# damaggu/StableKeypoints

Hardware: AMD Instinct MI355X
Metric: images/sec (token-opt step, 512², N=500 tokens) (higher is better)
Workload: dtype f32

## Files before the change

include/skp.h:

```cpp
#ifndef SKP_H
#define SKP_H

#ifdef __cplusplus
extern "C" {
#endif

#define SKP_OK 0
#define SKP_EBADARG (-1)
#define SKP_ELAUNCH (-2)
#define SKP_MAX_LAYERS 16

const char* skp_last_error(void);
int skp_version(void);

int skp_capture_fwd(const float* z_low, int BH, int s, int N, int R, float* attn, float* stats, void* stream);

int skp_capture_bwd(const float* z_low, int BH, int s, int N, int R, const float* dattn, int group, long long sb,
                    long long sp, long long sn, float gscale, const float* stats, float* dz_low, float* workspace,
                    void* stream);

int skp_capture_maps_fwd(const float* const* z_low, const int* sizes, int L, int B, int H, int N, int R, float* maps,
                         float* const* stats, void* stream);

int skp_capture_maps_bwd(const float* const* z_low, const int* sizes, int L, int B, int H, int N, int R,
                         const float* dmaps, float gscale, const float* const* stats, float* const* dz_low,
                         float* workspace, void* stream);

long long skp_capture_maps_bwd_sel_workspace(const int* sizes, int L, int B, int H, int N, int R, int K);
int skp_capture_maps_bwd_sel(const float* const* z_low, const int* sizes, int L, int B, int H, int N, int R,
                             const long long* sel_tok, int K, const float* gsel, float gscale,
                             const float* const* stats, float* const* dz_low, float* workspace, void* stream);
int skp_sel_bwd_timing(int enable);
int skp_sel_bwd_timing_read(double* ms, int* calls);

int skp_aggregate(const float* const* layers, int L, int BH, int RR, int N, const long long* indices,
                  int n_out, float* out, void* stream);

int skp_resize_bilinear(const float* in, int C, int R, int Ro, float* out, void* stream);
int skp_resize_bilinear_bwd(const float* gout, int C, int R, int Ro, float* gin, void* stream);

int skp_argmax2d(const float* maps, int T, int h, int w, const long long* rows, int n_rows, float* pos,
                 long long* idx, void* stream);

int skp_k_max_pixels(const float* maps, int T, int h, int w, int num, float radius2, float* pos,
                     float* masked, void* stream);

int skp_mask_radius(const float* maps, int T, int h, int w, const float* pos, float radius2, float* out,
                    void* stream);

int skp_weighted_avg(float* maps, int T, int h, int w, float distance, int mutate, float* pos, void* stream);

int skp_gaussian_target(const float* pos, int num, int T, int size, float sigma, float* out, void* stream);

int skp_topk_gaussian(const float* maps, int T, int h, int w, int top_k, float sigma, float epsilon,
                      int num_subjects, long long* out, double* kl, void* workspace, void* stream);

int skp_topk_gaussian_batch(const float* maps, int nb, int T, int h, int w, int top_k, float sigma,
                            float epsilon, int num_subjects, long long* out, double* kl, void* workspace,
                            void* stream);

int skp_topk_keys(const double* keys, int nb, int T, int top_k, long long* out, void* stream);

int skp_entropy_sort(const float* maps, int T, int h, int w, int top_k, long long* out, double* ent,
                     void* workspace, void* stream);

int skp_fps(const float* maps, int T, int h, int w, const long long* cand, int n_cand, int top_k,
            long long* out, int* n_out, void* workspace, void* stream);
int skp_fps_batch(const float* maps, int nb, int T, int h, int w, const long long* cand, int n_cand, int top_k,
                  long long* out, int* n_out, void* workspace, void* stream);
int skp_fps_keys_batch(const double* keys, const float* maps, int nb, int T, int h, int w, int n_cand, int top_k,
                       long long* cand, long long* out, int* n_out, void* workspace, void* stream);

int skp_sharpen_fwd(const float* A, int T, int h, int w, float sigma, int num_subjects, float* pos,
                     double* partial, float* loss, void* stream);
int skp_sharpen_bwd(const float* A, int T, int h, int w, float sigma, int num_subjects, const float* pos,
                     const float* gout, float* dA, void* stream);
int skp_sharpen_fwd_batch(const float* A, int nb, int T, int h, int w, float sigma, int num_subjects, float* pos,
                          double* partial, float* loss, void* stream);
int skp_sharpen_bwd_batch(const float* A, int nb, int T, int h, int w, float sigma, int num_subjects,
                          const float* pos, const float* gout, float* dA, void* stream);

int skp_affine_warp(const float* x, int B, int C, int H, int W, const float* theta, float* out, void* stream);
int skp_affine_warp_bwd(const float* gout, int B, int C, int H, int W, const float* theta, float* gin,
                        void* stream);

int skp_equiv_fwd(const float* A, const float* At, int T, int h, int w, const float* theta_inv,
                  double* partial, float* loss, void* stream);
int skp_equiv_bwd(const float* A, const float* At, int T, int h, int w, const float* theta_inv,
                  const float* gout, float* dA, float* dAt, void* stream);
int skp_equiv_fwd_batch(const float* A, const float* At, int nb, int T, int h, int w, const float* theta_inv,
                        double* partial, float* loss, void* stream);
int skp_equiv_bwd_batch(const float* A, const float* At, int nb, int T, int h, int w, const float* theta_inv,
                        const float* gout, float* dA, float* dAt, void* stream);

int skp_wino_in_transform(const float* x, int B, int C, int H, int W, float* V, void* stream);
int skp_wino_out_transform(const float* M, int B, int K, int H, int W, const float* bias, const float* residual,
                           float* y, void* stream);
int skp_wino_out_transform_kt(const float* M, int B, int K, int H, int W, const float* bias, const float* residual,
                              float* y, float* gn_part, void* stream);

int skp_bgemm_f32(const float* A, long long sAb, long long sAm, long long sAk, const float* B, long long sBb,
                  long long sBk, long long sBn, float* C, long long sCb, long long sCm, long long sCn, int batch,
                  int M, int N, int K, float alpha, int accumulate, void* stream);
int skp_bgemm_f32_2b(const float* A, long long sAo, long long sAb, long long sAm, long long sAk, const float* B,
                     long long sBo, long long sBb, long long sBk, long long sBn, float* C, long long sCo, long long sCb,
                     long long sCm, long long sCn, int batch, int hb, int M, int N, int K, float alpha, int accumulate,
                     void* stream);

int skp_groupnorm_workspace(int B, int C, long long HW, int G);
int skp_groupnorm_fwd(const float* x, const float* gamma, const float* beta, const float* shift, int B, int C,
                      long long HW, int G, float eps, int act, float* y, float* stats, double* partial,
                      void* stream);
int skp_groupnorm_bwd(const float* x, const float* dy, const float* gamma, const float* beta, const float* shift,
                      const float* stats, int B, int C, long long HW, int G, int act, float* dx, double* partial,
                      void* stream);
int skp_groupnorm_fwd_part(const float* x, const float* gamma, const float* beta, const float* shift, const float* part,
                           int nseg, int B, int C, long long HW, int G, float eps, int act, float* y, float* stats,
                           double* partial, void* stream);
int skp_groupnorm_stats(const float* x, const float* shift, int B, int C, long long HW, int G, float eps, float* stats,
                        double* partial, void* stream);
int skp_groupnorm_stats_part(const float* part, int nseg, const float* shift, int B, int C, long long HW, int G,
                             float eps, float* stats, double* partial, void* stream);
int skp_groupnorm_bwd_add(const float* x, const float* dy, const float* gamma, const float* beta, const float* shift,
                          const float* stats, int B, int C, long long HW, int G, int act, const float* dres, float* dx,
                          double* partial, void* stream);
int skp_softmax_bwd(const float* P, float* dP, long long rows, int cols, float alpha, void* stream);
int skp_softmax_fwd(float* S, long long rows, int cols, void* stream);
int skp_attn_dscore(const float* P, const float* dO, const float* V, const float* D, float* out, int BH, int S, int L,
                    int d, float alpha, void* stream);
int skp_attn_bwd_kv(const float* P, const float* dO, const float* Q, const float* V, const float* D, float* dS,
                    float* dV, float* dK, int BH, int S, int L, int d, float alpha, void* stream);
int skp_attn_fwd(const float* Q, const float* K, const float* V, float* O, float* stats, int BH, int S, int L, int d,
                 float scale, void* stream);
int skp_attn_bwd_flash(const float* Q, const float* K, const float* V, const float* dO, const float* stats,
                       const float* D, float* dS, float* dV, float* dK, int BH, int S, int L, int d, float scale,
                       void* stream);
int skp_attn_fwd_bshd(const float* Q, long long q_sb, int q_rs, const float* K, long long k_sb, int k_rs,
                      const float* V, long long v_sb, int v_rs, float* O, long long o_sb, int o_rs, float* stats, int B,
                      int H, int S, int L, int d, float scale, void* stream);
int skp_attn_bwd_flash_bshd(const float* Q, long long q_sb, int q_rs, const float* K, long long k_sb, int k_rs,
                            const float* V, long long v_sb, int v_rs, const float* dO, long long o_sb, int o_rs,
                            const float* stats, const float* D, float* dS, float* dV, long long dv_sb, int dv_rs,
                            float* dK, long long dk_sb, int dk_rs, int B, int H, int S, int L, int d, float scale,
                            void* stream);
int skp_layernorm_fwd(const float* x, const float* gamma, const float* beta, long long rows, int C, float eps, float* y,
                      float* stats, void* stream);
int skp_layernorm_bwd(const float* x, const float* dy, const float* gamma, const float* stats, long long rows, int C,
                      float* dx, void* stream);
int skp_layernorm_bwd_add(const float* x, const float* dy, const float* gamma, const float* stats, long long rows,
                          int C, const float* dres, float* dx, void* stream);
int skp_geglu_fwd(const float* h, long long rows, int I, float* out, void* stream);
int skp_geglu_bwd(const float* h, const float* dout, long long rows, int I, float* dh, void* stream);
int skp_residual_bias_add(const float* a, const float* h, const float* bias, int B, int C, long long HW,
                          float* out, void* stream);
int skp_wino_weights(const float* w, int K, int C, int flip, float* U, void* stream);
int skp_conv3x3_wino(const float* x, const float* U, const float* bias, const float* residual, float* y, int B, int C,
                     int K, int H, int W, int nsplit, float* ws, void* stream);
int skp_wino2_weights(const float* w, int K, int C, int flip, float* U, void* stream);
int skp_conv3x3_wino2(const float* x, const float* U, const float* bias, const float* residual, float* y, int B,
                      int C, int K, int H, int W, int nsplit, float* ws, void* stream);
int skp_conv3x3_wino2_gn(const float* x, const float* U, const float* bias, const float* residual, float* y, int B,
                         int C, int K, int H, int W, int nsplit, float* ws, float* gn_part, void* stream);
int skp_wino2_vtransform(const float* x, float* V, int B, int C, int H, int W, void* stream);
int skp_wino2_vtransform_gn(const float* x, const float* stats, const float* gamma, const float* beta,
                            const float* shift, int G, int act, float* V, int B, int C, int H, int W, void* stream);
int skp_conv3x3_wino2_v(const float* V, const float* U, const float* bias, const float* residual, float* y, int B,
                        int C, int K, int H, int W, int nsplit, float* ws, void* stream);
int skp_conv3x3_wino2_v_gn(const float* V, const float* U, const float* bias, const float* residual, float* y, int B,
                           int C, int K, int H, int W, int nsplit, float* ws, float* gn_part, void* stream);
int skp_conv3x3s2_wino2(const float* x, const float* U, const float* bias, float* y, int B, int C, int K, int H,
                        int W, int nsplit, float* ws, void* stream);

int skp_map_range(const float* maps, int n, int h, int w, float* range, void* stream);
int skp_render_sheet(const float* images, int n, int H, int W, const float* maps, int h, int w, const float* range,
                     const float* lut, float alpha, const float* points, int K, float radius,
                     const unsigned char* colors, int rows, int cols, int f, int pad, unsigned char* out,
                     void* stream);

int skp_tta_reduce_workspace(int B, int n, int S);
int skp_tta_reduce(const float* maps, int B, int C, int n, int S, const float* theta_inv, float* pos, float* avg,
                   void* workspace, void* stream);

#ifdef __cplusplus
}
#endif
#endif
```

stablekeypoints_amd/_lib.py:

```python
import ctypes
import os

import torch

_HERE = os.path.dirname(os.path.abspath(__file__))
LIB_PATH = os.environ.get("SKP_LIB", os.path.join(_HERE, "libskp.so"))

_c_int, _c_float, _c_ll, _p = ctypes.c_int, ctypes.c_float, ctypes.c_longlong, ctypes.c_void_p

_SIGS = {
    "skp_capture_fwd": [_p, _c_int, _c_int, _c_int, _c_int, _p, _p, _p],
    "skp_capture_bwd": [_p, _c_int, _c_int, _c_int, _c_int, _p, _c_int, _c_ll, _c_ll, _c_ll, _c_float, _p, _p, _p,
                        _p],
    "skp_capture_maps_fwd": [ctypes.POINTER(_p), ctypes.POINTER(_c_int), _c_int, _c_int, _c_int, _c_int, _c_int, _p,
                             ctypes.POINTER(_p), _p],
    "skp_capture_maps_bwd": [ctypes.POINTER(_p), ctypes.POINTER(_c_int), _c_int, _c_int, _c_int, _c_int, _c_int, _p,
                             _c_float, ctypes.POINTER(_p), ctypes.POINTER(_p), _p, _p],
    "skp_capture_maps_bwd_sel": [ctypes.POINTER(_p), ctypes.POINTER(_c_int), _c_int, _c_int, _c_int, _c_int, _c_int,
                                 _p, _c_int, _p, _c_float, ctypes.POINTER(_p), ctypes.POINTER(_p), _p, _p],
    "skp_sel_bwd_timing": [_c_int],
    "skp_sel_bwd_timing_read": [_p, _p],
    "skp_capture_maps_bwd_sel_workspace": [ctypes.POINTER(_c_int), _c_int, _c_int, _c_int, _c_int, _c_int, _c_int],
    "skp_aggregate": [ctypes.POINTER(_p), _c_int, _c_int, _c_int, _c_int, _p, _c_int, _p, _p],
    "skp_resize_bilinear": [_p, _c_int, _c_int, _c_int, _p, _p],
    "skp_resize_bilinear_bwd": [_p, _c_int, _c_int, _c_int, _p, _p],
    "skp_argmax2d": [_p, _c_int, _c_int, _c_int, _p, _c_int, _p, _p, _p],
    "skp_k_max_pixels": [_p, _c_int, _c_int, _c_int, _c_int, _c_float, _p, _p, _p],
    "skp_mask_radius": [_p, _c_int, _c_int, _c_int, _p, _c_float, _p, _p],
    "skp_weighted_avg": [_p, _c_int, _c_int, _c_int, _c_float, _c_int, _p, _p],
    "skp_gaussian_target": [_p, _c_int, _c_int, _c_int, _c_float, _p, _p],
    "skp_topk_gaussian": [_p, _c_int, _c_int, _c_int, _c_int, _c_float, _c_float, _c_int, _p, _p, _p, _p],
    "skp_topk_gaussian_batch": [_p, _c_int, _c_int, _c_int, _c_int, _c_int, _c_float, _c_float, _c_int, _p, _p, _p,
                                _p],
    "skp_topk_keys": [_p, _c_int, _c_int, _c_int, _p, _p],
    "skp_entropy_sort": [_p, _c_int, _c_int, _c_int, _c_int, _p, _p, _p, _p],
    "skp_fps": [_p, _c_int, _c_int, _c_int, _p, _c_int, _c_int, _p, _p, _p, _p],
    "skp_fps_batch": [_p, _c_int, _c_int, _c_int, _c_int, _p, _c_int, _c_int, _p, _p, _p, _p],
    "skp_fps_keys_batch": [_p, _p, _c_int, _c_int, _c_int, _c_int, _c_int, _c_int, _p, _p, _p, _p, _p],
    "skp_sharpen_fwd": [_p, _c_int, _c_int, _c_int, _c_float, _c_int, _p, _p, _p, _p],
    "skp_sharpen_bwd": [_p, _c_int, _c_int, _c_int, _c_float, _c_int, _p, _p, _p, _p],
    "skp_wino_in_transform": [_p, _c_int, _c_int, _c_int, _c_int, _p, _p],
    "skp_wino_out_transform": [_p, _c_int, _c_int, _c_int, _c_int, _p, _p, _p, _p],
    "skp_wino_out_transform_kt": [_p, _c_int, _c_int, _c_int, _c_int, _p, _p, _p, _p, _p],
    "skp_sharpen_fwd_batch": [_p, _c_int, _c_int, _c_int, _c_int, _c_float, _c_int, _p, _p, _p, _p],
    "skp_sharpen_bwd_batch": [_p, _c_int, _c_int, _c_int, _c_int, _c_float, _c_int, _p, _p, _p, _p],
    "skp_affine_warp": [_p, _c_int, _c_int, _c_int, _c_int, _p, _p, _p],
    "skp_affine_warp_bwd": [_p, _c_int, _c_int, _c_int, _c_int, _p, _p, _p],
    "skp_equiv_fwd": [_p, _p, _c_int, _c_int, _c_int, _p, _p, _p, _p],
    "skp_equiv_bwd": [_p, _p, _c_int, _c_int, _c_int, _p, _p, _p, _p, _p],
    "skp_equiv_fwd_batch": [_p, _p, _c_int, _c_int, _c_int, _c_int, _p, _p, _p, _p],
    "skp_equiv_bwd_batch": [_p, _p, _c_int, _c_int, _c_int, _c_int, _p, _p, _p, _p, _p],
    "skp_bgemm_f32": [_p, _c_ll, _c_ll, _c_ll, _p, _c_ll, _c_ll, _c_ll, _p, _c_ll, _c_ll, _c_ll, _c_int, _c_int,
                      _c_int, _c_int, _c_float, _c_int, _p],
    "skp_bgemm_f32_2b": [_p, _c_ll, _c_ll, _c_ll, _c_ll, _p, _c_ll, _c_ll, _c_ll, _c_ll, _p, _c_ll, _c_ll, _c_ll,
                         _c_ll, _c_int, _c_int, _c_int, _c_int, _c_int, _c_float, _c_int, _p],
    "skp_groupnorm_workspace": [_c_int, _c_int, _c_ll, _c_int],
    "skp_groupnorm_fwd": [_p, _p, _p, _p, _c_int, _c_int, _c_ll, _c_int, _c_float, _c_int, _p, _p, _p, _p],
    "skp_groupnorm_bwd": [_p, _p, _p, _p, _p, _p, _c_int, _c_int, _c_ll, _c_int, _c_int, _p, _p, _p],
    "skp_groupnorm_bwd_add": [_p, _p, _p, _p, _p, _p, _c_int, _c_int, _c_ll, _c_int, _c_int, _p, _p, _p, _p],
    "skp_residual_bias_add": [_p, _p, _p, _c_int, _c_int, _c_ll, _p, _p],
    "skp_softmax_bwd": [_p, _p, _c_ll, _c_int, _c_float, _p],
    "skp_softmax_fwd": [_p, _c_ll, _c_int, _p],
    "skp_attn_dscore": [_p, _p, _p, _p, _p, _c_int, _c_int, _c_int, _c_int, _c_float, _p],
    "skp_attn_bwd_kv": [_p, _p, _p, _p, _p, _p, _p, _p, _c_int, _c_int, _c_int, _c_int, _c_float, _p],
    "skp_attn_fwd": [_p, _p, _p, _p, _p, _c_int, _c_int, _c_int, _c_int, _c_float, _p],
    "skp_attn_bwd_flash": [_p, _p, _p, _p, _p, _p, _p, _p, _p, _c_int, _c_int, _c_int, _c_int, _c_float, _p],
    "skp_attn_fwd_bshd": [_p, _c_ll, _c_int, _p, _c_ll, _c_int, _p, _c_ll, _c_int, _p, _c_ll, _c_int, _p, _c_int, _c_int,
                          _c_int, _c_int, _c_int, _c_float, _p],
    "skp_attn_bwd_flash_bshd": [_p, _c_ll, _c_int, _p, _c_ll, _c_int, _p, _c_ll, _c_int, _p, _c_ll, _c_int, _p, _p, _p,
                                _p, _c_ll, _c_int, _p, _c_ll, _c_int, _c_int, _c_int, _c_int, _c_int, _c_int, _c_float,
                                _p],
    "skp_layernorm_fwd": [_p, _p, _p, _c_ll, _c_int, _c_float, _p, _p, _p],
    "skp_layernorm_bwd": [_p, _p, _p, _p, _c_ll, _c_int, _p, _p],
    "skp_layernorm_bwd_add": [_p, _p, _p, _p, _c_ll, _c_int, _p, _p, _p],
    "skp_geglu_fwd": [_p, _c_ll, _c_int, _p, _p],
    "skp_geglu_bwd": [_p, _p, _c_ll, _c_int, _p, _p],
    "skp_wino_weights": [_p, _c_int, _c_int, _c_int, _p, _p],
    "skp_conv3x3_wino": [_p, _p, _p, _p, _p, _c_int, _c_int, _c_int, _c_int, _c_int, _c_int, _p, _p],
    "skp_wino2_weights": [_p, _c_int, _c_int, _c_int, _p, _p],
    "skp_conv3x3_wino2": [_p, _p, _p, _p, _p, _c_int, _c_int, _c_int, _c_int, _c_int, _c_int, _p, _p],
    "skp_conv3x3_wino2_gn": [_p, _p, _p, _p, _p, _c_int, _c_int, _c_int, _c_int, _c_int, _c_int, _p, _p, _p],
    "skp_groupnorm_fwd_part": [_p, _p, _p, _p, _p, _c_int, _c_int, _c_int, _c_ll, _c_int, _c_float, _c_int, _p, _p, _p,
                               _p],
    "skp_groupnorm_stats": [_p, _p, _c_int, _c_int, _c_ll, _c_int, _c_float, _p, _p, _p],
    "skp_groupnorm_stats_part": [_p, _c_int, _p, _c_int, _c_int, _c_ll, _c_int, _c_float, _p, _p, _p],
    "skp_wino2_vtransform": [_p, _p, _c_int, _c_int, _c_int, _c_int, _p],
    "skp_wino2_vtransform_gn": [_p, _p, _p, _p, _p, _c_int, _c_int, _p, _c_int, _c_int, _c_int, _c_int, _p],
    "skp_conv3x3_wino2_v": [_p, _p, _p, _p, _p, _c_int, _c_int, _c_int, _c_int, _c_int, _c_int, _p, _p],
    "skp_conv3x3_wino2_v_gn": [_p, _p, _p, _p, _p, _c_int, _c_int, _c_int, _c_int, _c_int, _c_int, _p, _p, _p],
    "skp_conv3x3s2_wino2":[_p, _p, _p, _p, _c_int, _c_int, _c_int, _c_int, _c_int, _c_int, _p, _p],
    "skp_map_range": [_p, _c_int, _c_int, _c_int, _p, _p],
    "skp_render_sheet": [_p, _c_int, _c_int, _c_int, _p, _c_int, _c_int, _p, _p, _c_float, _p, _c_int, _c_float, _p,
                         _c_int, _c_int, _c_int, _c_int, _p, _p],
    "skp_tta_reduce_workspace": [_c_int, _c_int, _c_int],
    "skp_tta_reduce": [_p, _c_int, _c_int, _c_int, _c_int, _p, _p, _p, _p, _p],
    "skp_version": [],
}


_RESTYPE = {"skp_capture_maps_bwd_sel_workspace": _c_ll}
_MEASUREMENT_ONLY = {"skp_sel_bwd_timing", "skp_sel_bwd_timing_read"}


class SkpLibraryError(RuntimeError):
    pass


_lib = None


def lib():
    global _lib
    if _lib is None:
        if not os.path.exists(LIB_PATH):
            raise SkpLibraryError(f"libskp.so not found at {LIB_PATH}: build it with "
                                  "`python -c 'import __graft_entry__ as g; g.build()'` or `make -C stablekeypoints_amd/csrc`")
        try:
            L = ctypes.CDLL(LIB_PATH)
        except OSError as e:
            raise SkpLibraryError(f"cannot load {LIB_PATH}: {e}") from e
        for name, args in _SIGS.items():
            if name in _MEASUREMENT_ONLY and not hasattr(L, name):
                continue
            f = getattr(L, name)
            f.argtypes = args
            f.restype = _RESTYPE.get(name, _c_int)
        L.skp_last_error.argtypes = []
        L.skp_last_error.restype = ctypes.c_char_p
        _lib = L
    return _lib


def exported_symbols():
    return list(_SIGS) + ["skp_last_error"]


def call(name, *args):
    rc = getattr(lib(), name)(*args)
    if rc != 0:
        msg = lib().skp_last_error().decode(errors="replace")
        raise RuntimeError(f"{name} failed (rc={rc}): {msg}")


def ptr(t):
    return None if t is None else ctypes.c_void_p(t.data_ptr())


def stream(device=None):
    return ctypes.c_void_p(torch.cuda.current_stream(device).cuda_stream)


def require_device(*tensors):
    for t in tensors:
        if t is not None and not t.is_cuda:
            raise ValueError("stablekeypoints_amd ops run on the HIP device only; got a CPU tensor "
                             "(there is no CPU fallback: the CPU oracle lives under oracle/ and is test-only)")
```

stablekeypoints_amd/csrc/skp_conv.hip:

```cpp
#include <cstdlib>

#include "skp_common.h"
#include "skp_gn.h"

using namespace skp;

#ifndef SKP_WINO_DEBUG
#define SKP_WINO_DEBUG 0
#endif
#ifndef SKP_WINO2_DEBUG
#define SKP_WINO2_DEBUG 0
#endif

namespace {

typedef float f32x4 __attribute__((ext_vector_type(4)));
typedef unsigned int u32x4 __attribute__((ext_vector_type(4)));

constexpr int kMT = 64;
constexpr int kNC = 32;
constexpr int kCK = 4;
constexpr int kP = 36;
constexpr int kThreads = 512;
constexpr int kUs = kCK * kNC * kP;
constexpr int kUChunks = kUs * 4 / 1024;
constexpr int kRawRow = 64 * 16 + 64 * 4 + 64 * 4;
constexpr int kRawWave = 6 * kRawRow;

static_assert(kMT == 64 && kCK == 4, "wave w of 0..3 = stage channel w, lane = tile");
static_assert(kUs * 4 % 1024 == 0, "U stage in whole 1-KB chunks");

typedef __attribute__((address_space(3))) void* lds_ptr_t;

__device__ __forceinline__ void bt6(float a0, float a1, float a2, float a3, float a4, float a5, float* y, int s) {
  y[0 * s] = a0 - 1.5f * a1 - 2.0f * a2 + 1.5f * a3 + a4;
  y[1 * s] = -a1 + 0.5f * a2 + 2.5f * a3 + a4;
  y[2 * s] = a1 - 2.5f * a2 + 0.5f * a3 + a4;
  y[3 * s] = -2.0f * a1 - a2 + 2.0f * a3 + a4;
  y[4 * s] = 0.5f * a1 - a2 - 0.5f * a3 + a4;
  y[5 * s] = a1 - 1.5f * a2 - 2.0f * a3 + 1.5f * a4 + a5;
}

__device__ __forceinline__ void at6(float m0, float m1, float m2, float m3, float m4, float m5, float* y, int s) {
  const float p = m1 + m2, q = m1 - m2;
  y[0 * s] = m0 + p + m3 + m4;
  y[1 * s] = q + 0.5f * m3 - 2.0f * m4;
  y[2 * s] = p + 0.25f * m3 + 4.0f * m4;
  y[3 * s] = q + 0.125f * m3 - 8.0f * m4 + m5;
}

__device__ __forceinline__ void input_transform(const float* d, float* v) {
  float t[36];
#pragma unroll
  for (int c = 0; c < 6; ++c) bt6(d[c], d[6 + c], d[12 + c], d[18 + c], d[24 + c], d[30 + c], t + c, 6);
#pragma unroll
  for (int r = 0; r < 6; ++r) bt6(t[6 * r], t[6 * r + 1], t[6 * r + 2], t[6 * r + 3], t[6 * r + 4], t[6 * r + 5], v + 6 * r, 1);
}

__device__ __forceinline__ void output_transform(const float* m, float* y) {
  float s[24];
#pragma unroll
  for (int c = 0; c < 6; ++c) at6(m[c], m[6 + c], m[12 + c], m[18 + c], m[24 + c], m[30 + c], s + c, 6);
#pragma unroll
  for (int r = 0; r < 4; ++r) at6(s[6 * r], s[6 * r + 1], s[6 * r + 2], s[6 * r + 3], s[6 * r + 4], s[6 * r + 5], y + 4 * r, 1);
}

struct PatchAddr {
  unsigned row[6];
  unsigned dl;
  unsigned mask;
};

__device__ __forceinline__ void dma_patches(__amdgpu_buffer_rsrc_t rs, const PatchAddr& pa, char* raw) {
#pragma unroll
  for (int r = 0; r < 6; ++r) {
    char* dst = raw + r * kRawRow;
    __builtin_amdgcn_raw_ptr_buffer_load_lds(rs, (lds_ptr_t)dst, 16, pa.row[r], 0, 0, 0);
    __builtin_amdgcn_raw_ptr_buffer_load_lds(rs, (lds_ptr_t)(dst + 1024), 4, pa.row[r] - pa.dl, 0, 0, 0);
    __builtin_amdgcn_raw_ptr_buffer_load_lds(rs, (lds_ptr_t)(dst + 1280), 4, pa.row[r] + 16, 0, 0, 0);
  }
}

__device__ __forceinline__ void transform_patch(const char* raw, unsigned mask, int lane, float* vd, bool store = true) {
  float d[36];
#pragma unroll
  for (int r = 0; r < 6; ++r) {
    const char* row = raw + r * kRawRow;
    const float4 m = *reinterpret_cast<const float4*>(row + lane * 16);
    const float l = *reinterpret_cast<const float*>(row + 1024 + lane * 4);
    const float rr = *reinterpret_cast<const float*>(row + 1280 + lane * 4);
    const bool ok = (mask >> r) & 1u;
    d[6 * r + 0] = (ok && (mask & 64u)) ? l : 0.0f;
    d[6 * r + 1] = ok ? m.x : 0.0f;
    d[6 * r + 2] = ok ? m.y : 0.0f;
    d[6 * r + 3] = ok ? m.z : 0.0f;
    d[6 * r + 4] = ok ? m.w : 0.0f;
    d[6 * r + 5] = (ok && (mask & 128u)) ? rr : 0.0f;
  }
#pragma unroll
  for (int c = 0; c < 6; ++c) {
    float t[6];
    bt6(d[c], d[6 + c], d[12 + c], d[18 + c], d[24 + c], d[30 + c], t, 1);
#pragma unroll
    for (int i = 0; i < 6; ++i) d[6 * i + c] = t[i];
  }
#pragma unroll
  for (int i = 0; i < 6; ++i) {
    float v[6];
    bt6(d[6 * i], d[6 * i + 1], d[6 * i + 2], d[6 * i + 3], d[6 * i + 4], d[6 * i + 5], v, 1);
    if (store) {
      *reinterpret_cast<float2*>(vd + 6 * i) = make_float2(v[0], v[1]);
      *reinterpret_cast<float2*>(vd + 6 * i + 2) = make_float2(v[2], v[3]);
      *reinterpret_cast<float2*>(vd + 6 * i + 4) = make_float2(v[4], v[5]);
    }
  }
}

template <int EPI, int MT>
__global__ __launch_bounds__(kThreads) __attribute__((amdgpu_waves_per_eu(2, 2))) void wino_f4_kernel(
    const float* __restrict__ x, const float* __restrict__ U, const float* __restrict__ bias,
    const float* __restrict__ res, float* __restrict__ y, int nimg, int C, int K, int H, int W, int tw, int tpi,
    int ntiles, int ntb, int nkb, int kb_major, int csplit, int dbg) {
  constexpr int NC = kMT * kNC / MT;
  constexpr int VS = kCK * MT * kP, US = kCK * NC * kP;
  constexpr int NWM = MT / 16;
  __shared__ __attribute__((aligned(16))) float V0[VS], V1[VS];
  __shared__ __attribute__((aligned(16))) float U0[US], U1[US];
  __shared__ __attribute__((aligned(16))) char Raw[4 * kRawWave];

  const int G = gridDim.x;
  const int g = blockIdx.x;
  const int Lg = (G % 8 == 0) ? (g % 8) * (G / 8) + g / 8 : g;
  const int sp = Lg / (ntb * nkb);
  const int L = Lg - sp * (ntb * nkb);
  int tb, kb;
  if (kb_major) {
    kb = L / ntb;
    tb = L - kb * ntb;
  } else {
    tb = L / nkb;
    kb = L - tb * nkb;
  }
  const int c0 = sp * csplit;
  y += (size_t)sp * nimg * K * ((EPI & 4) ? (H / 2) * (W / 2) : H * W);

  const int tid = threadIdx.x, lane = tid & 63;
  const int wv = __builtin_amdgcn_readfirstlane(tid >> 6);
  const int wm = wv % NWM, wn = wv / NWM;
  const bool patcher = wv < 4;
  const size_t plane = (size_t)H * W;
  PatchAddr pa;
  {
    const int pt = tb * MT + lane;
    const bool pvalid = lane < MT && pt < ntiles;
    int pb = 0, py0 = 0, px0 = 0;
    if (pvalid) {
      pb = pt / tpi;
      const int r = pt - pb * tpi;
      const int ty = r / tw;
      py0 = 4 * ty;
      px0 = 4 * (r - ty * tw);
    }
    const unsigned base = (unsigned)(((size_t)pb * C + (wv & 3)) * plane);
    pa.mask = (px0 > 0 ? 64u : 0u) | (px0 + 4 < W ? 128u : 0u);
    pa.dl = px0 > 0 ? 4u : 0u;
#pragma unroll
    for (int r = 0; r < 6; ++r) {
      const int yy = py0 - 1 + r;
      if (pvalid && yy >= 0 && yy < H) pa.mask |= 1u << r;
      const int yc = yy < 0 ? 0 : (yy >= H ? H - 1 : yy);
      pa.row[r] = (base + (unsigned)(yc * W + px0)) * 4u;
    }
  }
  const float* Ub = U + ((size_t)(kb * (NC / kNC)) * C + c0) * kNC * kP;
  const size_t uhalf = (size_t)C * kNC * kP;
  const int nst = csplit / kCK;
  const size_t xfloats = (size_t)nimg * C * plane;
  char* raw = Raw + (wv & 3) * kRawWave;
  const bool vstore = lane < MT;
  const int vrow = ((wv & 3) * MT + (vstore ? lane : 0)) * kP;
  auto xrsrc = [&](int s) {
    const size_t off = ((size_t)c0 + (size_t)s * kCK) * plane;
    return __builtin_amdgcn_make_buffer_rsrc((void*)(x + off), (short)0, (dbg & 1) ? 0 : (int)((xfloats - off) * 4), 0x00020000);
  };
  auto dma_u = [&](int s, float* ubuf) {
    char* dst = reinterpret_cast<char*>(ubuf);
#pragma unroll
    for (int h = 0; h < NC / kNC; ++h) {
      const __amdgpu_buffer_rsrc_t rs = __builtin_amdgcn_make_buffer_rsrc(
          (void*)(Ub + h * uhalf + (size_t)s * kUs), (short)0, (dbg & 2) ? 0 : kUs * 4, 0x00020000);
#pragma unroll
      for (int c = wv - 4; c < kUChunks; c += 4)
        __builtin_amdgcn_raw_ptr_buffer_load_lds(rs, (lds_ptr_t)(dst + h * kUs * 4 + c * 1024), 16, lane * 16, c * 1024,
                                                 0, 0);
    }
  };

  f32x4 acc[kP];
#pragma unroll
  for (int p = 0; p < kP; ++p) acc[p] = f32x4{0.f, 0.f, 0.f, 0.f};

  if (patcher) {
    dma_patches(xrsrc(0), pa, raw);
    __builtin_amdgcn_s_waitcnt(0);
    transform_patch(raw, pa.mask, lane, V0 + vrow, vstore);
    if (nst > 1) dma_patches(xrsrc(1), pa, raw);
  } else {
    dma_u(0, U0);
  }
  __builtin_amdgcn_s_waitcnt(0);
  __syncthreads();

  const int aoff = ((lane >> 4) * MT + wm * 16 + (lane & 15)) * kP;
  const int boff = (wn >> 1) * kUs + ((lane >> 4) * kNC + (wn & 1) * 16 + (lane & 15)) * kP;
  auto phase = [&](int s, const float* vc, const float* uc, float* vn, float* un) {
    if (s + 1 < nst) {
      if (patcher) {
        if (!(dbg & 4)) transform_patch(raw, pa.mask, lane, vn + vrow, vstore);
        if (s + 2 < nst) dma_patches(xrsrc(s + 2), pa, raw);
      } else {
        dma_u(s + 1, un);
      }
    }
    const float* va = vc + aoff;
    const float* ub = uc + boff;
#pragma unroll
    for (int q = 0; q < 9; ++q) {
      if (dbg & 8) break;
      const float4 a = *reinterpret_cast<const float4*>(va + 4 * q);
      const float4 b = *reinterpret_cast<const float4*>(ub + 4 * q);
      acc[4 * q + 0] = __builtin_amdgcn_mfma_f32_16x16x4f32(a.x, b.x, acc[4 * q + 0], 0, 0, 0);
      acc[4 * q + 1] = __builtin_amdgcn_mfma_f32_16x16x4f32(a.y, b.y, acc[4 * q + 1], 0, 0, 0);
      acc[4 * q + 2] = __builtin_amdgcn_mfma_f32_16x16x4f32(a.z, b.z, acc[4 * q + 2], 0, 0, 0);
      acc[4 * q + 3] = __builtin_amdgcn_mfma_f32_16x16x4f32(a.w, b.w, acc[4 * q + 3], 0, 0, 0);
    }
    __builtin_amdgcn_s_waitcnt(0);
    __syncthreads();
  };
  for (int s = 0; s < nst; s += 2) {
    phase(s, V0, U0, V1, U1);
    if (s + 1 < nst) phase(s + 1, V1, U1, V0, U0);
  }

  const int k = kb * NC + wn * 16 + (lane & 15);
  const float bv = (EPI & 1) ? bias[k] : 0.0f;
#pragma unroll
  for (int r = 0; r < 4; ++r) {
    const int t = tb * MT + wm * 16 + 4 * (lane >> 4) + r;
    if (t >= ntiles) continue;
    float m[36], o[16];
#pragma unroll
    for (int p = 0; p < kP; ++p) m[p] = acc[p][r];
    output_transform(m, o);
    const int b = t / tpi;
    const int rr = t - b * tpi;
    const int ty = rr / tw;
    const int tx = rr - ty * tw;
    const size_t off = ((size_t)b * K + k) * plane + (size_t)(4 * ty) * W + 4 * tx;
#pragma unroll
    for (int i = 0; i < 4; ++i) {
      float4 val = make_float4(o[4 * i] + bv, o[4 * i + 1] + bv, o[4 * i + 2] + bv, o[4 * i + 3] + bv);
      if (EPI & 2) {
        const float4 rv = *reinterpret_cast<const float4*>(res + off + (size_t)i * W);
        val.x += rv.x;
        val.y += rv.y;
        val.z += rv.z;
        val.w += rv.w;
      }
      *reinterpret_cast<float4*>(y + off + (size_t)i * W) = val;
    }
  }
}

__global__ void wino_weights_kernel(const float* __restrict__ w, int K, int C, int flip, float* __restrict__ U) {
  const long long i = blockIdx.x * (long long)blockDim.x + threadIdx.x;
  if (i >= (long long)K * C) return;
  const int k = (int)(i / C), c = (int)(i - (long long)k * C);
  double g[9];
  for (int u = 0; u < 3; ++u)
    for (int v = 0; v < 3; ++v)
      g[3 * u + v] = flip ? (double)w[((size_t)c * K + k) * 9 + (2 - u) * 3 + (2 - v)]
                          : (double)w[((size_t)k * C + c) * 9 + u * 3 + v];
  const double Gm[6][3] = {{1.0, 0.0, 0.0},
                           {1.0 / 3, 1.0 / 3, 1.0 / 3},
                           {-1.0 / 3, 1.0 / 3, -1.0 / 3},
                           {-16.0 / 15, -8.0 / 15, -4.0 / 15},
                           {1.0 / 15, -2.0 / 15, 4.0 / 15},
                           {0.0, 0.0, 1.0}};
  double t[6][3];
  for (int a = 0; a < 6; ++a)
    for (int v = 0; v < 3; ++v) t[a][v] = Gm[a][0] * g[v] + Gm[a][1] * g[3 + v] + Gm[a][2] * g[6 + v];
  float* out = U + (((size_t)(k / kNC) * C + c) * kNC + (k % kNC)) * kP;
  for (int a = 0; a < 6; ++a)
    for (int b = 0; b < 6; ++b) out[6 * a + b] = (float)(t[a][0] * Gm[b][0] + t[a][1] * Gm[b][1] + t[a][2] * Gm[b][2]);
}

bool aligned16(const void* p) { return (reinterpret_cast<uintptr_t>(p) & 15) == 0; }

}

extern "C" int skp_wino_weights(const float* w, int K, int C, int flip, float* U, void* stream) {
  SKP_CHECK_ARG(w && U, "null pointer");
  SKP_CHECK_ARG(K > 0 && C > 0, "non-positive shape");
  SKP_CHECK_ARG(K % kNC == 0, "output channels must be a multiple of 32");
  const long long n = (long long)K * C;
  hipLaunchKernelGGL(wino_weights_kernel, dim3((unsigned)((n + 255) / 256)), dim3(256), 0, as_stream(stream), w, K, C,
                     flip, U);
  SKP_LAUNCH_CHECK();
  return SKP_OK;
}

namespace {

__global__ void splitk_reduce_kernel(const float4* __restrict__ ws, int nsplit, long long n4, int K, int hw4,
                                     const float* __restrict__ bias, const float4* __restrict__ res,
                                     float4* __restrict__ y) {
  const long long i = blockIdx.x * (long long)blockDim.x + threadIdx.x;
  if (i >= n4) return;
  float4 v = ws[i];
  for (int s = 1; s < nsplit; ++s) {
    const float4 p = ws[(long long)s * n4 + i];
    v.x += p.x;
    v.y += p.y;
    v.z += p.z;
    v.w += p.w;
  }
  if (bias) {
    const float b = bias[(i / hw4) % K];
    v.x += b;
    v.y += b;
    v.z += b;
    v.w += b;
  }
  if (res) {
    const float4 r = res[i];
    v.x += r.x;
    v.y += r.y;
    v.z += r.z;
    v.w += r.w;
  }
  y[i] = v;
}

int splitk_reduce(const float* ws, int nsplit, int B, int K, int HW, const float* bias, const float* residual,
                  float* y, hipStream_t st) {
  const long long n4 = (long long)B * K * HW / 4;
  hipLaunchKernelGGL(splitk_reduce_kernel, dim3((unsigned)((n4 + 255) / 256)), dim3(256), 0, st,
                     reinterpret_cast<const float4*>(ws), nsplit, n4, K, HW / 4, bias,
                     reinterpret_cast<const float4*>(residual), reinterpret_cast<float4*>(y));
  SKP_LAUNCH_CHECK();
  return SKP_OK;
}

}

extern "C" int skp_conv3x3_wino(const float* x, const float* U, const float* bias, const float* residual, float* y,
                                int B, int C, int K, int H, int W, int nsplit, float* ws, void* stream) {
  SKP_CHECK_ARG(x && U && y, "null pointer");
  SKP_CHECK_ARG(B > 0 && C > 0 && K > 0 && H > 0 && W > 0, "non-positive shape");
  SKP_CHECK_ARG(C % kCK == 0, "input channels must be a multiple of 4");
  SKP_CHECK_ARG(K % kNC == 0, "output channels must be a multiple of 32");
  SKP_CHECK_ARG(H % 4 == 0 && W % 4 == 0, "H and W must be multiples of 4");
  SKP_CHECK_ARG(nsplit >= 1 && C % (kCK * nsplit) == 0, "nsplit must divide C into multiples of 4");
  SKP_CHECK_ARG(nsplit == 1 || ws, "split-K needs a workspace of nsplit·B·K·H·W floats");
  SKP_CHECK_ARG(aligned16(x) && aligned16(U) && aligned16(y) && (!residual || aligned16(residual)) &&
                    (!ws || aligned16(ws)),
                "tensors must be 16-byte aligned");
  const int tw = W / 4, tpi = (H / 4) * tw;
  const long long ntiles = (long long)B * tpi;
  SKP_CHECK_ARG(ntiles <= 0x7fffffffLL - kMT, "too many tiles");
  SKP_CHECK_ARG((long long)B * C * H * W * 4 < 0x7fffffffLL, "input larger than 2 GiB (32-bit buffer offsets)");
  const bool wide = ntiles <= 32 && K % 64 == 0;
  const int mt = wide ? 32 : kMT;
  const int ntb = (int)((ntiles + mt - 1) / mt), nkb = K / (wide ? 64 : kNC);
  SKP_CHECK_ARG((long long)ntb * nkb * nsplit <= 0x7fffffffLL, "grid too large");
  const long long ubytes = (long long)K * C * kP * 4;
  const int kb_major = ubytes > (2LL << 20);
  const int epi = nsplit > 1 ? 0 : (bias ? 1 : 0) | (residual ? 2 : 0);
  float* out = nsplit > 1 ? ws : y;
  const int dbg = SKP_WINO_DEBUG;
  hipStream_t st = as_stream(stream);
  const dim3 grid((unsigned)(ntb * nkb * nsplit));
#define SKP_WG(E)                                                                                                    \
  if (wide)                                                                                                          \
    hipLaunchKernelGGL((wino_f4_kernel<E, 32>), grid, dim3(kThreads), 0, st, x, U, bias, residual, out, B, C, K, H, W, \
                       tw, tpi, (int)ntiles, ntb, nkb, kb_major, C / nsplit, dbg);                                    \
  else                                                                                                               \
    hipLaunchKernelGGL((wino_f4_kernel<E, 64>), grid, dim3(kThreads), 0, st, x, U, bias, residual, out, B, C, K, H, W, \
                       tw, tpi, (int)ntiles, ntb, nkb, kb_major, C / nsplit, dbg)
  switch (epi) {
    case 0: SKP_WG(0); break;
    case 1: SKP_WG(1); break;
    case 2: SKP_WG(2); break;
    default: SKP_WG(3); break;
  }
#undef SKP_WG
  SKP_LAUNCH_CHECK();
  if (nsplit > 1) return splitk_reduce(ws, nsplit, B, K, H * W, bias, residual, y, st);
  return SKP_OK;
}

namespace {
namespace w2 {

constexpr int kNC = 32;
constexpr int kCK = 4;
template <int TXB>
struct Geo;
template <>
struct Geo<8> {
  static constexpr int NI = 1, RR = 34, RC = 10, CHF = 1408;
};
template <>
struct Geo<4> {
  static constexpr int NI = 4, RR = 18, RC = 6, CHF = 1744;
};
template <int TXB, int NW>
struct GeoN : Geo<TXB> {};
template <>
struct GeoN<8, 4> {
  static constexpr int NI = 1, RR = 18, RC = 10, CHF = 768;
};
template <>
struct GeoN<4, 4> {
  static constexpr int NI = 2, RR = 18, RC = 6, CHF = 880;
};
template <int TXB, int NW = 8>
struct GeoT : GeoN<TXB, NW> {
  using GeoN<TXB, NW>::NI;
  using GeoN<TXB, NW>::RR;
  using GeoN<TXB, NW>::RC;
  using GeoN<TXB, NW>::CHF;
  static constexpr int RF = 4 * RC;
  static constexpr int RAWF = (4 * CHF + 255) / 256 * 256;
  static constexpr int RAW_INSTR = RAWF / 256;
  static_assert(NI * RR * RF <= CHF, "channel region");
};
constexpr int kUP = 40;
constexpr int kUF = kCK * kNC * kUP;
constexpr int kUInstr = kUF / 256;
constexpr unsigned kOOB = 0x80000000u;
constexpr int kVWF = 4 * 256 + 128;
constexpr int kVF = 4 * kVWF;
typedef unsigned int u32x2 __attribute__((ext_vector_type(2)));
static_assert(kUF % 256 == 0, "whole 1-KB chunks");
static_assert((4 * GeoT<8>::RAWF + 3 * kUF) * 4 <= 160 * 1024 && 3 * (GeoT<4>::RAWF + kUF) * 4 <= 160 * 1024, "LDS");
static_assert(2 * 8 * 1024 <= kUF * 4, "epilogue exchange: two waves' 8 KB per ring buffer");

__device__ constexpr float kBt[6][6] = {{1.f, -1.5f, -2.f, 1.5f, 1.f, 0.f},  {0.f, -1.f, 0.5f, 2.5f, 1.f, 0.f},
                                        {0.f, 1.f, -2.5f, 0.5f, 1.f, 0.f},  {0.f, -2.f, -1.f, 2.f, 1.f, 0.f},
                                        {0.f, 0.5f, -1.f, -0.5f, 1.f, 0.f}, {0.f, 1.f, -1.5f, -2.f, 1.5f, 1.f}};
__device__ constexpr float kAt[4][6] = {{1.f, 1.f, 1.f, 1.f, 1.f, 0.f},
                                        {0.f, 1.f, -1.f, 0.5f, -2.f, 0.f},
                                        {0.f, 1.f, 1.f, 0.25f, 4.f, 0.f},
                                        {0.f, 1.f, -1.f, 0.125f, -8.f, 1.f}};

#ifndef SKP_W2_PACKED
#define SKP_W2_PACKED 1
#endif
#if SKP_W2_PACKED
#define W2_TRANSFORM half_transform_pk
#else
#define W2_TRANSFORM half_transform
#endif

#define W2_VMCNT(n) __builtin_amdgcn_s_waitcnt(((n) & 15) | (((n) >> 4) << 14) | (7 << 4) | (15 << 8))

template <int H, int RF>
__device__ __forceinline__ void half_transform(const float* raw, float* a) {
  float t[3][6];
#pragma unroll
  for (int r = 0; r < 6; ++r) {
    const float4 c0 = *reinterpret_cast<const float4*>(raw + r * RF);
    const float4 c1 = *reinterpret_cast<const float4*>(raw + r * RF + 4);
    const float4 c2 = *reinterpret_cast<const float4*>(raw + r * RF + 8);
    const float d[6] = {c0.w, c1.x, c1.y, c1.z, c1.w, c2.x};
#pragma unroll
    for (int ii = 0; ii < 3; ++ii) {
      const float c = kBt[3 * H + ii][r];
      if (c == 0.0f) continue;
      bool first = true;
#pragma unroll
      for (int rp = 0; rp < r; ++rp)
        if (kBt[3 * H + ii][rp] != 0.0f) first = false;
#pragma unroll
      for (int b = 0; b < 6; ++b)
        t[ii][b] = first ? ((c == 1.0f) ? d[b] : c * d[b]) : ((c == 1.0f) ? t[ii][b] + d[b] : fmaf(c, d[b], t[ii][b]));
    }
    asm volatile("" ::"v"(c0.x), "v"(c0.y), "v"(c0.z), "v"(c2.y), "v"(c2.z), "v"(c2.w));
  }
#pragma unroll
  for (int ii = 0; ii < 3; ++ii) bt6(t[ii][0], t[ii][1], t[ii][2], t[ii][3], t[ii][4], t[ii][5], a + 6 * ii, 1);
}

typedef float f2 __attribute__((ext_vector_type(2)));

template <typename T>
__device__ __forceinline__ void bt6_shared(T a0, T a1, T a2, T a3, T a4, T a5, T* y) {
  const T e = a4 - a2, f = a3 - a1, g = a2 + a3, h = a3 - a2;
  y[0] = __builtin_elementwise_fma((T)1.5f, f, (a0 + e) - a2);
  y[1] = __builtin_elementwise_fma((T)1.5f, g, e + f);
  y[2] = __builtin_elementwise_fma((T)1.5f, h, e - f);
  y[3] = __builtin_elementwise_fma((T)2.0f, f, e);
  y[4] = __builtin_elementwise_fma((T)-0.5f, f, e);
  y[5] = __builtin_elementwise_fma((T)1.5f, e, __builtin_elementwise_fma((T)-2.0f, f, a5 - a1));
}

template <int H, int RF>
__device__ __forceinline__ void half_transform_pk(const float* raw, float* a) {
  f2 t[3][3];
  f2 k0[3], k1[3], k2[3], k3[3];
#pragma unroll
  for (int r = 0; r < 6; ++r) {
    if (H == 1 && r == 0) continue;
    const f32x4 c0 = *reinterpret_cast<const f32x4*>(raw + r * RF);
    const f32x4 c1 = *reinterpret_cast<const f32x4*>(raw + r * RF + 4);
    const f32x4 c2 = *reinterpret_cast<const f32x4*>(raw + r * RF + 8);
    const f2 d[3] = {__builtin_shufflevector(c1, c1, 0, 1), __builtin_shufflevector(c1, c1, 2, 3),
                     __builtin_shufflevector(c0, c2, 3, 4)};
#pragma unroll
    for (int p = 0; p < 3; ++p) {
      if (H == 0) {
        if (r == 0) k0[p] = d[p];
        if (r == 1) { k1[p] = d[p]; k0[p] = __builtin_elementwise_fma((f2)-1.5f, d[p], k0[p]); }
        if (r == 2) { k2[p] = d[p]; k3[p] = __builtin_elementwise_fma((f2)1.5f, d[p], -k1[p]); }
        if (r == 3) { k1[p] = __builtin_elementwise_fma((f2)1.5f, d[p], -k2[p]); k3[p] = k3[p] + d[p]; }
        if (r == 4) {
          const f2 sv = k1[p] + d[p];
          t[0][p] = k0[p] + (sv - k2[p]);
          t[1][p] = sv + k3[p];
          t[2][p] = sv - k3[p];
        }
      } else {
        if (r == 1) k0[p] = d[p];
        if (r == 2) k1[p] = d[p];
        if (r == 3) { k2[p] = d[p] - k0[p]; k3[p] = __builtin_elementwise_fma((f2)-2.0f, k2[p], -k0[p]); }
        if (r == 4) {
          const f2 e = d[p] - k1[p];
          t[0][p] = __builtin_elementwise_fma((f2)2.0f, k2[p], e);
          t[1][p] = __builtin_elementwise_fma((f2)-0.5f, k2[p], e);
          k3[p] = __builtin_elementwise_fma((f2)1.5f, e, k3[p]);
        }
        if (r == 5) t[2][p] = k3[p] + d[p];
      }
    }
    asm volatile("" ::"v"(c0.x), "v"(c0.y), "v"(c0.z), "v"(c2.y), "v"(c2.z), "v"(c2.w));
  }
  const f2 u0 = __builtin_shufflevector(t[0][2], t[1][2], 0, 2), u1 = __builtin_shufflevector(t[0][0], t[1][0], 0, 2);
  const f2 u2 = __builtin_shufflevector(t[0][0], t[1][0], 1, 3), u3 = __builtin_shufflevector(t[0][1], t[1][1], 0, 2);
  const f2 u4 = __builtin_shufflevector(t[0][1], t[1][1], 1, 3), u5 = __builtin_shufflevector(t[0][2], t[1][2], 1, 3);
  f2 y01[6];
  bt6_shared<f2>(u0, u1, u2, u3, u4, u5, y01);
  float y2[6];
  bt6_shared<float>(t[2][2].x, t[2][0].x, t[2][0].y, t[2][1].x, t[2][1].y, t[2][2].y, y2);
#pragma unroll
  for (int j = 0; j < 6; ++j) {
    a[j] = y01[j].x;
    a[6 + j] = y01[j].y;
    a[12 + j] = y2[j];
  }
}

template <int H>
__device__ __forceinline__ void half_output(const float* m, float* y) {
  float s[3][4];
#pragma unroll
  for (int ii = 0; ii < 3; ++ii) at6(m[6 * ii], m[6 * ii + 1], m[6 * ii + 2], m[6 * ii + 3], m[6 * ii + 4], m[6 * ii + 5], s[ii], 1);
#pragma unroll
  for (int r = 0; r < 4; ++r)
#pragma unroll
    for (int c = 0; c < 4; ++c) {
      float v = 0.0f;
      bool first = true;
#pragma unroll
      for (int ii = 0; ii < 3; ++ii) {
        const float a = kAt[r][3 * H + ii];
        if (a == 0.0f) continue;
        v = first ? ((a == 1.0f) ? s[ii][c] : a * s[ii][c]) : fmaf(a, s[ii][c], v);
        first = false;
      }
      y[4 * r + c] = v;
    }
}

}

struct W2Smem {
  float *R0, *R1, *R2, *R3, *U0, *U1, *U2;
};

__device__ __forceinline__ void w2_vmcnt(int n) {
  switch (n) {
    case 0: W2_VMCNT(0); break;
    case 1: W2_VMCNT(1); break;
    case 2: W2_VMCNT(2); break;
    case 3: W2_VMCNT(3); break;
    case 4: W2_VMCNT(4); break;
    case 5: W2_VMCNT(5); break;
    case 6: W2_VMCNT(6); break;
    case 7: W2_VMCNT(7); break;
    case 8: W2_VMCNT(8); break;
    case 9: W2_VMCNT(9); break;
    case 10: W2_VMCNT(10); break;
    case 11: W2_VMCNT(11); break;
    case 12: W2_VMCNT(12); break;
    case 13: W2_VMCNT(13); break;
    case 14: W2_VMCNT(14); break;
    case 15: W2_VMCNT(15); break;
    default: W2_VMCNT(0); break;
  }
}

#ifndef SKP_W2_RS4
#define SKP_W2_RS4 0
#endif

template <int EPI, int HH, int TXB, int NW, bool VST = false>
__device__ __forceinline__ void wino2_body(const W2Smem& sm, const float* __restrict__ x, const float* __restrict__ U,
                                           const float* __restrict__ bias, const float* __restrict__ res,
                                           float* __restrict__ y, int C, int K, int H, int W, int img, int x0,
                                           int y0, int kb, int c0, int csplit, int wv, int dbg,
                                           float2* __restrict__ gnp) {
  using Geo = w2::GeoT<TXB, NW>;
  constexpr int kChF = Geo::CHF, kRowF = Geo::RF, kRawInstr = Geo::RAW_INSTR, NI = Geo::NI, RR = Geo::RR,
                RC = Geo::RC;
  constexpr int kInstr = kRawInstr + w2::kUInstr;
  constexpr int kMaxRaw = (kRawInstr + NW - 1) / NW;
  constexpr int kMaxU = (w2::kUInstr + NW - 1) / NW + 1;
  constexpr int NT = NW * WAVE;
  constexpr int US = NW == 4 ? 2 : 3;
  using w2::kUF;
  using w2::kUP;
  static_assert(!VST || (TXB == 8 && NW == 4), "V-staged form: half-height blocks of 4 waves");
  constexpr int RS = (VST || (TXB == 4 && NW == 4)) ? 2 : (TXB == 8 && NW == 8 && SKP_W2_RS4) ? 4 : 3;
  float *R0 = sm.R0, *R1 = sm.R1, *R2 = sm.R2, *U0 = sm.U0, *U1 = sm.U1, *U2 = sm.U2;
  const int tid = threadIdx.x, lane = tid & 63;
  const int wm = wv % (NW / 2);
  const size_t plane = (size_t)H * W;
  const size_t ximg = (size_t)img * C * plane;

  unsigned voff[kMaxRaw];
  int nraw = 0;
#pragma unroll
  for (int m = 0; m < kMaxRaw; ++m) {
    const int gi = wv + NW * m;
    voff[m] = w2::kOOB;
    if (gi < kRawInstr) {
      ++nraw;
      const int f = 64 * gi + lane;
      const int ch = f / (kChF / 4);
      const int e = f - ch * (kChF / 4);
      const int ii = e / (RR * RC), rem = e - ii * (RR * RC);
      const int row = rem / RC, c4 = rem - row * RC;
      const int yy = y0 - 1 + row, xx = x0 - 4 + 4 * c4;
      if (ch < w2::kCK && ii < NI && yy >= 0 && yy < H && xx >= 0 && xx < W)
        voff[m] = (unsigned)((ximg + ((size_t)ii * C + ch) * plane + (size_t)yy * W + xx) * 4);
    }
  }
  const int nuw = (kInstr - 1 - wv) / NW + 1 - nraw;
  const int ufirst = wv + NW * nraw - kRawInstr;
  const int allow_step = RS == 2 ? 0 : US == 2 ? nraw : RS == 4 ? nuw + 2 * nraw : nuw + nraw;
  const int allow_pro = RS == 2 ? nuw + nraw : US == 2 ? nuw + 2 * nraw : RS == 4 ? 2 * nuw + 3 * nraw : 2 * nuw + 2 * nraw;
  const size_t xend = (size_t)(img + NI) * C * plane;
  const float* Ub = U + ((size_t)kb * C + c0) * w2::kNC * kUP;
  const int nst = csplit / w2::kCK;

  auto issue_raw = [&](int t, float* rs_lds) {
    const bool ok = t < nst;
    const size_t off = ((size_t)c0 + (size_t)(ok ? t : 0) * w2::kCK) * plane;
    const __amdgpu_buffer_rsrc_t rx = __builtin_amdgcn_make_buffer_rsrc(
        (void*)(x + off), (short)0, ok ? (int)((xend - off) * 4) : 0, 0x00020000);
#pragma unroll
    for (int m = 0; m < kMaxRaw; ++m)
      if (m < nraw && !(dbg & 4))
        __builtin_amdgcn_raw_ptr_buffer_load_lds(rx, (lds_ptr_t)(rs_lds + 256 * (wv + NW * m)), 16, voff[m], 0, 0, 0);
  };
  auto issue_u = [&](int t, float* us_lds) {
    const __amdgpu_buffer_rsrc_t ru =
        __builtin_amdgcn_make_buffer_rsrc((void*)(Ub + (size_t)t * kUF), (short)0, kUF * 4, 0x00020000);
#pragma unroll
    for (int m = 0; m < kMaxU; ++m)
      if (m < nuw && !(dbg & 8)) {
        const int q = ufirst + NW * m;
        __builtin_amdgcn_raw_ptr_buffer_load_lds(ru, (lds_ptr_t)(us_lds + 256 * q), 16, lane * 16, q * 1024, 0, 0);
      }
  };

  const int kc = lane >> 4;
  const int tx = lane & (TXB - 1);
  const int ty = TXB == 8 ? 2 * wm + ((lane >> 3) & 1) : (lane >> 2) & 3;
  const int roff = kc * kChF + (TXB == 8 ? 0 : wm * RR * kRowF) + 4 * ty * kRowF + 4 * tx;
  const int uoff = (kc * w2::kNC + (lane & 15)) * kUP + 20 * HH;

  f32x4 acc[2][18];
#pragma unroll
  for (int b = 0; b < 2; ++b)
#pragma unroll
    for (int q = 0; q < 18; ++q) acc[b][q] = f32x4{0.f, 0.f, 0.f, 0.f};
  float a0[18], a1[18];

  auto mfmas = [&](const float* us, const float (&acur)[18]) {
#pragma unroll
    for (int b = 0; b < 2; ++b) {
      const float* ub = us + uoff + b * 16 * kUP;
      float u[18];
#pragma unroll
      for (int j = 0; j < 4; ++j) {
        const float4 v = *reinterpret_cast<const float4*>(ub + 4 * j);
        u[4 * j] = v.x;
        u[4 * j + 1] = v.y;
        u[4 * j + 2] = v.z;
        u[4 * j + 3] = v.w;
      }
      const float2 v2 = *reinterpret_cast<const float2*>(ub + 16);
      u[16] = v2.x;
      u[17] = v2.y;
#pragma unroll
      for (int q = 0; q < 18; ++q) acc[b][q] = __builtin_amdgcn_mfma_f32_16x16x4f32(acur[q], u[q], acc[b][q], 0, 0, 0);
    }
  };

  if constexpr (VST) {
    using w2::kVF;
    using w2::kVWF;
    const int bw = W >> 5;
    const size_t tb = (size_t)img * ((H >> 4) * bw) + (size_t)(y0 >> 4) * bw + (x0 >> 5);
    const float* Vb = x + (tb * (size_t)(C / w2::kCK) + (size_t)(c0 / w2::kCK)) * kVF + wv * kVWF;
    asm volatile("" : "+s"(Vb));
    struct AReg {
      u32x4 c[4];
      w2::u32x2 d;
    };
    auto issue_vu = [&](int t, AReg& an, float* us_lds) {
      const bool ok = t < nst;
      const size_t tt = ok ? (size_t)t : 0;
      const __amdgpu_buffer_rsrc_t rv =
          __builtin_amdgcn_make_buffer_rsrc((void*)(Vb + tt * kVF), (short)0, ok ? kVWF * 4 : 0, 0x00020000);
      const __amdgpu_buffer_rsrc_t ru =
          __builtin_amdgcn_make_buffer_rsrc((void*)(Ub + tt * kUF), (short)0, ok ? kUF * 4 : 0, 0x00020000);
#pragma unroll
      for (int j = 0; j < 4; ++j) an.c[j] = __builtin_amdgcn_raw_buffer_load_b128(rv, lane * 16, j * 1024, 0);
      an.d = __builtin_amdgcn_raw_buffer_load_b64(rv, lane * 8, 4096, 0);
#pragma unroll
      for (int m = 0; m < w2::kUInstr / NW; ++m) {
        const int q = wv + NW * m;
        __builtin_amdgcn_raw_ptr_buffer_load_lds(ru, (lds_ptr_t)(us_lds + 256 * q), 16, lane * 16, q * 1024, 0, 0);
      }
    };
    static_assert(w2::kUInstr % NW == 0, "whole chunks per wave");
    constexpr int kPerStage = 5 + w2::kUInstr / NW;
    auto vstep = [&](int s, const AReg& ac, const float* Us, AReg& ai, float* Ui) {
      W2_VMCNT(kPerStage);
      asm volatile("" ::: "memory");
      __builtin_amdgcn_s_waitcnt(0xC07F);
      __builtin_amdgcn_s_barrier();
      asm volatile("" ::: "memory");
      asm volatile("" ::"v"(ac.c[0]), "v"(ac.c[1]), "v"(ac.c[2]), "v"(ac.c[3]), "v"(ac.d));
      issue_vu(s + 2, ai, Ui);
      __builtin_amdgcn_sched_barrier(0);
      if (s < nst) {
        float a[18];
#pragma unroll
        for (int j = 0; j < 4; ++j)
#pragma unroll
          for (int i = 0; i < 4; ++i) {
            const unsigned v = ac.c[j][i];
            a[4 * j + i] = __uint_as_float(v);
          }
        const unsigned d0 = ac.d[0], d1 = ac.d[1];
        a[16] = __uint_as_float(d0);
        a[17] = __uint_as_float(d1);
        mfmas(Us, a);
      }
    };
    AReg A0, A1, A2;
    issue_vu(0, A0, U0);
    asm volatile("" ::: "memory");
    __builtin_amdgcn_sched_barrier(0);
    issue_vu(1, A1, U1);
    for (int s0 = 0; s0 < nst; s0 += 3) {
      vstep(s0, A0, U0, A2, U2);
      vstep(s0 + 1, A1, U1, A0, U0);
      vstep(s0 + 2, A2, U2, A1, U1);
    }
  } else {
    issue_raw(0, R0);
    if (RS == 4) issue_raw(1, R1);
    issue_u(0, U0);
    if (RS >= 3) issue_raw(RS - 2, RS == 4 ? R2 : R1);
    if (US == 3 && nst > 1) issue_u(1, U1);
    issue_raw(RS - 1, RS == 4 ? sm.R3 : RS == 3 ? R2 : R1);
    w2_vmcnt(nst > 1 ? allow_pro : 0);
    __syncthreads();
    w2::W2_TRANSFORM<HH, kRowF>(R0 + roff, a0);

    auto step = [&](int s, float* Rn, float* Us, float* Ri, float* Ui, const float (&acur)[18], float (&anext)[18]) {
      w2_vmcnt(s + 1 < nst ? allow_step : 0);
      __syncthreads();
      if (s + US - 1 < nst) issue_u(s + US - 1, Ui);
      issue_raw(s + RS, Ri);
      const bool tr = s + 1 < nst && !(dbg & 1);
      if (HH == 0) {
        if (tr) w2::W2_TRANSFORM<HH, kRowF>(Rn + roff, anext);
        if (!(dbg & 2)) mfmas(Us, acur);
      } else {
        if (!(dbg & 2)) mfmas(Us, acur);
        if (tr) w2::W2_TRANSFORM<HH, kRowF>(Rn + roff, anext);
      }
    };
    constexpr int PER = RS == 4 ? 12 : RS == 2 ? 2 : 6;
    float* const Rsl[4] = {R0, R1, R2, sm.R3};
    float* const Usl[3] = {U0, U1, U2};
    for (int s0 = 0; s0 < ((dbg & 16) ? 0 : nst); s0 += PER) {
      step(s0, Rsl[1 % RS], Usl[0], Rsl[0], Usl[US - 1], a0, a1);
  #pragma unroll
      for (int j = 1; j < PER; ++j) {
        if (s0 + j < nst) {
          if ((j & 1) == 0) step(s0 + j, Rsl[(j + 1) % RS], Usl[j % US], Rsl[j % RS], Usl[(j + US - 1) % US], a0, a1);
          else step(s0 + j, Rsl[(j + 1) % RS], Usl[j % US], Rsl[j % RS], Usl[(j + US - 1) % US], a1, a0);
        }
      }
    }

  }

  W2_VMCNT(0);
  __syncthreads();
  if (dbg & 32) return;
  constexpr int PH = (TXB == 8 && NW == 4) ? 16 : 32;
  constexpr int PLS = (TXB == 8 ? PH * 32 : NI * 256) + 4;
  float* const P2 = RS == 2 ? U1 : R2;
  auto plane_of = [&](int c) -> float* {
    float* b = (c >> 2) == 0 ? R0 : (c >> 2) == 1 ? R1 : (c >> 2) == 2 ? P2 : U0;
    return b + (c & 3) * PLS + (c >> 2) * 16;
  };
  float* pl = plane_of(lane & 15);
  const int pbase = TXB == 8 ? (4 * (2 * wm + (lane >> 5))) * 32 + 4 * (4 * ((lane >> 4) & 1))
                             : wm * 256 + (4 * (lane >> 4)) * 16;
  constexpr int PW = TXB == 8 ? 32 : 16;
#pragma unroll
  for (int blk = 0; blk < 2; ++blk) {
    if (HH != blk) {
#pragma unroll
      for (int r = 0; r < 4; ++r) {
        float m[18], o[16];
#pragma unroll
        for (int q = 0; q < 18; ++q) m[q] = acc[blk][q][r];
        w2::half_output<HH>(m, o);
#pragma unroll
        for (int f = 0; f < 4; ++f)
          *reinterpret_cast<float4*>(pl + pbase + f * PW + 4 * r) =
              make_float4(o[4 * f], o[4 * f + 1], o[4 * f + 2], o[4 * f + 3]);
      }
    }
    __syncthreads();
    if (HH == blk) {
#pragma unroll
      for (int r = 0; r < 4; ++r) {
        float m[18], o[16];
#pragma unroll
        for (int q = 0; q < 18; ++q) m[q] = acc[blk][q][r];
        w2::half_output<HH>(m, o);
#pragma unroll
        for (int f = 0; f < 4; ++f) {
          float4* d = reinterpret_cast<float4*>(pl + pbase + f * PW + 4 * r);
          const float4 p = *d;
          *d = make_float4(o[4 * f] + p.x, o[4 * f + 1] + p.y, o[4 * f + 2] + p.z, o[4 * f + 3] + p.w);
        }
      }
    }
    __syncthreads();
    if constexpr ((EPI & 4) != 0) {
      static_assert(TXB == 8 && (EPI & 2) == 0, "stride-2 output: 32-wide blocks, no residual");
      const int Ho = H / 2, Wo = W / 2;
      constexpr int PC2 = (PH / 2) * 4;
#pragma unroll
      for (int i = 0; i < 16 * PC2 / NT; ++i) {
        const int idx = i * NT + tid;
        const int c = idx / PC2, q = idx % PC2;
        const int row = q >> 2, c4 = q & 3;
        const float* pp = plane_of(c) + (2 * row + 1) * 32 + 8 * c4 + 1;
        const int k = kb * w2::kNC + 16 * blk + c;
        const float bv = (EPI & 1) ? bias[k] : 0.0f;
        const size_t o = (((size_t)img * K + k) * Ho + y0 / 2 + row) * Wo + x0 / 2 + 4 * c4;
        const float4 v = make_float4(pp[0] + bv, pp[2] + bv, pp[4] + bv, pp[6] + bv);
        if (dbg & 128) __builtin_nontemporal_store(f32x4{v.x, v.y, v.z, v.w}, reinterpret_cast<f32x4*>(y + o));
        else if (!(dbg & 64)) *reinterpret_cast<float4*>(y + o) = v;
      }
      if (blk == 0) __syncthreads();
      continue;
    }
    constexpr int PCF = TXB == 8 ? PH * 8 : NI * 64;
    constexpr int NIT = 16 * PCF / NT;
    static_assert(TXB != 8 || NIT == 8, "TXB 8: eight wave instructions per wave");
    float g1[4] = {0.f, 0.f, 0.f, 0.f}, g2[4] = {0.f, 0.f, 0.f, 0.f}, piv[4] = {0.f, 0.f, 0.f, 0.f};
#pragma unroll
    for (int i = 0; i < NIT; ++i) {
      const int idx = TXB == 8 ? (((tid >> 6) * NIT + i) << 6) + (tid & 63) : i * NT + tid;
      const int c = idx / PCF, q = idx % PCF;
      const float4 v0 = *reinterpret_cast<const float4*>(plane_of(c) + 4 * q);
      const int k = kb * w2::kNC + 16 * blk + c;
      const float bv = (EPI & 1) ? bias[k] : 0.0f;
      size_t o;
      if (TXB == 8) {
        const int row = q >> 3, c4 = q & 7;
        o = (((size_t)img * K + k) * H + y0 + row) * W + x0 + 4 * c4;
      } else {
        o = ((size_t)(img + (q >> 6)) * K + k) * 256 + 4 * (q & 63);
      }
      float4 v = make_float4(v0.x + bv, v0.y + bv, v0.z + bv, v0.w + bv);
      if (EPI & 2) {
        const float4 rv = *reinterpret_cast<const float4*>(res + o);
        v.x += rv.x;
        v.y += rv.y;
        v.z += rv.z;
        v.w += rv.w;
      }
      if (dbg & 128) __builtin_nontemporal_store(f32x4{v.x, v.y, v.z, v.w}, reinterpret_cast<f32x4*>(y + o));
      else if (!(dbg & 64)) *reinterpret_cast<float4*>(y + o) = v;
      if (TXB == 8 && gnp) {
        if ((i & 1) == 0) piv[i >> 1] = __builtin_bit_cast(float, __builtin_amdgcn_readfirstlane(__builtin_bit_cast(int, v.x)));
        const float p = piv[i >> 1];
        const float dx = v.x - p, dy = v.y - p, dz = v.z - p, dw = v.w - p;
        g1[i >> 1] += (dx + dy) + (dz + dw);
        g2[i >> 1] += (dx * dx + dy * dy) + (dz * dz + dw * dw);
      }
    }
    if (TXB == 8 && gnp) {
      float a[4] = {g1[0], g2[0], g1[1], g2[1]}, b[4] = {g1[2], g2[2], g1[3], g2[3]};
      float u[4];
#pragma unroll
      for (int j = 0; j < 4; ++j) {
        asm volatile("s_nop 1\n\tv_permlane32_swap_b32 %0, %1" : "+v"(a[j]), "+v"(b[j]));
        u[j] = a[j] + b[j];
      }
      float w[2];
#pragma unroll
      for (int j = 0; j < 2; ++j) {
        float x0 = u[j], x1 = u[j + 2];
        asm volatile("s_nop 1\n\tv_permlane16_swap_b32 %0, %1" : "+v"(x0), "+v"(x1));
        w[j] = x0 + x1;
      }
      const int lane = tid & 63;
      const bool hi = (lane & 8) != 0;
      const float keep = hi ? w[1] : w[0], send = hi ? w[0] : w[1];
      float x = keep + dpp_read<0x140>(send);
      x += dpp_read<0x141>(x);
      x += dpp_read<0x4E>(x);
      x += dpp_read<0xB1>(x);
      const float x2 = __shfl_xor(x, 8, 64);
      if ((lane & 15) == 0) {
        const int r = lane >> 4;
        const int J = (tid >> 6) * NIT + 2 * r;
        const int c = (J << 6) / PCF, piece = ((J << 6) % PCF) >> 6;
        const int k = kb * w2::kNC + 16 * blk + c;
        const int seg = ((y0 + 8 * piece) >> 4) * (W >> 5) + (x0 >> 5);
        const float p = r == 0 ? piv[0] : r == 1 ? piv[1] : r == 2 ? piv[2] : piv[3];
        constexpr float inv_n = 1.0f / 512.0f;
        gnp[((size_t)img * K + k) * (size_t)((H >> 4) * (W >> 5)) + seg] =
            make_float2(p + x * inv_n, fmaxf(x2 - x * (x * inv_n), 0.0f));
      }
    }
    if (blk == 0) __syncthreads();
  }
}

template <int EPI, int TXB, int NW = 8>
__global__ __launch_bounds__(NW * WAVE) __attribute__((amdgpu_waves_per_eu(2, 2))) void wino2_kernel(
    const float* __restrict__ x, const float* __restrict__ U, const float* __restrict__ bias,
    const float* __restrict__ res, float* __restrict__ y, int nimg, int C, int K, int H, int W, int bw, int bpi,
    int nblk, int nkb, int kb_major, int csplit, int dbg, float2* __restrict__ gnp) {
  __shared__ __attribute__((aligned(16))) float R0[w2::GeoT<TXB, NW>::RAWF], R1[w2::GeoT<TXB, NW>::RAWF],
      R2[(TXB == 4 && NW == 4) ? 4 : w2::GeoT<TXB, NW>::RAWF],
      R3[(TXB == 8 && NW == 8 && SKP_W2_RS4) ? w2::GeoT<TXB, NW>::RAWF : 4];
  __shared__ __attribute__((aligned(16))) float U0[w2::kUF], U1[w2::kUF], U2[NW == 4 ? 4 : w2::kUF];
  const int G = gridDim.x;
  const int g = blockIdx.x;
  const int Lg = (G % 8 == 0) ? (g % 8) * (G / 8) + g / 8 : g;
  const int sp = Lg / (nblk * nkb);
  const int L = Lg - sp * (nblk * nkb);
  y += (size_t)sp * nimg * K * ((EPI & 4) ? (H / 2) * (W / 2) : H * W);
  int tb, kb;
  if (kb_major) {
    kb = L / nblk;
    tb = L - kb * nblk;
  } else {
    tb = L / nkb;
    kb = L - tb * nkb;
  }
  int img, x0 = 0, y0 = 0;
  if (TXB == 8) {
    img = tb / bpi;
    const int br = tb - img * bpi;
    const int by = br / bw;
    x0 = 32 * (br - by * bw);
    y0 = (NW == 4 ? 16 : 32) * by;
  } else {
    img = (NW == 4 ? 2 : 4) * tb;
  }
  const int wv = __builtin_amdgcn_readfirstlane(threadIdx.x >> 6);
  const W2Smem sm{R0, R1, R2, R3, U0, U1, U2};
  const int c0 = sp * csplit;
  if (wv < NW / 2)
    wino2_body<EPI, 0, TXB, NW>(sm, x, U, bias, res, y, C, K, H, W, img, x0, y0, kb, c0, csplit, wv, dbg, gnp);
  else wino2_body<EPI, 1, TXB, NW>(sm, x, U, bias, res, y, C, K, H, W, img, x0, y0, kb, c0, csplit, wv, dbg, gnp);
}

__global__ void wino2_weights_kernel(const float* __restrict__ w, int K, int C, int flip, float* __restrict__ U) {
  const long long i = blockIdx.x * (long long)blockDim.x + threadIdx.x;
  if (i >= (long long)K * C) return;
  const int k = (int)(i / C), c = (int)(i - (long long)k * C);
  double g[9];
  for (int u = 0; u < 3; ++u)
    for (int v = 0; v < 3; ++v)
      g[3 * u + v] = flip ? (double)w[((size_t)c * K + k) * 9 + (2 - u) * 3 + (2 - v)]
                          : (double)w[((size_t)k * C + c) * 9 + u * 3 + v];
  const double Gm[6][3] = {{1.0, 0.0, 0.0},
                           {1.0 / 3, 1.0 / 3, 1.0 / 3},
                           {-1.0 / 3, 1.0 / 3, -1.0 / 3},
                           {-16.0 / 15, -8.0 / 15, -4.0 / 15},
                           {1.0 / 15, -2.0 / 15, 4.0 / 15},
                           {0.0, 0.0, 1.0}};
  double t[6][3];
  for (int a = 0; a < 6; ++a)
    for (int v = 0; v < 3; ++v) t[a][v] = Gm[a][0] * g[v] + Gm[a][1] * g[3 + v] + Gm[a][2] * g[6 + v];
  float* out = U + (((size_t)(k / w2::kNC) * C + c) * w2::kNC + (k % w2::kNC)) * w2::kUP;
  for (int p = 0; p < w2::kUP; ++p) out[p] = 0.0f;
  for (int a = 0; a < 6; ++a)
    for (int b = 0; b < 6; ++b) {
      const int p = 6 * a + b;
      out[p < 18 ? p : p + 2] = (float)(t[a][0] * Gm[b][0] + t[a][1] * Gm[b][1] + t[a][2] * Gm[b][2]);
    }
}

template <int EPI>
__global__ __launch_bounds__(4 * WAVE) __attribute__((amdgpu_waves_per_eu(2, 2))) void wino2v_kernel(
    const float* __restrict__ V, const float* __restrict__ U, const float* __restrict__ bias,
    const float* __restrict__ res, float* __restrict__ y, int nimg, int C, int K, int H, int W, int bw, int bpi,
    int nblk, int nkb, int kb_major, int csplit, int dbg, float2* __restrict__ gnp) {
  __shared__ __attribute__((aligned(16))) float U0[w2::kUF], U1[w2::kUF], U2[w2::kUF];
  static_assert(3 * w2::kUF * 4 <= 80 * 1024, "two workgroups per CU");
  static_assert(4 * (16 * 32 + 4) + 48 <= w2::kUF / 2, "a plane buffer per half U slot");
  const int G = gridDim.x;
  const int g = blockIdx.x;
  const int Lg = (G % 8 == 0) ? (g % 8) * (G / 8) + g / 8 : g;
  const int sp = Lg / (nblk * nkb);
  const int L = Lg - sp * (nblk * nkb);
  y += (size_t)sp * nimg * K * H * W;
  int tb, kb;
  if (kb_major) {
    kb = L / nblk;
    tb = L - kb * nblk;
  } else {
    tb = L / nkb;
    kb = L - tb * nkb;
  }
  const int img = tb / bpi;
  const int br = tb - img * bpi;
  const int by = br / bw;
  const int x0 = 32 * (br - by * bw), y0 = 16 * by;
  const int wv = __builtin_amdgcn_readfirstlane(threadIdx.x >> 6);
  const W2Smem sm{U0 + w2::kUF / 2, U1 + w2::kUF / 2, nullptr, nullptr, U0, U1, U2};
  const int c0 = sp * csplit;
  if (wv < 2)
    wino2_body<EPI, 0, 8, 4, true>(sm, V, U, bias, res, y, C, K, H, W, img, x0, y0, kb, c0, csplit, wv, dbg, gnp);
  else wino2_body<EPI, 1, 8, 4, true>(sm, V, U, bias, res, y, C, K, H, W, img, x0, y0, kb, c0, csplit, wv, dbg, gnp);
}

template <int GN>
__global__ __launch_bounds__(4 * WAVE) void wino2_vtransform_kernel(
    const float* __restrict__ x, const float* __restrict__ stats, const float* __restrict__ gamma,
    const float* __restrict__ beta, const float* __restrict__ shift, int G, float* __restrict__ V, int C, int H, int W,
    int bw, int bpi) {
  using Geo = w2::GeoT<8, 4>;
  constexpr int RR = Geo::RR, RC = Geo::RC, kChF = Geo::CHF, kRowF = Geo::RF;
  __shared__ __attribute__((aligned(16))) float R[Geo::RAWF];
  const int tid = threadIdx.x, lane = tid & 63;
  const int nst = C / w2::kCK;
  const int tb = blockIdx.x / nst, st = blockIdx.x - tb * nst;
  const int img = tb / bpi;
  const int br = tb - img * bpi;
  const int by = br / bw;
  const int x0 = 32 * (br - by * bw), y0 = 16 * by;
  const int cpg = C / (G > 0 ? G : 1);
  for (int f = tid; f < w2::kCK * RR * RC; f += 4 * WAVE) {
    const int ch = f / (RR * RC), e = f - ch * (RR * RC);
    const int row = e / RC, c4 = e - row * RC;
    const int yy = y0 - 1 + row, xx = x0 - 4 + 4 * c4;
    float4 v = make_float4(0.f, 0.f, 0.f, 0.f);
    if (yy >= 0 && yy < H && xx >= 0 && xx < W) {
      const int c = w2::kCK * st + ch;
      v = *reinterpret_cast<const float4*>(x + (((size_t)img * C + c) * H + yy) * W + xx);
      if (GN) {
        const int grp = img * G + c / cpg;
        const GNCoef k = gn_coef(gamma[c], beta[c], stats[2 * grp], stats[2 * grp + 1]);
        const float t = shift ? shift[(size_t)img * C + c] : 0.0f;
        v.x = gn_elem<GN == 2>(v.x, t, k); v.y = gn_elem<GN == 2>(v.y, t, k);
        v.z = gn_elem<GN == 2>(v.z, t, k); v.w = gn_elem<GN == 2>(v.w, t, k);
      }
    }
    *reinterpret_cast<float4*>(R + ch * kChF + row * kRowF + 4 * c4) = v;
  }
  __syncthreads();
  const int wv = __builtin_amdgcn_readfirstlane(tid >> 6);
  const int HH = wv >> 1, wm = wv & 1;
  const int kc = lane >> 4, tx = lane & 7, ty = 2 * wm + ((lane >> 3) & 1);
  const int roff = kc * kChF + 4 * ty * kRowF + 4 * tx;
  float a[18];
  if (HH == 0) w2::W2_TRANSFORM<0, kRowF>(R + roff, a);
  else w2::W2_TRANSFORM<1, kRowF>(R + roff, a);
  float* o = V + (size_t)blockIdx.x * w2::kVF + wv * w2::kVWF;
#pragma unroll
  for (int j = 0; j < 4; ++j)
    *reinterpret_cast<float4*>(o + 256 * j + 4 * lane) = make_float4(a[4 * j], a[4 * j + 1], a[4 * j + 2], a[4 * j + 3]);
  *reinterpret_cast<float2*>(o + 1024 + 2 * lane) = make_float2(a[16], a[17]);
}

}

extern "C" int skp_wino2_weights(const float* w, int K, int C, int flip, float* U, void* stream) {
  SKP_CHECK_ARG(w && U, "null pointer");
  SKP_CHECK_ARG(K > 0 && C > 0, "non-positive shape");
  SKP_CHECK_ARG(K % w2::kNC == 0, "output channels must be a multiple of 32");
  const long long n = (long long)K * C;
  hipLaunchKernelGGL(wino2_weights_kernel, dim3((unsigned)((n + 255) / 256)), dim3(256), 0, as_stream(stream), w, K, C,
                     flip, U);
  SKP_LAUNCH_CHECK();
  return SKP_OK;
}

namespace {
int wino_nt_flag(long long out_bytes, int nsplit) {
  if (nsplit > 1) return 0;
  return out_bytes >= (256LL << 20) ? 128 : 0;
}
}

extern "C" int skp_conv3x3s2_wino2(const float* x, const float* U, const float* bias, float* y, int B, int C, int K,
                                   int H, int W, int nsplit, float* ws, void* stream) {
  SKP_CHECK_ARG(x && U && y, "null pointer");
  SKP_CHECK_ARG(B > 0 && C > 0 && K > 0 && H > 0 && W > 0, "non-positive shape");
  SKP_CHECK_ARG(C % w2::kCK == 0, "input channels must be a multiple of 4");
  SKP_CHECK_ARG(K % w2::kNC == 0, "output channels must be a multiple of 32");
  SKP_CHECK_ARG(H % 32 == 0 && W % 32 == 0, "H and W must be multiples of 32");
  SKP_CHECK_ARG(nsplit >= 1 && C % (w2::kCK * nsplit) == 0, "nsplit must divide C into multiples of 4");
  SKP_CHECK_ARG(nsplit == 1 || ws, "split-K needs a workspace of nsplit·B·K·(H/2)·(W/2) floats");
  SKP_CHECK_ARG(aligned16(x) && aligned16(U) && aligned16(y) && (!ws || aligned16(ws)), "tensors must be 16-byte aligned");
  SKP_CHECK_ARG((long long)B * C * H * W * 4 < 0x7fffffffLL, "input larger than 2 GiB (32-bit buffer offsets)");
  const int bw = W / 32, bpi = (H / 16) * bw;
  const long long nblk = (long long)B * bpi;
  const int nkb = K / w2::kNC;
  SKP_CHECK_ARG(nblk * nkb * nsplit <= 0x7fffffffLL, "grid too large");
  float* out = nsplit > 1 ? ws : y;
  hipStream_t st = as_stream(stream);
  const dim3 grid((unsigned)(nblk * nkb * nsplit));
  const int fl = SKP_WINO2_DEBUG | wino_nt_flag((long long)B * K * (H / 2) * (W / 2) * 4, nsplit);
  if (nsplit == 1 && bias)
    hipLaunchKernelGGL((wino2_kernel<5, 8, 4>), grid, dim3(4 * WAVE), 0, st, x, U, bias, nullptr, out, B, C, K, H, W,
                       bw, bpi, (int)nblk, nkb, 0, C / nsplit, fl, nullptr);
  else
    hipLaunchKernelGGL((wino2_kernel<4, 8, 4>), grid, dim3(4 * WAVE), 0, st, x, U, nullptr, nullptr, out, B, C, K, H,
                       W, bw, bpi, (int)nblk, nkb, 0, C / nsplit, fl, nullptr);
  SKP_LAUNCH_CHECK();
  if (nsplit > 1) return splitk_reduce(ws, nsplit, B, K, (H / 2) * (W / 2), bias, nullptr, y, st);
  return SKP_OK;
}

extern "C" int skp_conv3x3_wino2_gn(const float* x, const float* U, const float* bias, const float* residual, float* y,
                                    int B, int C, int K, int H, int W, int nsplit, float* ws, float* gn_part,
                                    void* stream) {
  SKP_CHECK_ARG(x && U && y, "null pointer");
  SKP_CHECK_ARG(!gn_part || (nsplit == 1 && H % 32 == 0 && W % 32 == 0 && (reinterpret_cast<uintptr_t>(gn_part) & 7) == 0),
                "gn_part: one split, H and W multiples of 32, 8-byte aligned");
  SKP_CHECK_ARG(B > 0 && C > 0 && K > 0 && H > 0 && W > 0, "non-positive shape");
  SKP_CHECK_ARG(C % w2::kCK == 0, "input channels must be a multiple of 4");
  SKP_CHECK_ARG(K % w2::kNC == 0, "output channels must be a multiple of 32");
  const bool g16 = H == 16 && W == 16;
  SKP_CHECK_ARG((H % 32 == 0 && W % 32 == 0) || (g16 && B % 4 == 0),
                "H and W must be multiples of 32, or 16×16 with B a multiple of 4");
  SKP_CHECK_ARG(nsplit >= 1 && C % (w2::kCK * nsplit) == 0, "nsplit must divide C into multiples of 4");
  SKP_CHECK_ARG(nsplit == 1 || ws, "split-K needs a workspace of nsplit·B·K·H·W floats");
  SKP_CHECK_ARG(aligned16(x) && aligned16(U) && aligned16(y) && (!residual || aligned16(residual)) &&
                    (!ws || aligned16(ws)),
                "tensors must be 16-byte aligned");
  SKP_CHECK_ARG((long long)B * C * H * W * 4 < 0x7fffffffLL, "input larger than 2 GiB (32-bit buffer offsets)");
  const int bw = W / 32, bpi = (H / 16) * bw;
  const long long nblk = g16 ? B / 2 : (long long)B * bpi;
  const int nkb = K / w2::kNC;
  SKP_CHECK_ARG(nblk * nkb * nsplit <= 0x7fffffffLL, "grid too large");
  const int dbg = SKP_WINO2_DEBUG;
  const int kb_major = 0;
  const int epi = nsplit > 1 ? 0 : (bias ? 1 : 0) | (residual ? 2 : 0);
  float* out = nsplit > 1 ? ws : y;
  hipStream_t st = as_stream(stream);
  const dim3 grid((unsigned)(nblk * nkb * nsplit));
  const int fl = dbg | wino_nt_flag((long long)B * K * H * W * 4, nsplit);
  float2* gnp = reinterpret_cast<float2*>(gn_part);
#define SKP_WG2(E)                                                                                            \
  if (g16)                                                                                                    \
    hipLaunchKernelGGL((wino2_kernel<E, 4, 4>), grid, dim3(4 * WAVE), 0, st, x, U, bias, residual, out, B, C, K,  \
                       H, W, bw, bpi, (int)nblk, nkb, kb_major, C / nsplit, fl, nullptr);                              \
  else                                                                                                        \
    hipLaunchKernelGGL((wino2_kernel<E, 8, 4>), grid, dim3(4 * WAVE), 0, st, x, U, bias, residual, out, B, C, K,  \
                       H, W, bw, bpi, (int)nblk, nkb, kb_major, C / nsplit, fl, gnp)
  switch (epi) {
    case 0: SKP_WG2(0); break;
    case 1: SKP_WG2(1); break;
    case 2: SKP_WG2(2); break;
    default: SKP_WG2(3); break;
  }
#undef SKP_WG2
  SKP_LAUNCH_CHECK();
  if (nsplit > 1) return splitk_reduce(ws, nsplit, B, K, H * W, bias, residual, y, st);
  return SKP_OK;
}

extern "C" int skp_conv3x3_wino2(const float* x, const float* U, const float* bias, const float* residual, float* y,
                                 int B, int C, int K, int H, int W, int nsplit, float* ws, void* stream) {
  return skp_conv3x3_wino2_gn(x, U, bias, residual, y, B, C, K, H, W, nsplit, ws, nullptr, stream);
}

namespace {
int vtransform_launch(const float* x, const float* stats, const float* gamma, const float* beta, const float* shift,
                      int G, int act, float* V, int B, int C, int H, int W, void* stream) {
  const int bw = W / 32, bpi = (H / 16) * bw;
  const long long nwg = (long long)B * bpi * (C / w2::kCK);
  if (nwg > 0x7fffffffLL) return -2;
  const dim3 grid((unsigned)nwg), block(4 * WAVE);
  hipStream_t st = as_stream(stream);
  if (!stats) hipLaunchKernelGGL(wino2_vtransform_kernel<0>, grid, block, 0, st, x, stats, gamma, beta, shift, G, V, C, H, W, bw, bpi);
  else if (!act) hipLaunchKernelGGL(wino2_vtransform_kernel<1>, grid, block, 0, st, x, stats, gamma, beta, shift, G, V, C, H, W, bw, bpi);
  else hipLaunchKernelGGL(wino2_vtransform_kernel<2>, grid, block, 0, st, x, stats, gamma, beta, shift, G, V, C, H, W, bw, bpi);
  return 0;
}
}

extern "C" int skp_wino2_vtransform(const float* x, float* V, int B, int C, int H, int W, void* stream) {
  SKP_CHECK_ARG(x && V, "null pointer");
  SKP_CHECK_ARG(B > 0 && C > 0 && H > 0 && W > 0, "non-positive shape");
  SKP_CHECK_ARG(C % w2::kCK == 0, "input channels must be a multiple of 4");
  SKP_CHECK_ARG(H % 32 == 0 && W % 32 == 0, "H and W must be multiples of 32");
  SKP_CHECK_ARG(aligned16(x) && aligned16(V), "tensors must be 16-byte aligned");
  SKP_CHECK_ARG(vtransform_launch(x, nullptr, nullptr, nullptr, nullptr, 0, 0, V, B, C, H, W, stream) == 0,
                "grid too large");
  SKP_LAUNCH_CHECK();
  return SKP_OK;
}

extern "C" int skp_wino2_vtransform_gn(const float* x, const float* stats, const float* gamma, const float* beta,
                                       const float* shift, int G, int act, float* V, int B, int C, int H, int W,
                                       void* stream) {
  SKP_CHECK_ARG(x && V && stats && gamma && beta, "null pointer");
  SKP_CHECK_ARG(B > 0 && C > 0 && H > 0 && W > 0, "non-positive shape");
  SKP_CHECK_ARG(C % w2::kCK == 0, "input channels must be a multiple of 4");
  SKP_CHECK_ARG(G > 0 && C % G == 0, "C must be divisible by G");
  SKP_CHECK_ARG(H % 32 == 0 && W % 32 == 0, "H and W must be multiples of 32");
  SKP_CHECK_ARG(aligned16(x) && aligned16(V), "tensors must be 16-byte aligned");
  SKP_CHECK_ARG(vtransform_launch(x, stats, gamma, beta, shift, G, act, V, B, C, H, W, stream) == 0, "grid too large");
  SKP_LAUNCH_CHECK();
  return SKP_OK;
}

extern "C" int skp_conv3x3_wino2_v_gn(const float* V, const float* U, const float* bias, const float* residual,
                                      float* y, int B, int C, int K, int H, int W, int nsplit, float* ws,
                                      float* gn_part, void* stream) {
  SKP_CHECK_ARG(V && U && y, "null pointer");
  SKP_CHECK_ARG(!gn_part || (nsplit == 1 && (reinterpret_cast<uintptr_t>(gn_part) & 7) == 0),
                "gn_part: one split, 8-byte aligned");
  SKP_CHECK_ARG(B > 0 && C > 0 && K > 0 && H > 0 && W > 0, "non-positive shape");
  SKP_CHECK_ARG(C % w2::kCK == 0, "input channels must be a multiple of 4");
  SKP_CHECK_ARG(K % w2::kNC == 0, "output channels must be a multiple of 32");
  SKP_CHECK_ARG(H % 32 == 0 && W % 32 == 0, "H and W must be multiples of 32");
  SKP_CHECK_ARG(nsplit >= 1 && C % (w2::kCK * nsplit) == 0, "nsplit must divide C into multiples of 4");
  SKP_CHECK_ARG(nsplit == 1 || ws, "split-K needs a workspace of nsplit·B·K·H·W floats");
  SKP_CHECK_ARG(aligned16(V) && aligned16(U) && aligned16(y) && (!residual || aligned16(residual)) &&
                    (!ws || aligned16(ws)),
                "tensors must be 16-byte aligned");
  const int bw = W / 32, bpi = (H / 16) * bw;
  const long long nblk = (long long)B * bpi;
  const int nkb = K / w2::kNC;
  SKP_CHECK_ARG(nblk * nkb * nsplit <= 0x7fffffffLL, "grid too large");
  const int kb_major = 0;
  const int epi = nsplit > 1 ? 0 : (bias ? 1 : 0) | (residual ? 2 : 0);
  float* out = nsplit > 1 ? ws : y;
  hipStream_t st = as_stream(stream);
  const dim3 grid((unsigned)(nblk * nkb * nsplit));
  const int fl = SKP_WINO2_DEBUG | wino_nt_flag((long long)B * K * H * W * 4, nsplit);
  float2* gnp = reinterpret_cast<float2*>(gn_part);
#define SKP_WV(E)                                                                                                  \
  hipLaunchKernelGGL((wino2v_kernel<E>), grid, dim3(4 * WAVE), 0, st, V, U, bias, residual, out, B, C, K, H, W, bw, \
                     bpi, (int)nblk, nkb, kb_major, C / nsplit, fl, gnp)
  switch (epi) {
    case 0: SKP_WV(0); break;
    case 1: SKP_WV(1); break;
    case 2: SKP_WV(2); break;
    default: SKP_WV(3); break;
  }
#undef SKP_WV
  SKP_LAUNCH_CHECK();
  if (nsplit > 1) return splitk_reduce(ws, nsplit, B, K, H * W, bias, residual, y, st);
  return SKP_OK;
}

extern "C" int skp_conv3x3_wino2_v(const float* V, const float* U, const float* bias, const float* residual, float* y,
                                   int B, int C, int K, int H, int W, int nsplit, float* ws, void* stream) {
  return skp_conv3x3_wino2_v_gn(V, U, bias, residual, y, B, C, K, H, W, nsplit, ws, nullptr, stream);
}
```

stablekeypoints_amd/ops.py:

```python
import ctypes
import os

import torch

from . import _lib
from ._lib import call, ptr, stream

F32 = torch.float32

_TIMER = None


def set_kernel_timer(timer):
    global _TIMER
    _TIMER = timer


class _NoTimer:
    def __enter__(self):
        return self

    def __exit__(self, *a):
        return False


def _timed(name, nbytes=0, flops=0, cycles=0):
    return _TIMER.record(name, nbytes, flops, cycles) if _TIMER is not None else _NoTimer()


def _c(t, dtype=F32):
    return t.contiguous() if t.dtype == dtype else t.to(dtype).contiguous()


def _c16(t):
    t = _c(t)
    return t if t.data_ptr() % 16 == 0 else t.clone()


def _rows16(t):
    if (t.dtype == F32 and t.stride(-1) == 1 and t.stride(-2) % 4 == 0 and t.data_ptr() % 16 == 0
            and (t.dim() < 3 or t.shape[0] == 1 or t.stride(0) % 4 == 0)):
        return t
    return _c16(t)


def bgemm(a, b, alpha=1.0, out=None, accumulate=False):
    _lib.require_device(a, b)
    Z, M, K = a.shape
    Z2, K2, N = b.shape
    assert Z == Z2 and K == K2, (a.shape, b.shape)
    if out is None:
        out = torch.empty(Z, M, N, device=a.device, dtype=F32)
    call("skp_bgemm_f32", ptr(a), a.stride(0), a.stride(1), a.stride(2), ptr(b), b.stride(0), b.stride(1),
         b.stride(2), ptr(out), out.stride(0), out.stride(1), out.stride(2), Z, M, N, K, float(alpha),
         int(accumulate), stream(a.device))
    return out


def bgemm_2b(a, sa, b, sb, out, so, batch, hb, M, N, K, alpha=1.0, accumulate=False):
    call("skp_bgemm_f32_2b", ptr(a), *sa, ptr(b), *sb, ptr(out), *so, int(batch), int(hb), int(M), int(N), int(K),
         float(alpha), int(accumulate), stream(a.device))
    return out


class CaptureLogitsHeads(torch.autograd.Function):

    @staticmethod
    def forward(ctx, qf, k1, H, scale):
        qf, k1 = _c16(qf), _rows16(k1)
        B, S, C = qf.shape
        N, d, rk = k1.shape[1], C // H, k1.stride(1)
        z = torch.empty(B * H, S, N, device=qf.device, dtype=F32)
        bgemm_2b(qf, (S * C, d, C, 1), k1, (0, d, 1, rk), z, (H * S * N, S * N, N, 1), B * H, H, S, N, d, scale)
        ctx.save_for_backward(qf, k1)
        ctx.meta = (H, float(scale))
        return z

    @staticmethod
    def backward(ctx, dz):
        qf, k1 = ctx.saved_tensors
        H, scale = ctx.meta
        B, S, C = qf.shape
        N, d, rk = k1.shape[1], C // H, k1.stride(1)
        dz = _c16(dz)
        dq = dk1 = None
        if ctx.needs_input_grad[0]:
            dq = torch.empty_like(qf)
            bgemm_2b(dz, (H * S * N, S * N, N, 1), k1, (0, d, rk, 1), dq, (S * C, d, C, 1), B * H, H, S, d, N, scale)
        if ctx.needs_input_grad[1]:
            dkb = torch.empty(B, N, C, device=qf.device, dtype=F32)
            bgemm_2b(dz, (H * S * N, S * N, 1, N), qf, (S * C, d, C, 1), dkb, (N * C, d, C, 1), B * H, H, N, d, S,
                     scale)
            dk1 = dkb.sum(dim=0, keepdim=True) if B > 1 else dkb
        return dq, dk1, None, None


class AttnPVHeads(torch.autograd.Function):

    @staticmethod
    def forward(ctx, P, v1, H):
        P, v1 = _c16(P), _rows16(v1)
        BH, S, N = P.shape
        B, C = BH // H, v1.shape[2]
        d, rv = C // H, v1.stride(1)
        out = torch.empty(B, S, C, device=P.device, dtype=F32)
        bgemm_2b(P, (H * S * N, S * N, N, 1), v1, (0, d, rv, 1), out, (S * C, d, C, 1), BH, H, S, d, N)
        ctx.save_for_backward(P, v1)
        ctx.H = H
        return out

    @staticmethod
    def backward(ctx, dout):
        P, v1 = ctx.saved_tensors
        H = ctx.H
        BH, S, N = P.shape
        B, C = BH // H, v1.shape[2]
        d, rv = C // H, v1.stride(1)
        dout = _c16(dout)
        dP = dv1 = None
        if ctx.needs_input_grad[0]:
            dP = torch.empty_like(P)
            bgemm_2b(dout, (S * C, d, C, 1), v1, (0, d, 1, rv), dP, (H * S * N, S * N, N, 1), BH, H, S, N, d)
        if ctx.needs_input_grad[1]:
            dvb = torch.empty(B, N, C, device=P.device, dtype=F32)
            bgemm_2b(P, (H * S * N, S * N, 1, N), dout, (S * C, d, C, 1), dvb, (N * C, d, C, 1), BH, H, N, d, S)
            dv1 = dvb.sum(dim=0, keepdim=True) if B > 1 else dvb
        return dP, dv1, None


def capture_logits_heads(qf, k1, heads, scale):
    _lib.require_device(qf, k1)
    return CaptureLogitsHeads.apply(qf, k1, int(heads), float(scale))


def attn_pv_heads(P, v1, heads):
    _lib.require_device(P, v1)
    return AttnPVHeads.apply(P, v1, int(heads))


def heads_eligible(qf, k1, heads):
    C = qf.shape[-1]
    return (qf.dtype == F32 and k1.dtype == F32 and qf.dim() == 3 and k1.dim() == 3 and k1.shape[0] == 1
            and C % heads == 0 and (C // heads) % 4 == 0 and k1.shape[1] % 4 == 0 and k1.shape[2] == C)


class CaptureLogits(torch.autograd.Function):

    @staticmethod
    def forward(ctx, q, k, scale):
        q, k = _c(q), _c(k)
        ctx.save_for_backward(q, k)
        ctx.scale = scale
        return bgemm(q, k.transpose(1, 2), scale)

    @staticmethod
    def backward(ctx, dz):
        q, k = ctx.saved_tensors
        dz = _c(dz)
        dq = dk = None
        if ctx.needs_input_grad[0]:
            dq = bgemm(dz, k, ctx.scale)
        if ctx.needs_input_grad[1]:
            dk = bgemm(dz.transpose(1, 2), q, ctx.scale)
        return dq, dk, None


def capture_logits(q, k, scale):
    return CaptureLogits.apply(q, k, float(scale))


class CaptureAttn(torch.autograd.Function):

    @staticmethod
    def forward(ctx, z, s, R):
        z = _c(z)
        BH, S, N = z.shape
        assert S == s * s
        attn = torch.empty(BH, R * R, N, device=z.device, dtype=F32)
        with _timed("skp_capture_fwd", (BH * R * R * N + BH * S * N) * 4):
            call("skp_capture_fwd", ptr(z), BH, s, N, R, ptr(attn), None, stream(z.device))
        ctx.save_for_backward(z)
        ctx.s, ctx.R = s, R
        return attn

    @staticmethod
    def backward(ctx, dattn):
        (z,) = ctx.saved_tensors
        return capture_bwd(z, ctx.s, ctx.R, dattn), None, None


def capture_bwd(z, s, R, dattn, gscale=1.0, group=1, strides=None, stats=None):
    BH, S, N = z.shape
    if dattn.dtype != F32:
        dattn = dattn.float()
    if strides is None:
        sb, sp, sn = dattn.stride()
        if dattn.shape[0] == 1 and BH > 1:
            sb = 0
    else:
        sb, sp, sn = strides
    ws = torch.empty(BH, R, s, N, device=z.device, dtype=F32)
    dz = torch.empty_like(z)
    with _timed("skp_capture_bwd", (BH * S * N * 2 + BH * R * s * N * 2) * 4):
        call("skp_capture_bwd", ptr(z), BH, s, N, R, ptr(dattn), int(group), sb, sp, sn, float(gscale),
             ptr(stats) if stats is not None else None, ptr(dz), ptr(ws), stream(z.device))
    return dz


def capture_attn(z, s, R):
    return CaptureAttn.apply(z, int(s), int(R))


class _Aggregate(torch.autograd.Function):
    @staticmethod
    def forward(ctx, indices, upsample_res, *layers):
        layers = [_c(t) for t in layers]
        BH, RR, N = layers[0].shape
        R = int(round(RR ** 0.5))
        for t in layers:
            if t.shape != layers[0].shape:
                raise ValueError("collect_maps: captured layers must share (BH, R*R, N); got "
                                 f"{[tuple(x.shape) for x in layers]}")
        arr = (ctypes.c_void_p * len(layers))(*[t.data_ptr() for t in layers])
        n_out = N if indices is None else int(indices.numel())
        out = torch.empty(n_out, R, R, device=layers[0].device, dtype=F32)
        idx = None if indices is None else indices.to(device=out.device, dtype=torch.int64).contiguous()
        with _timed("skp_aggregate", (len(layers) * BH * RR * N + n_out * RR) * 4):
            call("skp_aggregate", ctypes.cast(arr, ctypes.POINTER(ctypes.c_void_p)), len(layers), BH, RR, N,
                 ptr(idx), n_out, ptr(out), stream(out.device))
        ctx.meta = (BH, RR, N, R, len(layers))
        ctx.idx = idx
        ctx.upsample_res = upsample_res
        if upsample_res != -1 and upsample_res != R:
            up = torch.empty(n_out, upsample_res, upsample_res, device=out.device, dtype=F32)
            call("skp_resize_bilinear", ptr(out), n_out, R, upsample_res, ptr(up), stream(out.device))
            out = up
        return out

    @staticmethod
    def backward(ctx, dmap):
        BH, RR, N, R, L = ctx.meta
        dmap = _c(dmap)
        if ctx.upsample_res != -1 and ctx.upsample_res != R:
            g = torch.empty(dmap.shape[0], R, R, device=dmap.device, dtype=F32)
            call("skp_resize_bilinear_bwd", ptr(dmap), dmap.shape[0], R, ctx.upsample_res, ptr(g), stream(dmap.device))
            dmap = g
        dmap = dmap.reshape(-1, RR) / float(L * BH)
        if ctx.idx is not None:
            full = torch.zeros(N, RR, device=dmap.device, dtype=F32)
            full.index_add_(0, ctx.idx, dmap)
            dmap = full
        g = dmap.t().unsqueeze(0).expand(BH, RR, N)
        return (None, None) + tuple(g for _ in range(L))


def aggregate(layers, indices=None, upsample_res=-1):
    return _Aggregate.apply(indices, int(upsample_res), *layers)


FUSED_MAPS = True


def capture_maps_bytes(B, H, N, R, sizes):
    RR = R * R
    return 4 * (sum(B * H * s * s * N for s in sizes) + B * N * RR + len(sizes) * B * H * RR * 2)


def capture_maps_flops(B, H, N, R, sizes):
    return sum(B * H * N * (15 * R * R + 8 * R * s) for s in sizes)


_PK, _TR = 4.0 / 128, 8.0 / 64


def capture_maps_issue_cycles(B, H, N, R, sizes):
    per_px = 4 * _PK + 0.5 * 4.0 / 64 + _PK + _TR + _PK + _PK
    return sum(B * H * N * (per_px * R * R + 4 * _PK * R * s) for s in sizes)


def capture_maps_sel_bwd_issue_cycles(B, H, N, R, sizes):
    per_px = 4 * _PK + _PK + _TR + _PK + 4 * _PK
    return sum(B * H * N * (per_px * R * R + 8 * _PK * R * s) for s in sizes)


def capture_maps_bwd_flops(B, H, N, R, sizes):
    return sum(B * H * N * (24 * R * R + 16 * R * s) for s in sizes)


def capture_maps_bwd_bytes(B, H, N, R, sizes):
    RR = R * R
    return 4 * (3 * B * N * RR + sum(2 * B * H * s * s * N + 2 * B * H * RR + 2 * B * H * R * s * N for s in sizes))


class CaptureMaps(torch.autograd.Function):

    @staticmethod
    def forward(ctx, B, R, sizes, *zs):
        zs = [_c16(z) for z in zs]
        BH, _, N = zs[0].shape
        H = BH // B
        L = len(zs)
        dev = zs[0].device
        RR = R * R
        if FUSED_MAPS:
            out, stats = _capture_maps_run(zs, sizes, B, R)
        else:
            stats = [torch.empty(BH, RR, 2, device=dev, dtype=F32) for _ in range(L)]
            out = torch.empty(B, N, R, R, device=dev, dtype=F32)
            attn = [torch.empty(BH, RR, N, device=dev, dtype=F32) for _ in range(L)]
            for z, a, st, s in zip(zs, attn, stats, sizes):
                with _timed("skp_capture_fwd", (BH * RR * N + BH * s * s * N) * 4):
                    call("skp_capture_fwd", ptr(z), BH, s, N, R, ptr(a), ptr(st), stream(dev))
            for b in range(B):
                off = b * H * RR * N * 4
                arr = (ctypes.c_void_p * L)(*[a.data_ptr() + off for a in attn])
                with _timed("skp_aggregate", (L * H * RR * N + N * RR) * 4):
                    call("skp_aggregate", ctypes.cast(arr, ctypes.POINTER(ctypes.c_void_p)), L, H, RR, N, None, N,
                         ptr(out[b]), stream(dev))
            del attn
        ctx.save_for_backward(*zs, *stats)
        ctx.meta = (B, H, R, N, list(sizes))
        return out

    @staticmethod
    def backward(ctx, dmaps):
        saved = ctx.saved_tensors
        L = len(saved) // 2
        return (None, None, None) + tuple(CaptureMaps._dense_bwd(saved[:L], saved[L:], ctx.meta, dmaps))

    @staticmethod
    def _dense_bwd(zs, stats, meta, dmaps):
        B, H, R, N, sizes = meta
        dmaps = _c(dmaps)
        RR = R * R
        scale = 1.0 / float(len(zs) * H)
        L = len(zs)
        if FUSED_MAPS and N % 4 == 0:
            dzs = [torch.empty_like(z) for z in zs]
            ws = torch.empty(B * RR * N + B * H * R * max(sizes) * N, device=dmaps.device, dtype=F32)
            zp = (ctypes.c_void_p * L)(*[z.data_ptr() for z in zs])
            sp = (ctypes.c_int * L)(*[int(s) for s in sizes])
            stp = (ctypes.c_void_p * L)(*[st.data_ptr() for st in stats])
            dp = (ctypes.c_void_p * L)(*[d.data_ptr() for d in dzs])
            with _timed("skp_capture_maps_bwd", capture_maps_bwd_bytes(B, H, N, R, sizes),
                        capture_maps_bwd_flops(B, H, N, R, sizes)):
                call("skp_capture_maps_bwd", ctypes.cast(zp, ctypes.POINTER(ctypes.c_void_p)), sp, L, B, H, N, R,
                     ptr(dmaps), scale, ctypes.cast(stp, ctypes.POINTER(ctypes.c_void_p)),
                     ctypes.cast(dp, ctypes.POINTER(ctypes.c_void_p)), ptr(ws), stream(dmaps.device))
            del ws
        else:
            dzs = [capture_bwd(z, s, R, dmaps, gscale=scale, group=H, strides=(N * RR, 1, RR), stats=st)
                   for z, s, st in zip(zs, sizes, stats)]
        return dzs


def capture_maps(zs, sizes, B, R):
    return CaptureMaps.apply(int(B), int(R), tuple(int(s) for s in sizes), *zs)


SEL_BWD = True
SEL_MAXK = 32


def capture_maps_sel_bwd_bytes(B, H, N, R, sizes, K):
    RR = R * R
    BH = B * H
    return 4 * sum(2 * BH * s * s * N + 2 * BH * RR + 4 * BH * RR + 2 * BH * K * RR + B * K * RR for s in sizes)


def capture_maps_sel_bwd_flops(B, H, N, R, sizes):
    return sum(B * H * N * (20 * R * R + 16 * R * s) for s in sizes)


class CapturedMaps:

    def __init__(self, zs, sizes, B, R):
        self.zs = list(zs)
        self.after_backward = None
        self.sizes = tuple(int(s) for s in sizes)
        self.B, self.R = int(B), int(R)
        with torch.no_grad():
            self.maps, self.stats = _capture_maps_run([z.detach() for z in self.zs], self.sizes, self.B, self.R)
        BH, _, N = self.zs[0].shape
        self.H, self.N = BH // self.B, N

    def select(self, rows):
        if len(rows) != self.B:
            raise ValueError(f"select: {len(rows)} row lists for {self.B} images")
        counts = [0 if r is None else int(r.numel()) for r in rows]
        toks = [r.to(device=self.maps.device, dtype=torch.int64).reshape(-1) for r, c in zip(rows, counts) if c]
        tok = torch.cat(toks) if toks else torch.empty(0, dtype=torch.int64, device=self.maps.device)
        return _SelectMaps.apply(self, tok, tuple(counts), *self.zs)


def _capture_maps_run(zs, sizes, B, R):
    zs = [_c16(z) for z in zs]
    BH, _, N = zs[0].shape
    H = BH // B
    L = len(zs)
    dev = zs[0].device
    RR = R * R
    stats = [torch.empty(BH, RR, 2, device=dev, dtype=F32) for _ in range(L)]
    out = torch.empty(B, N, R, R, device=dev, dtype=F32)
    zp = (ctypes.c_void_p * L)(*[z.data_ptr() for z in zs])
    sp = (ctypes.c_int * L)(*[int(s) for s in sizes])
    stp = (ctypes.c_void_p * L)(*[st.data_ptr() for st in stats])
    with _timed("skp_capture_maps_fwd", capture_maps_bytes(B, H, N, R, sizes), capture_maps_flops(B, H, N, R, sizes),
                capture_maps_issue_cycles(B, H, N, R, sizes)):
        call("skp_capture_maps_fwd", ctypes.cast(zp, ctypes.POINTER(ctypes.c_void_p)), sp, L, B, H, N, R,
             ptr(out), ctypes.cast(stp, ctypes.POINTER(ctypes.c_void_p)), stream(dev))
    return out, stats


def capture_maps_bwd_sel(zs, sizes, B, R, tok_table, gsel, gscale, stats):
    zs = [_c16(z) for z in zs]
    BH, _, N = zs[0].shape
    H = BH // B
    L = len(zs)
    K = tok_table.shape[1]
    dev = zs[0].device
    sp = (ctypes.c_int * L)(*[int(s) for s in sizes])
    nws = _lib.lib().skp_capture_maps_bwd_sel_workspace(sp, L, B, H, N, R, K)
    if nws < 0:
        raise ValueError(f"capture_maps_bwd_sel: bad shape B={B} H={H} N={N} R={R} K={K} sizes={sizes}")
    ws = torch.empty(int(nws), device=dev, dtype=F32)
    dzs = [torch.empty_like(z) for z in zs]
    arr = lambda ts: ctypes.cast((ctypes.c_void_p * L)(*[t.data_ptr() for t in ts]),
                                 ctypes.POINTER(ctypes.c_void_p))
    tok_table = tok_table.to(device=dev, dtype=torch.int64).contiguous()
    gsel = _c(gsel)
    with _timed("skp_capture_maps_bwd_sel", capture_maps_sel_bwd_bytes(B, H, N, R, sizes, K),
                capture_maps_sel_bwd_flops(B, H, N, R, sizes), capture_maps_sel_bwd_issue_cycles(B, H, N, R, sizes)):
        call("skp_capture_maps_bwd_sel", arr(zs), sp, L, B, H, N, R, ptr(tok_table), K, ptr(gsel), float(gscale),
             arr(stats), arr(dzs), ptr(ws), stream(dev))
    return dzs


class _SelectMaps(torch.autograd.Function):

    @staticmethod
    def forward(ctx, cm, tok, counts, *zs):
        B, N, R = cm.B, cm.N, cm.R
        img = torch.cat([torch.full((c,), b, dtype=torch.int64, device=tok.device) for b, c in enumerate(counts) if c]) \
            if tok.numel() else tok
        out = cm.maps.view(B * N, R * R)[img * N + tok].view(-1, R, R)
        ctx.cm, ctx.counts = cm, counts
        ctx.save_for_backward(tok)
        return out

    @staticmethod
    def backward(ctx, g):
        cm, counts = ctx.cm, ctx.counts
        (tok,) = ctx.saved_tensors
        B, N, R, L = cm.B, cm.N, cm.R, len(cm.zs)
        RR = R * R
        K = max(max(counts), 1)
        g = _c(g).view(-1, RR)
        scale = 1.0 / float(L * cm.H)
        if SEL_BWD and N % 4 == 0 and K <= SEL_MAXK:
            tt = torch.full((B, K), -1, dtype=torch.int64, device=g.device)
            gs = torch.zeros(B, K, RR, dtype=F32, device=g.device)
            off = 0
            for b, c in enumerate(counts):
                if c:
                    tt[b, :c] = tok[off:off + c]
                    gs[b, :c] = g[off:off + c]
                    off += c
            dzs = capture_maps_bwd_sel(cm.zs, cm.sizes, B, R, tt, gs, scale, cm.stats)
        else:
            dense = torch.zeros(B * N, RR, dtype=F32, device=g.device)
            img = torch.cat([torch.full((c,), b, dtype=torch.int64, device=g.device) for b, c in enumerate(counts) if c])
            dense.index_add_(0, img * N + tok, g)
            dzs = CaptureMaps._dense_bwd([_c(z) for z in cm.zs], cm.stats, (B, cm.H, R, N, list(cm.sizes)),
                                         dense.view(B, N, R, R))
        cb, cm.after_backward = cm.after_backward, None
        if cb is not None:
            cb()
        return (None, None, None) + tuple(dzs)


class _Resize(torch.autograd.Function):
    @staticmethod
    def forward(ctx, x, Ro):
        x = _c(x)
        C, R, _ = x.shape
        out = torch.empty(C, Ro, Ro, device=x.device, dtype=F32)
        call("skp_resize_bilinear", ptr(x), C, R, Ro, ptr(out), stream(x.device))
        ctx.R = R
        return out

    @staticmethod
    def backward(ctx, g):
        g = _c(g)
        C, Ro, _ = g.shape
        gin = torch.empty(C, ctx.R, ctx.R, device=g.device, dtype=F32)
        call("skp_resize_bilinear_bwd", ptr(g), C, ctx.R, Ro, ptr(gin), stream(g.device))
        return gin, None


def resize_bilinear(x, Ro):
    _lib.require_device(x)
    return _Resize.apply(x, int(Ro))


def find_max_pixel(maps):
    _lib.require_device(maps)
    maps = _c(maps)
    T, h, w = maps.shape
    pos = torch.empty(T, 2, device=maps.device, dtype=F32)
    call("skp_argmax2d", ptr(maps), T, h, w, None, 0, ptr(pos), None, stream(maps.device))
    return pos


def argmax_index(maps):
    maps = _c(maps)
    T, h, w = maps.shape
    idx = torch.empty(T, device=maps.device, dtype=torch.int64)
    call("skp_argmax2d", ptr(maps), T, h, w, None, 0, None, ptr(idx), stream(maps.device))
    return idx


def _radius2(h):
    r = 0.05 * h
    return float(r ** 2)


def find_k_max_pixels(maps, num=3, return_masked=False):
    _lib.require_device(maps)
    maps = _c(maps)
    T, h, w = maps.shape
    pos = torch.empty(num, T, 2, device=maps.device, dtype=F32)
    masked = torch.empty_like(maps) if return_masked else None
    call("skp_k_max_pixels", ptr(maps), T, h, w, int(num), _radius2(h), ptr(pos), ptr(masked), stream(maps.device))
    return (pos, masked) if return_masked else pos


def mask_radius(maps, max_coords, radius):
    _lib.require_device(maps)
    maps = _c(maps)
    T, h, w = maps.shape
    out = torch.empty_like(maps)
    call("skp_mask_radius", ptr(maps), T, h, w, ptr(_c(max_coords)), float(radius) ** 2, ptr(out),
         stream(maps.device))
    return out


def pixel_from_weighted_avg(heatmaps, distance=5):
    _lib.require_device(heatmaps)
    T, h, w = heatmaps.shape
    work = heatmaps if (heatmaps.is_contiguous() and heatmaps.dtype == F32) else heatmaps.float().contiguous()
    pos = torch.empty(T, 2, device=heatmaps.device, dtype=F32)
    call("skp_weighted_avg", ptr(work), T, h, w, float(distance) if distance != -1 else -1.0, 1, ptr(pos),
         stream(heatmaps.device))
    if work is not heatmaps:
        heatmaps.copy_(work)
    return pos


def gaussian_circles(pos, size, sigma):
    _lib.require_device(pos)
    pos = _c(pos)
    if pos.dim() == 2:
        pos = pos.unsqueeze(0)
    num, T, _ = pos.shape
    out = torch.empty(T, size, size, device=pos.device, dtype=F32)
    call("skp_gaussian_target", ptr(pos), num, T, int(size), float(sigma), ptr(out), stream(pos.device))
    return out


def find_top_k_gaussian(maps, top_k, sigma=3, epsilon=1e-5, num_subjects=1, return_kl=False):
    _lib.require_device(maps)
    maps = _c(maps)
    T, h, w = maps.shape
    top_k = min(int(top_k), T)
    out = torch.empty(top_k, device=maps.device, dtype=torch.int64)
    kl = torch.empty(T, device=maps.device, dtype=torch.float64)
    call("skp_topk_gaussian", ptr(maps), T, h, w, int(top_k), float(sigma), float(epsilon), int(num_subjects),
         ptr(out), ptr(kl), ptr(kl), stream(maps.device))
    return (out, kl) if return_kl else out


def find_top_k_gaussian_batch(maps, top_k, sigma=3, epsilon=1e-5, num_subjects=1):
    _lib.require_device(maps)
    maps = _c(maps)
    nb, T, h, w = maps.shape
    top_k = min(int(top_k), T)
    out = torch.empty(nb, top_k, device=maps.device, dtype=torch.int64)
    kl = torch.empty(nb, T, device=maps.device, dtype=torch.float64)
    with _timed("skp_topk_gaussian_batch", maps.numel() * 4 + nb * T * 8):
        call("skp_topk_gaussian_batch", ptr(maps), nb, T, h, w, int(top_k), float(sigma), float(epsilon),
             int(num_subjects), ptr(out), ptr(kl), ptr(kl), stream(maps.device))
    return out


def furthest_point_sampling_batch(maps, top_k, candidates):
    _lib.require_device(maps)
    maps = _c(maps)
    nb, T, h, w = maps.shape
    cand = candidates.to(device=maps.device, dtype=torch.int64).contiguous()
    if cand.dim() != 2 or cand.shape[0] != nb:
        raise ValueError(f"candidates {tuple(cand.shape)} for {nb} images")
    out = torch.empty(nb, top_k, device=maps.device, dtype=torch.int64)
    n_out = torch.empty(nb, device=maps.device, dtype=torch.int32)
    ws = torch.empty(2 * cand.numel() + 2, device=maps.device, dtype=F32)
    call("skp_fps_batch", ptr(maps), nb, T, h, w, ptr(cand), cand.shape[1], int(top_k), ptr(out), ptr(n_out),
         ptr(ws), stream(maps.device))
    return out, n_out


def fps_from_keys_batch(keys, maps, n_cand, top_k):
    _lib.require_device(maps)
    maps = _c(maps)
    nb, T, h, w = maps.shape
    keys = keys.to(device=maps.device, dtype=torch.float64).contiguous()
    if tuple(keys.shape) != (nb, T):
        raise ValueError(f"keys {tuple(keys.shape)} for maps {tuple(maps.shape)}")
    n_cand = min(int(n_cand), T)
    dev = maps.device
    cand = torch.empty(nb, n_cand, device=dev, dtype=torch.int64)
    out = torch.empty(nb, top_k, device=dev, dtype=torch.int64)
    n_out = torch.empty(nb, device=dev, dtype=torch.int32)
    ws = torch.empty(2 * nb * n_cand + 2, device=dev, dtype=F32)
    call("skp_fps_keys_batch", ptr(keys), ptr(maps), nb, T, h, w, n_cand, int(top_k), ptr(cand), ptr(out), ptr(n_out),
         ptr(ws), stream(dev))
    return out, n_out, cand


def gaussian_fps_batch(maps, maps_t, n_cand, top_k, sigma=3, epsilon=1e-5, num_subjects=1):
    _lib.require_device(maps)
    maps = _c(maps)
    nb, T, h, w = maps.shape
    if tuple(maps_t.shape) != (nb, T, h, w):
        raise ValueError(f"maps_t {tuple(maps_t.shape)} for maps {tuple(maps.shape)}")
    kl = torch.empty(nb, T, device=maps.device, dtype=torch.float64)
    with _timed("skp_selection", maps.numel() * 4 + nb * T * 8 + nb * min(int(n_cand), T) * h * w * 4):
        with _timed("skp_topk_gaussian_batch", maps.numel() * 4 + nb * T * 8):
            call("skp_topk_gaussian_batch", ptr(maps), nb, T, h, w, 0, float(sigma), float(epsilon),
                 int(num_subjects), ptr(kl), ptr(kl), ptr(kl), stream(maps.device))
        return fps_from_keys_batch(kl, maps_t, n_cand, top_k)


def entropy_keys_batch(maps):
    _lib.require_device(maps)
    maps = _c(maps)
    nb, T, h, w = maps.shape
    ent = torch.empty(nb, T, device=maps.device, dtype=torch.float64)
    call("skp_entropy_sort", ptr(maps), nb * T, h, w, 0, ptr(ent), ptr(ent), ptr(ent), stream(maps.device))
    return ent


def entropy_sort_batch(maps, top_k):
    _lib.require_device(maps)
    maps = _c(maps)
    nb, T, h, w = maps.shape
    top_k = min(int(top_k), T)
    out = torch.empty(nb, top_k, device=maps.device, dtype=torch.int64)
    ent = torch.empty(nb, T, device=maps.device, dtype=torch.float64)
    call("skp_entropy_sort", ptr(maps), nb * T, h, w, 0, ptr(out), ptr(ent), ptr(ent), stream(maps.device))
    if top_k > 0:
        call("skp_topk_keys", ptr(ent), nb, T, int(top_k), ptr(out), stream(maps.device))
    return out


def entropy_sort(maps, top_k, return_entropy=False):
    _lib.require_device(maps)
    maps = _c(maps)
    T, h, w = maps.shape
    top_k = min(int(top_k), T)
    out = torch.empty(top_k, device=maps.device, dtype=torch.int64)
    ent = torch.empty(T, device=maps.device, dtype=torch.float64)
    call("skp_entropy_sort", ptr(maps), T, h, w, int(top_k), ptr(out), ptr(ent), ptr(ent), stream(maps.device))
    return (out, ent) if return_entropy else out


def furthest_point_sampling(maps, top_k, candidates):
    _lib.require_device(maps)
    maps = _c(maps)
    T, h, w = maps.shape
    cand = candidates.to(device=maps.device, dtype=torch.int64).contiguous()
    out = torch.empty(top_k, device=maps.device, dtype=torch.int64)
    n_out = torch.empty(1, device=maps.device, dtype=torch.int32)
    ws = torch.empty(2 * cand.numel() + 2, device=maps.device, dtype=F32)
    call("skp_fps", ptr(maps), T, h, w, ptr(cand), cand.numel(), int(top_k), ptr(out), ptr(n_out), ptr(ws),
         stream(maps.device))
    return out, n_out


class SharpeningLoss(torch.autograd.Function):
    @staticmethod
    def forward(ctx, A, sigma, num_subjects):
        A = _c(A)
        T, h, w = A.shape
        pos = torch.empty(num_subjects, T, 2, device=A.device, dtype=F32)
        part = torch.empty(T, device=A.device, dtype=torch.float64)
        loss = torch.empty((), device=A.device, dtype=F32)
        call("skp_sharpen_fwd", ptr(A), T, h, w, float(sigma), int(num_subjects), ptr(pos), ptr(part), ptr(loss),
             stream(A.device))
        ctx.save_for_backward(A, pos)
        ctx.sigma, ctx.num = sigma, num_subjects
        return loss

    @staticmethod
    def backward(ctx, g):
        A, pos = ctx.saved_tensors
        T, h, w = A.shape
        dA = torch.empty_like(A)
        call("skp_sharpen_bwd", ptr(A), T, h, w, float(ctx.sigma), int(ctx.num), ptr(pos), ptr(_c(g.reshape(1))),
             ptr(dA), stream(A.device))
        return dA, None, None


def sharpening_loss(A, sigma=1.0, num_subjects=1):
    _lib.require_device(A)
    return SharpeningLoss.apply(A, float(sigma), int(num_subjects))


class SharpeningLossBatch(torch.autograd.Function):

    @staticmethod
    def forward(ctx, A, nb, sigma, num_subjects):
        A = _c(A)
        R, h, w = A.shape
        T = R // nb
        pos = torch.empty(num_subjects, R, 2, device=A.device, dtype=F32)
        part = torch.empty(R, device=A.device, dtype=torch.float64)
        loss = torch.empty(nb, device=A.device, dtype=F32)
        call("skp_sharpen_fwd_batch", ptr(A), nb, T, h, w, float(sigma), int(num_subjects), ptr(pos), ptr(part),
             ptr(loss), stream(A.device))
        ctx.save_for_backward(A, pos)
        ctx.meta = (nb, T, sigma, num_subjects)
        return loss

    @staticmethod
    def backward(ctx, g):
        A, pos = ctx.saved_tensors
        nb, T, sigma, num = ctx.meta
        _, h, w = A.shape
        dA = torch.empty_like(A)
        call("skp_sharpen_bwd_batch", ptr(A), nb, T, h, w, float(sigma), int(num), ptr(pos), ptr(_c(g.reshape(nb))),
             ptr(dA), stream(A.device))
        return dA, None, None, None


def sharpening_loss_batch(A, nb, sigma=1.0, num_subjects=1):
    _lib.require_device(A)
    if A.shape[0] % nb:
        raise ValueError(f"{A.shape[0]} rows for {nb} images")
    return SharpeningLossBatch.apply(A, int(nb), float(sigma), int(num_subjects))


class AffineWarp(torch.autograd.Function):
    @staticmethod
    def forward(ctx, x, theta):
        x = _c(x)
        B, C, H, W = x.shape
        th = _c(theta.to(x.device))
        out = torch.empty_like(x)
        call("skp_affine_warp", ptr(x), B, C, H, W, ptr(th), ptr(out), stream(x.device))
        ctx.save_for_backward(th)
        ctx.shape = (B, C, H, W)
        return out

    @staticmethod
    def backward(ctx, g):
        (th,) = ctx.saved_tensors
        B, C, H, W = ctx.shape
        gin = torch.empty(B, C, H, W, device=g.device, dtype=F32)
        call("skp_affine_warp_bwd", ptr(_c(g)), B, C, H, W, ptr(th), ptr(gin), stream(g.device))
        return gin, None


def affine_warp(x, theta):
    _lib.require_device(x)
    return AffineWarp.apply(x, theta)


class EquivarianceLoss(torch.autograd.Function):
    @staticmethod
    def forward(ctx, A, At, theta_inv):
        A, At = _c(A), _c(At)
        T, h, w = A.shape
        th = _c(theta_inv.to(A.device)).reshape(6)
        part = torch.empty(T, device=A.device, dtype=torch.float64)
        loss = torch.empty((), device=A.device, dtype=F32)
        call("skp_equiv_fwd", ptr(A), ptr(At), T, h, w, ptr(th), ptr(part), ptr(loss), stream(A.device))
        ctx.save_for_backward(A, At, th)
        return loss

    @staticmethod
    def backward(ctx, g):
        A, At, th = ctx.saved_tensors
        T, h, w = A.shape
        dA = torch.empty_like(A) if ctx.needs_input_grad[0] else None
        dAt = torch.empty_like(At)
        call("skp_equiv_bwd", ptr(A), ptr(At), T, h, w, ptr(th), ptr(_c(g.reshape(1))), ptr(dA), ptr(dAt),
             stream(A.device))
        return dA, (dAt if ctx.needs_input_grad[1] else None), None


def equivariance_loss_single(A, At, theta_inv):
    _lib.require_device(A, At)
    return EquivarianceLoss.apply(A, At, theta_inv)


class EquivarianceLossBatch(torch.autograd.Function):

    @staticmethod
    def forward(ctx, A, At, theta_inv, nb):
        A, At = _c(A), _c(At)
        R, h, w = A.shape
        T = R // nb
        th = _c(theta_inv.to(A.device)).reshape(nb * 6)
        part = torch.empty(R, device=A.device, dtype=torch.float64)
        loss = torch.empty(nb, device=A.device, dtype=F32)
        call("skp_equiv_fwd_batch", ptr(A), ptr(At), nb, T, h, w, ptr(th), ptr(part), ptr(loss), stream(A.device))
        ctx.save_for_backward(A, At, th)
        ctx.meta = (nb, T)
        return loss

    @staticmethod
    def backward(ctx, g):
        A, At, th = ctx.saved_tensors
        nb, T = ctx.meta
        _, h, w = A.shape
        dA = torch.empty_like(A) if ctx.needs_input_grad[0] else None
        dAt = torch.empty_like(At)
        call("skp_equiv_bwd_batch", ptr(A), ptr(At), nb, T, h, w, ptr(th), ptr(_c(g.reshape(nb))), ptr(dA), ptr(dAt),
             stream(A.device))
        return dA, (dAt if ctx.needs_input_grad[1] else None), None, None


def equivariance_loss_batch(A, At, theta_inv, nb):
    _lib.require_device(A, At)
    if A.shape[0] % nb or theta_inv.numel() != 6 * nb:
        raise ValueError(f"{A.shape[0]} rows / theta_inv {tuple(theta_inv.shape)} for {nb} images")
    return EquivarianceLossBatch.apply(A, At, theta_inv, int(nb))


GN_EPI = True


def _gn_parts_of(x):
    ent = getattr(x, "_skp_gn", None)
    if ent is None or ent[0] != x._version:
        return None
    return ent[1], ent[2]


def _gn_fwd(x, gamma, beta, shift, groups, eps, act):
    B, C = x.shape[:2]
    HW = x[0, 0].numel()
    nws = _lib.lib().skp_groupnorm_workspace(B, C, HW, groups)
    if nws < 0:
        raise ValueError(f"groupnorm: bad shape {tuple(x.shape)} groups={groups}")
    part = torch.empty(nws, device=x.device, dtype=torch.float64)
    stats = torch.empty(B * groups * 2, device=x.device, dtype=F32)
    y = torch.empty_like(x)
    g, b = _c(gamma.detach()), _c(beta.detach())
    pre = _gn_parts_of(x) if GN_EPI else None
    if pre is not None:
        call("skp_groupnorm_fwd_part", ptr(x), ptr(g), ptr(b), ptr(shift), ptr(pre[0]), pre[1], B, C, HW,
             int(groups), float(eps), int(act), ptr(y), ptr(stats), ptr(part), stream(x.device))
    else:
        call("skp_groupnorm_fwd", ptr(x), ptr(g), ptr(b), ptr(shift), B, C, HW, int(groups), float(eps), int(act),
             ptr(y), ptr(stats), ptr(part), stream(x.device))
    return y, stats, g, b, nws


class GroupNormAct(torch.autograd.Function):

    @staticmethod
    def forward(ctx, x, gamma, beta, groups, eps, act, shift):
        x = _c(x)
        B, C = x.shape[:2]
        HW = x[0, 0].numel()
        if shift is not None:
            shift = _c(shift.detach().expand(B, C))
        y, stats, g, b, nws = _gn_fwd(x, gamma, beta, shift, groups, eps, act)
        ctx.save_for_backward(x, g, b, stats, shift)
        ctx.meta = (B, C, HW, int(groups), int(act), nws)
        return y

    @staticmethod
    def backward(ctx, dy):
        x, g, b, stats, shift = ctx.saved_tensors
        B, C, HW, G, act, nws = ctx.meta
        dy = _c(dy)
        dx = torch.empty_like(x)
        part = torch.empty(nws, device=x.device, dtype=torch.float64)
        call("skp_groupnorm_bwd", ptr(x), ptr(dy), ptr(g), ptr(b), ptr(shift), ptr(stats), B, C, HW, G, act, ptr(dx),
             ptr(part), stream(x.device))
        return dx, None, None, None, None, None, None


class GroupNormActRes(torch.autograd.Function):

    @staticmethod
    def forward(ctx, x, gamma, beta, groups, eps, act, shift):
        xc = _c(x)
        B, C = xc.shape[:2]
        HW = xc[0, 0].numel()
        if shift is not None:
            shift = _c(shift.detach().expand(B, C))
        y, stats, g, b, nws = _gn_fwd(xc, gamma, beta, shift, groups, eps, act)
        ctx.save_for_backward(xc, g, b, stats, shift)
        ctx.meta = (B, C, HW, int(groups), int(act), nws)
        return y, x.view_as(x)

    @staticmethod
    def backward(ctx, dy, dpass):
        x, g, b, stats, shift = ctx.saved_tensors
        B, C, HW, G, act, nws = ctx.meta
        dy = _c(dy)
        dres = None if dpass is None else _c16(dpass)
        dx = torch.empty_like(x)
        part = torch.empty(nws, device=x.device, dtype=torch.float64)
        call("skp_groupnorm_bwd_add", ptr(x), ptr(dy), ptr(g), ptr(b), ptr(shift), ptr(stats), B, C, HW, G, act,
             ptr(dres), ptr(dx), ptr(part), stream(x.device))
        return dx, None, None, None, None, None, None


def group_norm_act_res(x, gamma, beta, groups, eps, act):
    _lib.require_device(x)
    return GroupNormActRes.apply(x, gamma, beta, int(groups), float(eps), bool(act), None)


def group_norm_act(x, gamma, beta, groups, eps, act, shift=None):
    _lib.require_device(x)
    if shift is not None:
        shift = shift.reshape(-1, x.shape[1]).to(x.device, F32)
    return GroupNormAct.apply(x, gamma, beta, int(groups), float(eps), bool(act), shift)


class ResidualBiasAdd(torch.autograd.Function):

    @staticmethod
    def forward(ctx, a, h, bias):
        a, h = _c(a), _c(h)
        B, C = a.shape[:2]
        out = torch.empty_like(a)
        call("skp_residual_bias_add", ptr(a), ptr(h), ptr(_c(bias.detach())), B, C, a[0, 0].numel(), ptr(out),
             stream(a.device))
        return out

    @staticmethod
    def backward(ctx, g):
        return g, g, None


def residual_bias_add(a, h, bias):
    _lib.require_device(a, h)
    if a.shape != h.shape:
        raise ValueError(f"residual_bias_add: shapes {tuple(a.shape)} and {tuple(h.shape)} differ")
    return ResidualBiasAdd.apply(a, h, bias)


def softmax_(s):
    if s.dtype != F32 or not s.is_contiguous() or s.shape[-1] % 4 or s.shape[-1] > 16384 or \
            s.data_ptr() % 16:
        return s.copy_(s.softmax(dim=-1))
    call("skp_softmax_fwd", ptr(s), s.numel() // s.shape[-1], s.shape[-1], stream(s.device))
    return s


def attention_probs(q, k, scale):
    sim = torch.baddbmm(torch.empty(q.shape[0], q.shape[1], k.shape[1], dtype=q.dtype, device=q.device),
                        q, k.transpose(1, 2), beta=0, alpha=scale)
    return softmax_(sim)


def attention_nograd(q, k, v, scale):
    BH, S, d = q.shape
    L = k.shape[1]
    if (q.dtype == F32 and S % 64 == 0 and d in (40, 64, 80) and q.is_contiguous()
            and k.is_contiguous() and v.is_contiguous()):
        out = torch.empty_like(q)
        call("skp_attn_fwd", ptr(q), ptr(k), ptr(v), ptr(out), None, BH, S, L, d, float(scale), stream(q.device))
        return out
    return torch.bmm(attention_probs(q, k, scale), v)


ATTN_FUSED_KV = (40,)


class MathAttention(torch.autograd.Function):

    @staticmethod
    def forward(ctx, q, k, v, scale):
        p = attention_probs(q, k, scale)
        out = torch.bmm(p, v)
        ctx.save_for_backward(q, k, v, p, out)
        ctx.scale = scale
        return out

    @staticmethod
    def backward(ctx, dout):
        q, k, v, p, out = ctx.saved_tensors
        dout = dout.contiguous()
        BH, S, L = p.shape
        d = q.shape[2]
        if (d in ATTN_FUSED_KV and S % 64 == 0 and L % 64 == 0 and ctx.needs_input_grad[1]
                and all(t.is_contiguous() and t.data_ptr() % 16 == 0 for t in (q, v, dout))):
            D = (dout * out).sum(-1)
            ds, dv, dk = torch.empty_like(p), torch.empty_like(v), torch.empty_like(k)
            call("skp_attn_bwd_kv", ptr(p), ptr(dout), ptr(q), ptr(v), ptr(D), ptr(ds), ptr(dv), ptr(dk),
                 BH, S, L, d, float(ctx.scale), stream(p.device))
            dq = torch.bmm(ds, k) if ctx.needs_input_grad[0] else None
            return dq, dk, dv if ctx.needs_input_grad[2] else None, None
        dv = torch.bmm(p.transpose(1, 2), dout) if ctx.needs_input_grad[2] else None
        dq = dk = None
        if ctx.needs_input_grad[0] or ctx.needs_input_grad[1]:
            if S % 64 == 0 and L % 64 == 0 and d in (40, 64, 80, 160) and v.is_contiguous():
                D = (dout * out).sum(-1)
                ds = torch.empty_like(p)
                call("skp_attn_dscore", ptr(p), ptr(dout), ptr(v), ptr(D), ptr(ds), BH, S, L, d,
                     float(ctx.scale), stream(p.device))
            else:
                ds = torch.bmm(dout, v.transpose(1, 2))
                call("skp_softmax_bwd", ptr(p), ptr(ds), p.shape[0] * p.shape[1], p.shape[2], float(ctx.scale),
                     stream(p.device))
            dq = torch.bmm(ds, k) if ctx.needs_input_grad[0] else None
            dk = torch.bmm(ds.transpose(1, 2), q) if ctx.needs_input_grad[1] else None
        return dq, dk, dv, None


class LayerNormFn(torch.autograd.Function):

    @staticmethod
    def forward(ctx, x, weight, bias, eps):
        x = _c(x)
        C = x.shape[-1]
        rows = x.numel() // C
        y = torch.empty_like(x)
        stats = torch.empty(rows, 2, device=x.device, dtype=F32)
        w, b = _c(weight.detach()), _c(bias.detach())
        call("skp_layernorm_fwd", ptr(x), ptr(w), ptr(b), rows, C, float(eps), ptr(y), ptr(stats), stream(x.device))
        ctx.save_for_backward(x, w, stats)
        return y

    @staticmethod
    def backward(ctx, dy):
        x, w, stats = ctx.saved_tensors
        dy = _c(dy)
        C = x.shape[-1]
        dx = torch.empty_like(x)
        call("skp_layernorm_bwd", ptr(x), ptr(dy), ptr(w), ptr(stats), x.numel() // C, C, ptr(dx), stream(x.device))
        return dx, None, None, None


class LayerNormRes(torch.autograd.Function):

    @staticmethod
    def forward(ctx, x, weight, bias, eps):
        xc = _c(x)
        C = xc.shape[-1]
        rows = xc.numel() // C
        y = torch.empty_like(xc)
        stats = torch.empty(rows, 2, device=xc.device, dtype=F32)
        w, b = _c(weight.detach()), _c(bias.detach())
        call("skp_layernorm_fwd", ptr(xc), ptr(w), ptr(b), rows, C, float(eps), ptr(y), ptr(stats), stream(xc.device))
        ctx.save_for_backward(xc, w, stats)
        return y, x.view_as(x)

    @staticmethod
    def backward(ctx, dy, dpass):
        x, w, stats = ctx.saved_tensors
        dy = _c(dy)
        dres = None if dpass is None else _c16(dpass)
        C = x.shape[-1]
        dx = torch.empty_like(x)
        call("skp_layernorm_bwd_add", ptr(x), ptr(dy), ptr(w), ptr(stats), x.numel() // C, C, ptr(dres), ptr(dx),
             stream(x.device))
        return dx, None, None, None


def layer_norm_res(x, weight, bias, eps):
    _lib.require_device(x)
    C = x.shape[-1]
    if (x.dtype != F32 or C % 4 or C > 2048 or weight is None or bias is None or weight.requires_grad
            or bias.requires_grad or x.numel() == 0 or x.numel() // C < LN_MIN_ROWS):
        return torch.nn.functional.layer_norm(x, (C,), weight, bias, eps), x
    return LayerNormRes.apply(x, weight, bias, float(eps))


LN_MIN_ROWS = 2048


def layer_norm(x, weight, bias, eps):
    _lib.require_device(x)
    C = x.shape[-1]
    if (x.dtype != F32 or C % 4 or C > 2048 or weight is None or bias is None or weight.requires_grad
            or bias.requires_grad or x.numel() == 0 or x.numel() // C < LN_MIN_ROWS):
        return torch.nn.functional.layer_norm(x, (C,), weight, bias, eps)
    return LayerNormFn.apply(x, weight, bias, float(eps))


class Geglu(torch.autograd.Function):

    @staticmethod
    def forward(ctx, h):
        h = _c(h)
        I = h.shape[-1] // 2
        out = torch.empty(*h.shape[:-1], I, device=h.device, dtype=F32)
        call("skp_geglu_fwd", ptr(h), h.numel() // h.shape[-1], I, ptr(out), stream(h.device))
        ctx.save_for_backward(h)
        return out

    @staticmethod
    def backward(ctx, dout):
        (h,) = ctx.saved_tensors
        dout = _c(dout)
        dh = torch.empty_like(h)
        call("skp_geglu_bwd", ptr(h), ptr(dout), h.numel() // h.shape[-1], h.shape[-1] // 2, ptr(dh),
             stream(h.device))
        return dh


def geglu(h):
    _lib.require_device(h)
    if h.dtype != F32 or h.shape[-1] % 8:
        x, gate = h.chunk(2, dim=-1)
        return x * torch.nn.functional.gelu(gate)
    return Geglu.apply(h)


ATTN_FLASH = (40, 64)


class FlashAttention(torch.autograd.Function):

    @staticmethod
    def forward(ctx, q, k, v, scale):
        BH, S, d = q.shape
        L = k.shape[1]
        out = torch.empty_like(q)
        stats = torch.empty(BH, S, 2, device=q.device, dtype=F32)
        call("skp_attn_fwd", ptr(q), ptr(k), ptr(v), ptr(out), ptr(stats), BH, S, L, d, float(scale),
             stream(q.device))
        ctx.save_for_backward(q, k, v, out, stats)
        ctx.scale = scale
        return out

    @staticmethod
    def backward(ctx, dout):
        q, k, v, out, stats = ctx.saved_tensors
        dout = dout.contiguous()
        BH, S, d = q.shape
        L = k.shape[1]
        D = (dout * out).sum(-1)
        ds = torch.empty(BH, S, L, device=q.device, dtype=F32)
        dv, dk = torch.empty_like(v), torch.empty_like(k)
        call("skp_attn_bwd_flash", ptr(q), ptr(k), ptr(v), ptr(dout), ptr(stats), ptr(D), ptr(ds), ptr(dv), ptr(dk),
             BH, S, L, d, float(ctx.scale), stream(q.device))
        dq = torch.bmm(ds, k) if ctx.needs_input_grad[0] else None
        return dq, dk if ctx.needs_input_grad[1] else None, dv if ctx.needs_input_grad[2] else None, None


def math_attention(q, k, v, scale):
    _lib.require_device(q, k, v)
    BH, S, d = q.shape
    L = k.shape[1]
    if (d in ATTN_FLASH and S % 64 == 0 and q.dtype == F32
            and all(t.dtype == F32 and t.is_contiguous() and t.data_ptr() % 16 == 0 for t in (q, k, v))):
        return FlashAttention.apply(q, k, v, float(scale))
    return MathAttention.apply(q, k, v, float(scale))


ATTN_BSHD = True


def _lay(t):
    return int(t.stride(0)), int(t.stride(1))


def _bshd_ok(q, k, v, H):
    B, S, C = q.shape
    if not ATTN_BSHD or C % H or S % 64 or k.shape[-1] != C or v.shape[-1] != C:
        return False
    return all(t.is_cuda and t.dtype == F32 and t.dim() == 3 and t.stride(2) == 1 and t.stride(1) % 4 == 0
               and t.stride(0) % 4 == 0 and t.data_ptr() % 16 == 0 for t in (q, k, v))


class FlashAttentionBSHD(torch.autograd.Function):

    @staticmethod
    def forward(ctx, q, k, v, H, scale):
        B, S, C = q.shape
        L = k.shape[1]
        d = C // H
        out = torch.empty(B, S, C, device=q.device, dtype=F32)
        stats = torch.empty(B * H, S, 2, device=q.device, dtype=F32)
        call("skp_attn_fwd_bshd", ptr(q), *_lay(q), ptr(k), *_lay(k), ptr(v), *_lay(v), ptr(out), S * C, C, ptr(stats),
             B, H, S, L, d, float(scale), stream(q.device))
        ctx.save_for_backward(q, k, v, out, stats)
        ctx.H, ctx.scale = H, scale
        return out

    @staticmethod
    def backward(ctx, dout):
        q, k, v, out, stats = ctx.saved_tensors
        H, scale = ctx.H, ctx.scale
        dout = _c16(dout)
        B, S, C = q.shape
        L = k.shape[1]
        d = C // H
        D = (dout.view(B, S, H, d) * out.view(B, S, H, d)).sum(-1).transpose(1, 2).contiguous()
        ds = torch.empty(B * H, S, L, device=q.device, dtype=F32)
        dv = torch.empty(B, L, C, device=q.device, dtype=F32)
        dk = torch.empty(B, L, C, device=q.device, dtype=F32)
        call("skp_attn_bwd_flash_bshd", ptr(q), *_lay(q), ptr(k), *_lay(k), ptr(v), *_lay(v), ptr(dout), S * C, C,
             ptr(stats), ptr(D), ptr(ds), ptr(dv), L * C, C, ptr(dk), L * C, C, B, H, S, L, d, float(scale),
             stream(q.device))
        dq = None
        if ctx.needs_input_grad[0]:
            k4 = k.view(k.shape[0], L, H, d).transpose(1, 2).expand(B, H, L, d)
            dq = torch.matmul(ds.view(B, H, S, L), k4).transpose(1, 2).reshape(B, S, C)
        return (dq, dk if ctx.needs_input_grad[1] else None, dv if ctx.needs_input_grad[2] else None, None, None)


def attention_heads(q, k, v, H, scale):
    if not _bshd_ok(q, k, v, H):
        return None
    B, S, C = q.shape
    d = C // H
    if torch.is_grad_enabled() and (q.requires_grad or k.requires_grad or v.requires_grad):
        if d not in ATTN_FLASH or k.stride(0) != 0:
            return None
        return FlashAttentionBSHD.apply(q, k, v, int(H), float(scale))
    if d not in (40, 64, 80):
        return None
    out = torch.empty(B, S, C, device=q.device, dtype=F32)
    call("skp_attn_fwd_bshd", ptr(q), *_lay(q), ptr(k), *_lay(k), ptr(v), *_lay(v), ptr(out), S * C, C, None,
         B, H, S, k.shape[1], d, float(scale), stream(q.device))
    return out


_QKV_W = {}


def _qkv_weight(*ws):
    key = tuple(id(w) for w in ws)
    sig = tuple((w._version, w.data_ptr()) for w in ws)
    ent = _QKV_W.get(key)
    if ent is not None and ent[0] == sig and all(r() is w for r, w in zip(ent[1], ws)):
        return ent[2]
    w3 = torch.cat([w.detach() for w in ws], 0).contiguous()
    drop = lambda _r, key=key: _QKV_W.pop(key, None)
    _QKV_W[key] = (sig, tuple(_weakref.ref(w, drop) for w in ws), w3)
    return w3


class QKVProjection(torch.autograd.Function):

    @staticmethod
    def forward(ctx, x, w3, C):
        out = torch.matmul(x, w3.t())
        ctx.save_for_backward(w3)
        ctx.C = C
        ctx.x_shape = x.shape
        ctx.set_materialize_grads(False)
        return tuple(out[..., i * C:(i + 1) * C] for i in range(w3.shape[0] // C))

    @staticmethod
    def backward(ctx, *grads):
        (w3,) = ctx.saved_tensors
        C = ctx.C
        dx = None
        for i, g in enumerate(grads):
            if g is None:
                continue
            g2 = g.reshape(-1, C)
            wi = w3[i * C:(i + 1) * C]
            if dx is None:
                dx = torch.mm(g2, wi)
            else:
                dx.addmm_(g2, wi)
        if dx is None:
            return None, None, None
        return dx.view(ctx.x_shape), None, None


QKV_FUSED = True


def qkv_projection(x, *ws):
    _lib.require_device(x)
    return QKVProjection.apply(x, _qkv_weight(*ws), int(ws[0].shape[0]))


class TokensProjIn(torch.autograd.Function):

    @staticmethod
    def forward(ctx, x, w, bias):
        B, C, HW = x.shape
        h = torch.bmm(x.transpose(1, 2), w.t().expand(B, C, w.shape[0]))
        if bias is not None:
            h.add_(bias)
        ctx.save_for_backward(w)
        return h

    @staticmethod
    def backward(ctx, dh):
        (w,) = ctx.saved_tensors
        B = dh.shape[0]
        dx = torch.bmm(w.t().expand(B, w.shape[1], w.shape[0]), dh.transpose(1, 2))
        return dx, None, None


class TokensProjOut(torch.autograd.Function):

    @staticmethod
    def forward(ctx, h, w):
        B = h.shape[0]
        ctx.save_for_backward(w)
        return torch.bmm(w.expand(B, *w.shape), h.transpose(1, 2))

    @staticmethod
    def backward(ctx, dy):
        (w,) = ctx.saved_tensors
        B = dy.shape[0]
        return torch.bmm(dy.transpose(1, 2), w.expand(B, *w.shape)), None


def tokens_proj_in(x, weight, bias):
    B, C = x.shape[:2]
    return TokensProjIn.apply(x.reshape(B, C, -1), weight.detach().reshape(weight.shape[0], C),
                              None if bias is None else bias.detach())


def tokens_proj_out(h, weight, bias, residual):
    B, C = residual.shape[:2]
    y = TokensProjOut.apply(h, weight.detach().reshape(C, h.shape[-1]))
    return residual_bias_add(residual, y.view(residual.shape), bias)


import weakref as _weakref

_WINO_U = {}
WINO_MIN_WORKGROUPS = 128
WINO_KERNEL = "auto"
WINO_SPLIT = True
WINO_NSPLIT_FORCE = 0


def _wino_v2(H, W, B=None):
    if WINO_KERNEL == "v1":
        return False
    return (H % 32 == 0 and W % 32 == 0) or (H == 16 and W == 16 and B is not None and B % 4 == 0)


def _wino_u(weight, flip, v2=False):
    ent = _WINO_U.get(id(weight))
    if ent is None or ent[0]() is not weight:
        key = id(weight)
        ent = (_weakref.ref(weight, lambda _r, key=key: _WINO_U.pop(key, None)), {})
        _WINO_U[key] = ent
    per = ent[1]
    hit = per.get((flip, v2))
    if hit is not None and hit[0] == weight._version:
        return hit[1]
    w = _c(weight.detach())
    K, C = (w.shape[0], w.shape[1]) if not flip else (w.shape[1], w.shape[0])
    U = torch.empty(K * C * (40 if v2 else 36), device=w.device, dtype=F32)
    call("skp_wino2_weights" if v2 else "skp_wino_weights", ptr(w), K, C, int(flip), ptr(U), stream(w.device))
    per[(flip, v2)] = (weight._version, U)
    return U


def _wino_plan_uncached(B, C, K, H, W, force):
    v2 = _wino_v2(H, W, B)
    if v2:
        wgs = (B // 4 if H == 16 else B * (H // 32) * (W // 32)) * (K // 32)
    elif B * (H // 4) * (W // 4) <= 32 and K % 64 == 0:
        wgs = K // 64
    else:
        wgs = -(-(B * (H // 4) * (W // 4)) // 64) * (K // 32)
    out_bytes = B * K * H * W * 4
    half = v2

    def cost(s):
        if half:
            k = -(-2 * wgs * s // 256)
            st = C // s // 4
            return (k // 2) * st * 1.72e-6 + (k % 2) * st * 1.48e-6 + (s > 1) * (s + 1) * out_bytes / 2e12
        rounds = -(-wgs * s // 256)
        return rounds * ((C // s // 4) * 2.4e-6 + 5e-6) + (s > 1) * (s + 1) * out_bytes / 5e12

    nsplit = 1
    if WINO_SPLIT:
        cands = [s for s in range(1, 33) if C % (4 * s) == 0 and (s == 1 or C // s >= 32)]
        nsplit = min(cands, key=cost)
        if force and C % (4 * force) == 0:
            nsplit = force
    return v2, nsplit, wgs * nsplit


_WINO_PLANS = {}


def _wino_plan(B, C, K, H, W):
    force = int(WINO_NSPLIT_FORCE)
    key = (B, C, K, H, W, force, WINO_KERNEL, WINO_SPLIT)
    plan = _WINO_PLANS.get(key)
    if plan is None:
        plan = _WINO_PLANS[key] = _wino_plan_uncached(B, C, K, H, W, force)
    return plan


def wino_eligible(B, C, K, H, W, min_workgroups=None):
    if C % 4 or K % 32 or H % 4 or W % 4:
        return False
    wgs = _wino_plan(B, C, K, H, W)[2]
    return wgs >= (WINO_MIN_WORKGROUPS if min_workgroups is None else min_workgroups)


WINO_GEMM_MAX_HW = 1024
WINO_GEMM_MIN_CH = 256
_WINO_G = ((1.0, 0.0, 0.0), (1 / 3, 1 / 3, 1 / 3), (-1 / 3, 1 / 3, -1 / 3), (-16 / 15, -8 / 15, -4 / 15),
           (1 / 15, -2 / 15, 4 / 15), (0.0, 0.0, 1.0))


def _wino_gemm_ok(B, C, K, H, W):
    return (0 < H * W <= WINO_GEMM_MAX_HW and C >= WINO_GEMM_MIN_CH and K >= WINO_GEMM_MIN_CH
            and H % 4 == 0 and W % 4 == 0 and B * (H // 4) * (W // 4) <= 65535)


def _wino_u_gemm(weight, flip):
    ent = _WINO_U.get(id(weight))
    if ent is None or ent[0]() is not weight:
        key = id(weight)
        ent = (_weakref.ref(weight, lambda _r, key=key: _WINO_U.pop(key, None)), {})
        _WINO_U[key] = ent
    hit = ent[1].get((flip, "gemm"))
    if hit is not None and hit[0] == weight._version:
        return hit[1]
    w = weight.detach().double()
    g = w.flip(2, 3).transpose(0, 1) if flip else w
    G = torch.tensor(_WINO_G, dtype=torch.float64, device=w.device)
    U = torch.einsum("iu,kcuv,jv->ijck", G, g, G).reshape(36, g.shape[1], g.shape[0]).float().contiguous()
    ent[1][(flip, "gemm")] = (weight._version, U)
    return U




def _wino_gemm_conv(x, weight, flip, bias, residual, K, gn=False):
    B, C, H, W = x.shape
    T = B * (H // 4) * (W // 4)
    U = _wino_u_gemm(weight, flip)
    V = torch.empty(36, C, T, device=x.device, dtype=F32)
    call("skp_wino_in_transform", ptr(x), B, C, H, W, ptr(V), stream(x.device))
    y = torch.empty(B, K, H, W, device=x.device, dtype=F32)
    bp, rp = ptr(bias) if bias is not None else None, ptr(residual) if residual is not None else None
    M = torch.bmm(U.transpose(1, 2), V)
    P = (H // 4) * (W // 4)
    gnp = None
    if gn and GN_EPI and (P in (16, 32) or P % 64 == 0):
        nseg = P // min(P, 64)
        gnp = torch.empty(B, K, nseg, 2, device=x.device, dtype=F32)
    call("skp_wino_out_transform_kt", ptr(M), B, K, H, W, bp, rp, ptr(y), ptr(gnp), stream(x.device))
    if gnp is not None:
        y._skp_gn = (y._version, gnp, gnp.shape[2])
    return y


def _wino_conv(x, weight, flip, bias, residual, K, gn=False):
    B, C, H, W = x.shape
    if _wino_gemm_ok(B, C, K, H, W):
        return _wino_gemm_conv(x, weight, flip, bias, residual, K, gn)
    y = torch.empty(B, K, H, W, device=x.device, dtype=F32)
    per_img = C * H * W * 4
    bmax = max(1, (2 ** 31 - 1) // per_img)
    gnp = None
    if gn and GN_EPI and H % 32 == 0 and W % 32 == 0 and all(
            _wino_plan(min(B, b0 + bmax) - b0, C, K, H, W)[:2] == (True, 1) for b0 in range(0, B, bmax)):
        nseg = (H // 16) * (W // 32)
        gnp = torch.empty(B, K, nseg, 2, device=x.device, dtype=F32)
    for b0 in range(0, B, bmax):
        b1 = min(B, b0 + bmax)
        _wino_launch(x[b0:b1], weight, flip, bias, None if residual is None else residual[b0:b1], y[b0:b1], K,
                     None if gnp is None else gnp[b0:b1])
    if gnp is not None:
        y._skp_gn = (y._version, gnp, gnp.shape[2])
    return y


def _wino_launch(x, weight, flip, bias, residual, y, K, gnp=None):
    B, C, H, W = x.shape
    v2, nsplit, _ = _wino_plan(B, C, K, H, W)
    U = _wino_u(weight, flip, v2)
    ws = torch.empty(nsplit, B, K, H, W, device=x.device, dtype=F32) if nsplit > 1 else None
    name = "skp_conv3x3_wino2" if v2 else "skp_conv3x3_wino"
    args = (ptr(x), ptr(U), ptr(bias) if bias is not None else None,
            ptr(residual) if residual is not None else None, ptr(y), B, C, K, H, W, nsplit,
            ptr(ws) if ws is not None else None)
    with _timed(name, 0):
        if gnp is not None:
            call("skp_conv3x3_wino2_gn", *args, ptr(gnp), stream(x.device))
        else:
            call(name, *args, stream(x.device))


class Conv3x3(torch.autograd.Function):

    @staticmethod
    def forward(ctx, x, weight, bias, residual):
        x = _c(x)
        K = weight.shape[0]
        y = _wino_conv(x, weight, False, None if bias is None else _c(bias.detach()),
                       None if residual is None else _c(residual), K, gn=True)
        ctx.weight = weight
        ctx.xshape = x.shape
        ctx.has_res = residual is not None
        return y

    @staticmethod
    def backward(ctx, dy):
        w = ctx.weight
        B, C, H, W = ctx.xshape
        K = w.shape[0]
        dx = None
        if ctx.needs_input_grad[0]:
            dy = _c(dy)
            if wino_eligible(B, K, C, H, W):
                dx = _wino_conv(dy, w, True, None, None, C)
            else:
                dx = torch.nn.grad.conv2d_input(ctx.xshape, w.detach(), dy, padding=1)
        return dx, None, None, (dy if ctx.has_res else None)


class Conv1x1(torch.autograd.Function):

    @staticmethod
    def forward(ctx, x, w):
        B, C, H, W = x.shape
        K = w.shape[0]
        y = torch.bmm(w.expand(B, K, C), x.reshape(B, C, H * W))
        ctx.save_for_backward(w)
        ctx.shape = (B, C, H, W)
        return y.view(B, K, H, W)

    @staticmethod
    def backward(ctx, dy):
        (w,) = ctx.saved_tensors
        B, C, H, W = ctx.shape
        K = w.shape[0]
        dx = torch.bmm(w.t().expand(B, C, K), dy.reshape(B, K, H * W)) if ctx.needs_input_grad[0] else None
        return (None if dx is None else dx.view(B, C, H, W)), None


CONV1X1_GEMM = False


def conv1x1(x, weight):
    _lib.require_device(x)
    if weight.requires_grad:
        raise ValueError("conv1x1: the weight must be frozen (requires_grad=False)")
    if not CONV1X1_GEMM or x.dtype != F32:
        return torch.nn.functional.conv2d(x, weight)
    return Conv1x1.apply(_c(x), weight.detach().reshape(weight.shape[0], weight.shape[1]))


WINO_S2 = True
WINO_S2_MIN_PIXELS = 384 * 384


def conv3x3_s2_eligible(x, weight):
    B, C, H, W = x.shape
    K = weight.shape[0]
    return (WINO_S2 and x.is_cuda and x.dtype == F32 and tuple(weight.shape[1:]) == (C, 3, 3) and C % 4 == 0
            and K % 32 == 0 and H % 32 == 0 and W % 32 == 0 and H * W >= WINO_S2_MIN_PIXELS
            and not weight.requires_grad and not (torch.is_grad_enabled() and x.requires_grad))


def conv3x3_s2(x, weight, bias=None):
    _lib.require_device(x)
    if not conv3x3_s2_eligible(x, weight):
        raise ValueError(f"conv3x3_s2: unsupported x {tuple(x.shape)} / weight {tuple(weight.shape)}")
    x = _c16(x)
    B, C, H, W = x.shape
    K = weight.shape[0]
    y = torch.empty(B, K, H // 2, W // 2, device=x.device, dtype=F32)
    U = _wino_u(weight, False, True)
    b = None if bias is None else _c(bias.detach())
    bmax = max(1, (2 ** 31 - 1) // (C * H * W * 4))
    for b0 in range(0, B, bmax):
        b1 = min(B, b0 + bmax)
        _, nsplit, _ = _wino_plan(b1 - b0, C, K, H, W)
        ws = torch.empty(nsplit, b1 - b0, K, H // 2, W // 2, device=x.device, dtype=F32) if nsplit > 1 else None
        with _timed("skp_conv3x3s2_wino2", 0):
            call("skp_conv3x3s2_wino2", ptr(x[b0:b1]), ptr(U), ptr(b), ptr(y[b0:b1]), b1 - b0, C, K, H, W, nsplit,
                 ptr(ws), stream(x.device))
    return y


def conv3x3(x, weight, bias=None, residual=None):
    _lib.require_device(x)
    if weight.requires_grad:
        raise ValueError("conv3x3: the weight must be frozen (requires_grad=False)")
    B, C, H, W = x.shape
    K = weight.shape[0]
    if tuple(weight.shape[1:]) != (C, 3, 3):
        raise ValueError(f"conv3x3: weight {tuple(weight.shape)} does not fit input {tuple(x.shape)}")
    if residual is not None and tuple(residual.shape) != (B, K, H, W):
        raise ValueError(f"conv3x3: residual {tuple(residual.shape)} is not ({B}, {K}, {H}, {W})")
    if C % 4 and C < 16 and x.dtype == F32 and wino_eligible(B, C + 4 - C % 4, K, H, W):
        pad = 4 - C % 4
        xp = torch.nn.functional.pad(x, (0, 0, 0, 0, 0, pad))
        wp = torch.nn.functional.pad(weight.detach(), (0, 0, 0, 0, 0, pad))
        return Conv3x3.apply(xp, wp, bias, residual)
    if x.dtype != F32 or not wino_eligible(B, C, K, H, W):
        y = torch.nn.functional.conv2d(x, weight, bias, 1, 1)
        return y if residual is None else residual + y
    return Conv3x3.apply(x, weight, bias, residual)


WINO_V_SHAPES = {(512, 512, 64, 64), (256, 512, 128, 128), (512, 512, 128, 128), (128, 256, 256, 256),
                 (256, 256, 256, 256)}
WINO_V_MIN_BATCH = 4


def gn_conv3x3_wins(B, C, K, H, W):
    return ((C, K, H, W) in WINO_V_SHAPES and B >= WINO_V_MIN_BATCH and C % 4 == 0 and K % 32 == 0
            and H % 32 == 0 and W % 32 == 0 and WINO_KERNEL == "auto" and not _wino_gemm_ok(B, C, K, H, W))


def gn_conv3x3(x, gamma, beta, groups, eps, act, shift, weight, bias=None, residual=None):
    _lib.require_device(x)
    if torch.is_grad_enabled() and (x.requires_grad or (residual is not None and residual.requires_grad)):
        raise ValueError("gn_conv3x3: forward only (no gradient reaches the normalised activation)")
    if weight.requires_grad or gamma.requires_grad or beta.requires_grad:
        raise ValueError("gn_conv3x3: the parameters must be frozen")
    pre = _gn_parts_of(x) if GN_EPI else None
    x = _c16(x.detach())
    B, C, H, W = x.shape
    K = weight.shape[0]
    if tuple(weight.shape[1:]) != (C, 3, 3):
        raise ValueError(f"gn_conv3x3: weight {tuple(weight.shape)} does not fit input {tuple(x.shape)}")
    if residual is not None:
        if tuple(residual.shape) != (B, K, H, W):
            raise ValueError(f"gn_conv3x3: residual {tuple(residual.shape)} is not ({B}, {K}, {H}, {W})")
        residual = _c16(residual.detach())
    if shift is not None:
        shift = _c(shift.detach().reshape(-1, C).to(x.device, F32).expand(B, C))
    dev = x.device
    nws = _lib.lib().skp_groupnorm_workspace(B, C, H * W, int(groups))
    if nws < 0:
        raise ValueError(f"gn_conv3x3: bad shape {tuple(x.shape)} groups={groups}")
    part = torch.empty(nws, device=dev, dtype=torch.float64)
    stats = torch.empty(B * groups * 2, device=dev, dtype=F32)
    g, b = _c(gamma.detach()), _c(beta.detach())
    if pre is not None:
        call("skp_groupnorm_stats_part", ptr(pre[0]), pre[1], ptr(shift), B, C, H * W, int(groups), float(eps),
             ptr(stats), ptr(part), stream(dev))
    else:
        call("skp_groupnorm_stats", ptr(x), ptr(shift), B, C, H * W, int(groups), float(eps), ptr(stats), ptr(part),
             stream(dev))
    V = torch.empty(B * C * (H // 4) * (W // 4) * 36, device=dev, dtype=F32)
    with _timed("skp_wino2_vtransform_gn", 0):
        call("skp_wino2_vtransform_gn", ptr(x), ptr(stats), ptr(g), ptr(b), ptr(shift), int(groups), int(bool(act)),
             ptr(V), B, C, H, W, stream(dev))
    _, nsplit, _ = _wino_plan(B, C, K, H, W)
    U = _wino_u(weight, False, True)
    y = torch.empty(B, K, H, W, device=dev, dtype=F32)
    ws = torch.empty(nsplit, B, K, H, W, device=dev, dtype=F32) if nsplit > 1 else None
    gnp = torch.empty(B, K, (H // 16) * (W // 32), 2, device=dev, dtype=F32) if GN_EPI and nsplit == 1 else None
    bias = None if bias is None else _c(bias.detach())
    with _timed("skp_conv3x3_wino2_v", 0):
        call("skp_conv3x3_wino2_v_gn", ptr(V), ptr(U), ptr(bias), ptr(residual), ptr(y), B, C, K, H, W, nsplit,
             ptr(ws), ptr(gnp), stream(dev))
    if gnp is not None:
        y._skp_gn = (y._version, gnp, gnp.shape[2])
    return y


TAB10 = ((31, 119, 180), (255, 127, 14), (44, 160, 44), (214, 39, 40), (148, 103, 189), (140, 86, 75),
         (227, 119, 194), (127, 127, 127), (188, 189, 34), (23, 190, 207))
_VIRIDIS_ANCHORS = ((0, (0.267004, 0.004874, 0.329415)), (32, (0.278826, 0.175490, 0.483397)),
                    (64, (0.229739, 0.322361, 0.545706)), (96, (0.172719, 0.448791, 0.557885)),
                    (128, (0.127568, 0.566949, 0.550556)), (160, (0.157851, 0.683765, 0.501686)),
                    (192, (0.369214, 0.788888, 0.382914)), (224, (0.678489, 0.863742, 0.189503)),
                    (255, (0.993248, 0.906157, 0.143936)))
_LUT_CACHE = {}


def default_colors(K):
    if K <= 10:
        rows = TAB10[:K]
    else:
        import colorsys
        rows = [tuple(int(round(255 * c)) for c in colorsys.hsv_to_rgb(j / K, 0.9, 1.0)) for j in range(K)]
    return torch.tensor(rows, dtype=torch.uint8).reshape(K, 3)


def fallback_lut():
    lut = torch.empty(256, 3, dtype=F32)
    for (i0, c0), (i1, c1) in zip(_VIRIDIS_ANCHORS[:-1], _VIRIDIS_ANCHORS[1:]):
        t = torch.arange(i0, i1 + 1, dtype=torch.float64).sub(i0).div(i1 - i0)[:, None]
        lut[i0:i1 + 1] = (torch.tensor(c0, dtype=torch.float64) * (1 - t) + torch.tensor(c1, dtype=torch.float64) * t).float()
    return lut.clamp_(0.0, 1.0)


def default_lut():
    try:
        import matplotlib
        import numpy as np
        cm = matplotlib.colormaps["viridis"]
        return torch.tensor(np.asarray(cm(np.linspace(0.0, 1.0, 256)))[:, :3], dtype=F32).contiguous()
    except ImportError:
        return fallback_lut()


def map_range(maps):
    _lib.require_device(maps)
    maps = _c(maps)
    n, h, w = maps.shape
    out = torch.empty(n, 2, device=maps.device, dtype=F32)
    call("skp_map_range", ptr(maps), n, h, w, ptr(out), stream(maps.device))
    return out


def sheet_shape(H, W, rows, cols, downscale=1, pad=2):
    return rows * (H // downscale + pad) + pad, cols * (W // downscale + pad) + pad


def render_sheet(images, maps=None, points=None, *, rows, cols, downscale=1, pad=2, alpha=0.7, radius=None,
                 colors=None, lut=None, overlay=None):
    _lib.require_device(images, maps, points)
    images = _c(images)
    n, C, H, W = images.shape
    if C != 3:
        raise ValueError(f"render_sheet: images must be (n, 3, H, W), got {tuple(images.shape)}")
    dev = images.device
    f = int(downscale)
    h = w = 0
    rng = None
    if maps is not None:
        maps = _c(maps)
        if maps.dim() != 3 or maps.shape[0] != n:
            raise ValueError(f"render_sheet: maps must be ({n}, h, w), got {tuple(maps.shape)}")
        h, w = maps.shape[1:]
        rng = map_range(maps)
        if overlay is not None:
            keep = torch.as_tensor(overlay, dtype=torch.bool).to(dev)
            if keep.shape != (n,):
                raise ValueError(f"render_sheet: overlay must be ({n},), got {tuple(keep.shape)}")
            rng[~keep] = float("nan")
        if lut is None:
            if dev not in _LUT_CACHE:
                _LUT_CACHE[dev] = default_lut().to(dev)
            lut = _LUT_CACHE[dev]
        lut = _c(lut.to(dev))
        if tuple(lut.shape) != (256, 3):
            raise ValueError(f"render_sheet: lut must be (256, 3), got {tuple(lut.shape)}")
    K = 0
    if points is not None:
        points = _c(points)
        if points.dim() != 3 or points.shape[0] != n or points.shape[2] != 2:
            raise ValueError(f"render_sheet: points must be ({n}, K, 2), got {tuple(points.shape)}")
        K = points.shape[1]
    if K:
        colors = default_colors(K) if colors is None else torch.as_tensor(colors)
        if colors.dtype != torch.uint8 or tuple(colors.shape) != (K, 3):
            raise ValueError(f"render_sheet: colors must be ({K}, 3) uint8")
        colors = colors.to(dev).contiguous()
        if radius is None:
            radius = max(2.0, (H // max(f, 1)) / 32.0)
    else:
        points = colors = None
    Hs, Ws = sheet_shape(H, W, rows, cols, max(f, 1), pad)
    out = torch.empty(Hs, Ws, 3, device=dev, dtype=torch.uint8)
    call("skp_render_sheet", ptr(images), n, H, W, ptr(maps), h, w, ptr(rng), ptr(lut) if maps is not None else None,
         float(alpha), ptr(points), K, float(radius or 0.0), ptr(colors), int(rows), int(cols), f, int(pad), ptr(out),
         stream(dev))
    return out


_TTA_WS = {}


def tta_reduce_bytes(B, C, n, S, avg=False):
    return 4 * B * C * n * S * S + (4 * B * n * S * S if avg else 0)


def tta_reduce(maps, theta_inv, return_avg=False):
    _lib.require_device(maps, theta_inv)
    if maps.dim() != 5 or maps.shape[-1] != maps.shape[-2]:
        raise ValueError(f"tta_reduce: maps must be (B, C, n, S, S), got {tuple(maps.shape)}")
    maps = _c(maps)
    B, C, n, S, _ = maps.shape
    if tuple(theta_inv.shape) != (B, C, 2, 3):
        raise ValueError(f"tta_reduce: theta_inv must be ({B}, {C}, 2, 3), got {tuple(theta_inv.shape)}")
    dev = maps.device
    th = _c(theta_inv.to(dev))
    key = (dev, B, n, S)
    ws = _TTA_WS.get(key)
    if ws is None:
        nbytes = _lib.lib().skp_tta_reduce_workspace(B, n, S)
        if nbytes <= 0:
            raise ValueError(f"tta_reduce: bad shape B={B}, n={n}, S={S}")
        ws = _TTA_WS[key] = torch.empty((nbytes + 7) // 8, device=dev, dtype=torch.int64)
    pos = torch.empty(B, n, 2, device=dev, dtype=F32)
    avg = torch.empty(B, n, S, S, device=dev, dtype=F32) if return_avg else None
    with _timed("skp_tta_reduce", tta_reduce_bytes(B, C, n, S, return_avg)):
        call("skp_tta_reduce", ptr(maps), B, C, n, S, ptr(th), ptr(pos), ptr(avg), ptr(ws), stream(dev))
    return pos, avg
```

Measured before the change: 44.92.

## Add dedicated stride-2 Winograd transform with fewer MFMA products per tile

Replaces the stride-2 conv path, which ran the full stride-1 Winograd F(4x4,3x3)-style kernel and then subsampled the output, with a dedicated stride-2 transform: 5x5 input/weight transform (15 or 10 products per half instead of 18), its own weight packing (28 floats per channel pair) and a new compact epilogue. This removes the wasted work of computing outputs that were thrown away, and shrinks U staging in LDS. The eligibility threshold for the stride-2 path is also lowered from 384² to 128² pixels, so smaller VAE downsample layers use it too. Risks include the numerical behaviour of the new transform and the reworked epilogue's correctness.

```diff
diff --git a/include/skp.h b/include/skp.h
--- a/include/skp.h
+++ b/include/skp.h
@@ -168,8 +168,9 @@
                         int C, int K, int H, int W, int nsplit, float* ws, void* stream);
 int skp_conv3x3_wino2_v_gn(const float* V, const float* U, const float* bias, const float* residual, float* y, int B,
                            int C, int K, int H, int W, int nsplit, float* ws, float* gn_part, void* stream);
-int skp_conv3x3s2_wino2(const float* x, const float* U, const float* bias, float* y, int B, int C, int K, int H,
-                        int W, int nsplit, float* ws, void* stream);
+int skp_wino2s2_weights(const float* w, int K, int C, float* U, void* stream);
+int skp_conv3x3s2_f2(const float* x, const float* U, const float* bias, float* y, int B, int C, int K, int H, int W,
+                     int nsplit, float* ws, void* stream);
 
 int skp_map_range(const float* maps, int n, int h, int w, float* range, void* stream);
 int skp_render_sheet(const float* images, int n, int H, int W, const float* maps, int h, int w, const float* range,
diff --git a/stablekeypoints_amd/_lib.py b/stablekeypoints_amd/_lib.py
--- a/stablekeypoints_amd/_lib.py
+++ b/stablekeypoints_amd/_lib.py
@@ -88,7 +88,8 @@
     "skp_wino2_vtransform_gn": [_p, _p, _p, _p, _p, _c_int, _c_int, _p, _c_int, _c_int, _c_int, _c_int, _p],
     "skp_conv3x3_wino2_v": [_p, _p, _p, _p, _p, _c_int, _c_int, _c_int, _c_int, _c_int, _c_int, _p, _p],
     "skp_conv3x3_wino2_v_gn": [_p, _p, _p, _p, _p, _c_int, _c_int, _c_int, _c_int, _c_int, _c_int, _p, _p, _p],
-    "skp_conv3x3s2_wino2":[_p, _p, _p, _p, _c_int, _c_int, _c_int, _c_int, _c_int, _c_int, _p, _p],
+    "skp_wino2s2_weights": [_p, _c_int, _c_int, _p, _p],
+    "skp_conv3x3s2_f2":   [_p, _p, _p, _p, _c_int, _c_int, _c_int, _c_int, _c_int, _c_int, _p, _p],
     "skp_map_range": [_p, _c_int, _c_int, _c_int, _p, _p],
     "skp_render_sheet": [_p, _c_int, _c_int, _c_int, _p, _c_int, _c_int, _p, _p, _c_float, _p, _c_int, _c_float, _p,
                          _c_int, _c_int, _c_int, _c_int, _p, _p],
diff --git a/stablekeypoints_amd/csrc/skp_conv.hip b/stablekeypoints_amd/csrc/skp_conv.hip
--- a/stablekeypoints_amd/csrc/skp_conv.hip
+++ b/stablekeypoints_amd/csrc/skp_conv.hip
@@ -142,7 +142,7 @@
     kb = L - tb * nkb;
   }
   const int c0 = sp * csplit;
-  y += (size_t)sp * nimg * K * ((EPI & 4) ? (H / 2) * (W / 2) : H * W);
+  y += (size_t)sp * nimg * K * H * W;
 
   const int tid = threadIdx.x, lane = tid & 63;
   const int wv = __builtin_amdgcn_readfirstlane(tid >> 6);
@@ -442,8 +442,10 @@
 constexpr unsigned kOOB = 0x80000000u;
 constexpr int kVWF = 4 * 256 + 128;
 constexpr int kVF = 4 * kVWF;
+constexpr int kUP2 = 28;
+constexpr int kUF2 = kCK * kNC * kUP2;
 typedef unsigned int u32x2 __attribute__((ext_vector_type(2)));
-static_assert(kUF % 256 == 0, "whole 1-KB chunks");
+static_assert(kUF % 256 == 0 && kUF2 % 256 == 0, "whole 1-KB chunks");
 static_assert((4 * GeoT<8>::RAWF + 3 * kUF) * 4 <= 160 * 1024 && 3 * (GeoT<4>::RAWF + kUF) * 4 <= 160 * 1024, "LDS");
 static_assert(2 * 8 * 1024 <= kUF * 4, "epilogue exchange: two waves' 8 KB per ring buffer");
 
@@ -583,6 +585,52 @@
     }
 }
 
+template <int H, int RF>
+__device__ __forceinline__ void s2_transform(const float* raw, float* a) {
+  constexpr int NR = H ? 2 : 3;
+  float d[NR][5];
+#pragma unroll
+  for (int i = 0; i < NR; ++i) {
+    const float* rp = raw + (H ? 2 + 2 * i : 1 + 2 * i) * RF;
+    const float4 c1 = *reinterpret_cast<const float4*>(rp + 4);
+    const float4 c2 = *reinterpret_cast<const float4*>(rp + 8);
+    d[i][0] = c1.x;
+    d[i][1] = c1.y;
+    d[i][2] = c1.z;
+    d[i][3] = c1.w;
+    d[i][4] = c2.x;
+    asm volatile("" ::"v"(c2.y), "v"(c2.z), "v"(c2.w));
+  }
+#pragma unroll
+  for (int ii = 0; ii < NR; ++ii) {
+    float t[5];
+#pragma unroll
+    for (int b = 0; b < 5; ++b)
+      t[b] = H ? d[ii][b] : ii == 0 ? d[0][b] - d[1][b] : ii == 1 ? d[1][b] : d[1][b] - d[2][b];
+    a[5 * ii] = t[0] - t[2];
+    a[5 * ii + 1] = t[2];
+    a[5 * ii + 2] = t[2] - t[4];
+    a[5 * ii + 3] = t[1];
+    a[5 * ii + 4] = t[3];
+  }
+}
+
+template <int H>
+__device__ __forceinline__ void s2_output(const float* m, float* y) {
+  constexpr int NR = H ? 2 : 3;
+  float s[NR][2];
+#pragma unroll
+  for (int ii = 0; ii < NR; ++ii) {
+    s[ii][0] = (m[5 * ii] + m[5 * ii + 1]) + m[5 * ii + 3];
+    s[ii][1] = (m[5 * ii + 1] - m[5 * ii + 2]) + m[5 * ii + 4];
+  }
+#pragma unroll
+  for (int c = 0; c < 2; ++c) {
+    y[c] = H ? s[0][c] : s[0][c] + s[1][c];
+    y[2 + c] = H ? s[1][c] : s[1][c] - s[NR - 1][c];
+  }
+}
+
 }
 
 struct W2Smem {
@@ -615,7 +663,7 @@
 #define SKP_W2_RS4 0
 #endif
 
-template <int EPI, int HH, int TXB, int NW, bool VST = false>
+template <int EPI, int HH, int TXB, int NW, bool VST = false, bool S2 = false>
 __device__ __forceinline__ void wino2_body(const W2Smem& sm, const float* __restrict__ x, const float* __restrict__ U,
                                            const float* __restrict__ bias, const float* __restrict__ res,
                                            float* __restrict__ y, int C, int K, int H, int W, int img, int x0,
@@ -624,13 +672,14 @@
   using Geo = w2::GeoT<TXB, NW>;
   constexpr int kChF = Geo::CHF, kRowF = Geo::RF, kRawInstr = Geo::RAW_INSTR, NI = Geo::NI, RR = Geo::RR,
                 RC = Geo::RC;
-  constexpr int kInstr = kRawInstr + w2::kUInstr;
+  static_assert(!S2 || (TXB == 8 && NW == 4 && !VST && (EPI & ~1) == 0), "stride-2 form: half-height blocks, bias only");
+  constexpr int kUP = S2 ? w2::kUP2 : w2::kUP, kUF = S2 ? w2::kUF2 : w2::kUF, kUInstr = kUF / 256;
+  constexpr int NP = S2 ? (HH ? 10 : 15) : 18;
+  constexpr int kInstr = kRawInstr + kUInstr;
   constexpr int kMaxRaw = (kRawInstr + NW - 1) / NW;
-  constexpr int kMaxU = (w2::kUInstr + NW - 1) / NW + 1;
+  constexpr int kMaxU = (kUInstr + NW - 1) / NW + 1;
   constexpr int NT = NW * WAVE;
   constexpr int US = NW == 4 ? 2 : 3;
-  using w2::kUF;
-  using w2::kUP;
   static_assert(!VST || (TXB == 8 && NW == 4), "V-staged form: half-height blocks of 4 waves");
   constexpr int RS = (VST || (TXB == 4 && NW == 4)) ? 2 : (TXB == 8 && NW == 8 && SKP_W2_RS4) ? 4 : 3;
   float *R0 = sm.R0, *R1 = sm.R1, *R2 = sm.R2, *U0 = sm.U0, *U1 = sm.U1, *U2 = sm.U2;
@@ -690,34 +739,41 @@
   const int tx = lane & (TXB - 1);
   const int ty = TXB == 8 ? 2 * wm + ((lane >> 3) & 1) : (lane >> 2) & 3;
   const int roff = kc * kChF + (TXB == 8 ? 0 : wm * RR * kRowF) + 4 * ty * kRowF + 4 * tx;
-  const int uoff = (kc * w2::kNC + (lane & 15)) * kUP + 20 * HH;
-
-  f32x4 acc[2][18];
+  const int uoff = (kc * w2::kNC + (lane & 15)) * kUP + (S2 ? 16 : 20) * HH;
+
+  f32x4 acc[2][NP];
 #pragma unroll
   for (int b = 0; b < 2; ++b)
 #pragma unroll
-    for (int q = 0; q < 18; ++q) acc[b][q] = f32x4{0.f, 0.f, 0.f, 0.f};
-  float a0[18], a1[18];
-
-  auto mfmas = [&](const float* us, const float (&acur)[18]) {
+    for (int q = 0; q < NP; ++q) acc[b][q] = f32x4{0.f, 0.f, 0.f, 0.f};
+  float a0[NP], a1[NP];
+
+  auto mfmas = [&](const float* us, const float (&acur)[NP]) {
+    constexpr int N4 = (NP + 1) / 4;
 #pragma unroll
     for (int b = 0; b < 2; ++b) {
       const float* ub = us + uoff + b * 16 * kUP;
-      float u[18];
-#pragma unroll
-      for (int j = 0; j < 4; ++j) {
+      float u[4 * N4 + 2];
+#pragma unroll
+      for (int j = 0; j < N4; ++j) {
         const float4 v = *reinterpret_cast<const float4*>(ub + 4 * j);
         u[4 * j] = v.x;
         u[4 * j + 1] = v.y;
         u[4 * j + 2] = v.z;
         u[4 * j + 3] = v.w;
       }
-      const float2 v2 = *reinterpret_cast<const float2*>(ub + 16);
-      u[16] = v2.x;
-      u[17] = v2.y;
-#pragma unroll
-      for (int q = 0; q < 18; ++q) acc[b][q] = __builtin_amdgcn_mfma_f32_16x16x4f32(acur[q], u[q], acc[b][q], 0, 0, 0);
-    }
+      if constexpr (NP % 4 == 2) {
+        const float2 v2 = *reinterpret_cast<const float2*>(ub + 4 * N4);
+        u[4 * N4] = v2.x;
+        u[4 * N4 + 1] = v2.y;
+      }
+#pragma unroll
+      for (int q = 0; q < NP; ++q) acc[b][q] = __builtin_amdgcn_mfma_f32_16x16x4f32(acur[q], u[q], acc[b][q], 0, 0, 0);
+    }
+  };
+  auto transform = [&](const float* raw, float (&an)[NP]) {
+    if constexpr (S2) w2::s2_transform<HH, kRowF>(raw + roff, an);
+    else w2::W2_TRANSFORM<HH, kRowF>(raw + roff, an);
   };
 
   if constexpr (VST) {
@@ -792,20 +848,20 @@
     issue_raw(RS - 1, RS == 4 ? sm.R3 : RS == 3 ? R2 : R1);
     w2_vmcnt(nst > 1 ? allow_pro : 0);
     __syncthreads();
-    w2::W2_TRANSFORM<HH, kRowF>(R0 + roff, a0);
-
-    auto step = [&](int s, float* Rn, float* Us, float* Ri, float* Ui, const float (&acur)[18], float (&anext)[18]) {
+    transform(R0, a0);
+
+    auto step = [&](int s, float* Rn, float* Us, float* Ri, float* Ui, const float (&acur)[NP], float (&anext)[NP]) {
       w2_vmcnt(s + 1 < nst ? allow_step : 0);
       __syncthreads();
       if (s + US - 1 < nst) issue_u(s + US - 1, Ui);
       issue_raw(s + RS, Ri);
       const bool tr = s + 1 < nst && !(dbg & 1);
       if (HH == 0) {
-        if (tr) w2::W2_TRANSFORM<HH, kRowF>(Rn + roff, anext);
+        if (tr) transform(Rn, anext);
         if (!(dbg & 2)) mfmas(Us, acur);
       } else {
         if (!(dbg & 2)) mfmas(Us, acur);
-        if (tr) w2::W2_TRANSFORM<HH, kRowF>(Rn + roff, anext);
+        if (tr) transform(Rn, anext);
       }
     };
     constexpr int PER = RS == 4 ? 12 : RS == 2 ? 2 : 6;
@@ -827,145 +883,177 @@
   W2_VMCNT(0);
   __syncthreads();
   if (dbg & 32) return;
-  constexpr int PH = (TXB == 8 && NW == 4) ? 16 : 32;
-  constexpr int PLS = (TXB == 8 ? PH * 32 : NI * 256) + 4;
-  float* const P2 = RS == 2 ? U1 : R2;
-  auto plane_of = [&](int c) -> float* {
-    float* b = (c >> 2) == 0 ? R0 : (c >> 2) == 1 ? R1 : (c >> 2) == 2 ? P2 : U0;
-    return b + (c & 3) * PLS + (c >> 2) * 16;
-  };
-  float* pl = plane_of(lane & 15);
-  const int pbase = TXB == 8 ? (4 * (2 * wm + (lane >> 5))) * 32 + 4 * (4 * ((lane >> 4) & 1))
-                             : wm * 256 + (4 * (lane >> 4)) * 16;
-  constexpr int PW = TXB == 8 ? 32 : 16;
-#pragma unroll
-  for (int blk = 0; blk < 2; ++blk) {
-    if (HH != blk) {
+  if constexpr (S2) {
+    constexpr int PLS2 = 8 * 16 + 4;
+    static_assert(16 * PLS2 <= Geo::RAWF, "stride-2 exchange planes fit one raw slot");
+    const int Ho = H / 2, Wo = W / 2;
+    float* pl = R0 + (lane & 15) * PLS2 + 2 * (2 * wm + (lane >> 5)) * 16 + 8 * ((lane >> 4) & 1);
+#pragma unroll
+    for (int blk = 0; blk < 2; ++blk) {
+      float o[4][4];
 #pragma unroll
       for (int r = 0; r < 4; ++r) {
-        float m[18], o[16];
-#pragma unroll
-        for (int q = 0; q < 18; ++q) m[q] = acc[blk][q][r];
-        w2::half_output<HH>(m, o);
-#pragma unroll
-        for (int f = 0; f < 4; ++f)
-          *reinterpret_cast<float4*>(pl + pbase + f * PW + 4 * r) =
-              make_float4(o[4 * f], o[4 * f + 1], o[4 * f + 2], o[4 * f + 3]);
-      }
-    }
-    __syncthreads();
-    if (HH == blk) {
-#pragma unroll
-      for (int r = 0; r < 4; ++r) {
-        float m[18], o[16];
-#pragma unroll
-        for (int q = 0; q < 18; ++q) m[q] = acc[blk][q][r];
-        w2::half_output<HH>(m, o);
-#pragma unroll
-        for (int f = 0; f < 4; ++f) {
-          float4* d = reinterpret_cast<float4*>(pl + pbase + f * PW + 4 * r);
-          const float4 p = *d;
-          *d = make_float4(o[4 * f] + p.x, o[4 * f + 1] + p.y, o[4 * f + 2] + p.z, o[4 * f + 3] + p.w);
-        }
-      }
-    }
-    __syncthreads();
-    if constexpr ((EPI & 4) != 0) {
-      static_assert(TXB == 8 && (EPI & 2) == 0, "stride-2 output: 32-wide blocks, no residual");
-      const int Ho = H / 2, Wo = W / 2;
-      constexpr int PC2 = (PH / 2) * 4;
-#pragma unroll
-      for (int i = 0; i < 16 * PC2 / NT; ++i) {
+        float m[NP];
+#pragma unroll
+        for (int q = 0; q < NP; ++q) m[q] = acc[blk][q][r];
+        w2::s2_output<HH>(m, o[r]);
+      }
+      if (HH != blk) {
+#pragma unroll
+        for (int f = 0; f < 2; ++f)
+#pragma unroll
+          for (int h = 0; h < 2; ++h)
+            *reinterpret_cast<float4*>(pl + f * 16 + 4 * h) =
+                make_float4(o[2 * h][2 * f], o[2 * h][2 * f + 1], o[2 * h + 1][2 * f], o[2 * h + 1][2 * f + 1]);
+      }
+      __syncthreads();
+      if (HH == blk) {
+#pragma unroll
+        for (int f = 0; f < 2; ++f)
+#pragma unroll
+          for (int h = 0; h < 2; ++h) {
+            float4* d = reinterpret_cast<float4*>(pl + f * 16 + 4 * h);
+            const float4 p = *d;
+            *d = make_float4(o[2 * h][2 * f] + p.x, o[2 * h][2 * f + 1] + p.y, o[2 * h + 1][2 * f] + p.z,
+                             o[2 * h + 1][2 * f + 1] + p.w);
+          }
+      }
+      __syncthreads();
+#pragma unroll
+      for (int i = 0; i < 16 * 32 / NT; ++i) {
         const int idx = i * NT + tid;
-        const int c = idx / PC2, q = idx % PC2;
-        const int row = q >> 2, c4 = q & 3;
-        const float* pp = plane_of(c) + (2 * row + 1) * 32 + 8 * c4 + 1;
+        const int c = idx >> 5, row = (idx >> 2) & 7, c4 = idx & 3;
+        const float4 p = *reinterpret_cast<const float4*>(R0 + c * PLS2 + row * 16 + 4 * c4);
         const int k = kb * w2::kNC + 16 * blk + c;
         const float bv = (EPI & 1) ? bias[k] : 0.0f;
-        const size_t o = (((size_t)img * K + k) * Ho + y0 / 2 + row) * Wo + x0 / 2 + 4 * c4;
-        const float4 v = make_float4(pp[0] + bv, pp[2] + bv, pp[4] + bv, pp[6] + bv);
+        const size_t o4 = (((size_t)img * K + k) * Ho + y0 / 2 + row) * Wo + x0 / 2 + 4 * c4;
+        const float4 v = make_float4(p.x + bv, p.y + bv, p.z + bv, p.w + bv);
+        if (dbg & 128) __builtin_nontemporal_store(f32x4{v.x, v.y, v.z, v.w}, reinterpret_cast<f32x4*>(y + o4));
+        else if (!(dbg & 64)) *reinterpret_cast<float4*>(y + o4) = v;
+      }
+      if (blk == 0) __syncthreads();
+    }
+  } else {
+    constexpr int PH = (TXB == 8 && NW == 4) ? 16 : 32;
+    constexpr int PLS = (TXB == 8 ? PH * 32 : NI * 256) + 4;
+    float* const P2 = RS == 2 ? U1 : R2;
+    auto plane_of = [&](int c) -> float* {
+      float* b = (c >> 2) == 0 ? R0 : (c >> 2) == 1 ? R1 : (c >> 2) == 2 ? P2 : U0;
+      return b + (c & 3) * PLS + (c >> 2) * 16;
+    };
+    float* pl = plane_of(lane & 15);
+    const int pbase = TXB == 8 ? (4 * (2 * wm + (lane >> 5))) * 32 + 4 * (4 * ((lane >> 4) & 1))
+                               : wm * 256 + (4 * (lane >> 4)) * 16;
+    constexpr int PW = TXB == 8 ? 32 : 16;
+#pragma unroll
+    for (int blk = 0; blk < 2; ++blk) {
+      if (HH != blk) {
+#pragma unroll
+        for (int r = 0; r < 4; ++r) {
+          float m[18], o[16];
+#pragma unroll
+          for (int q = 0; q < 18; ++q) m[q] = acc[blk][q][r];
+          w2::half_output<HH>(m, o);
+#pragma unroll
+          for (int f = 0; f < 4; ++f)
+            *reinterpret_cast<float4*>(pl + pbase + f * PW + 4 * r) =
+                make_float4(o[4 * f], o[4 * f + 1], o[4 * f + 2], o[4 * f + 3]);
+        }
+      }
+      __syncthreads();
+      if (HH == blk) {
+#pragma unroll
+        for (int r = 0; r < 4; ++r) {
+          float m[18], o[16];
+#pragma unroll
+          for (int q = 0; q < 18; ++q) m[q] = acc[blk][q][r];
+          w2::half_output<HH>(m, o);
+#pragma unroll
+          for (int f = 0; f < 4; ++f) {
+            float4* d = reinterpret_cast<float4*>(pl + pbase + f * PW + 4 * r);
+            const float4 p = *d;
+            *d = make_float4(o[4 * f] + p.x, o[4 * f + 1] + p.y, o[4 * f + 2] + p.z, o[4 * f + 3] + p.w);
+          }
+        }
+      }
+      __syncthreads();
+      constexpr int PCF = TXB == 8 ? PH * 8 : NI * 64;
+      constexpr int NIT = 16 * PCF / NT;
+      static_assert(TXB != 8 || NIT == 8, "TXB 8: eight wave instructions per wave");
+      float g1[4] = {0.f, 0.f, 0.f, 0.f}, g2[4] = {0.f, 0.f, 0.f, 0.f}, piv[4] = {0.f, 0.f, 0.f, 0.f};
+#pragma unroll
+      for (int i = 0; i < NIT; ++i) {
+        const int idx = TXB == 8 ? (((tid >> 6) * NIT + i) << 6) + (tid & 63) : i * NT + tid;
+        const int c = idx / PCF, q = idx % PCF;
+        const float4 v0 = *reinterpret_cast<const float4*>(plane_of(c) + 4 * q);
+        const int k = kb * w2::kNC + 16 * blk + c;
+        const float bv = (EPI & 1) ? bias[k] : 0.0f;
+        size_t o;
+        if (TXB == 8) {
+          const int row = q >> 3, c4 = q & 7;
+          o = (((size_t)img * K + k) * H + y0 + row) * W + x0 + 4 * c4;
+        } else {
+          o = ((size_t)(img + (q >> 6)) * K + k) * 256 + 4 * (q & 63);
+        }
+        float4 v = make_float4(v0.x + bv, v0.y + bv, v0.z + bv, v0.w + bv);
+        if (EPI & 2) {
+          const float4 rv = *reinterpret_cast<const float4*>(res + o);
+          v.x += rv.x;
+          v.y += rv.y;
+          v.z += rv.z;
+          v.w += rv.w;
+        }
         if (dbg & 128) __builtin_nontemporal_store(f32x4{v.x, v.y, v.z, v.w}, reinterpret_cast<f32x4*>(y + o));
         else if (!(dbg & 64)) *reinterpret_cast<float4*>(y + o) = v;
+        if (TXB == 8 && gnp) {
+          if ((i & 1) == 0) piv[i >> 1] = __builtin_bit_cast(float, __builtin_amdgcn_readfirstlane(__builtin_bit_cast(int, v.x)));
+          const float p = piv[i >> 1];
+          const float dx = v.x - p, dy = v.y - p, dz = v.z - p, dw = v.w - p;
+          g1[i >> 1] += (dx + dy) + (dz + dw);
+          g2[i >> 1] += (dx * dx + dy * dy) + (dz * dz + dw * dw);
+        }
+      }
+      if (TXB == 8 && gnp) {
+        float a[4] = {g1[0], g2[0], g1[1], g2[1]}, b[4] = {g1[2], g2[2], g1[3], g2[3]};
+        float u[4];
+#pragma unroll
+        for (int j = 0; j < 4; ++j) {
+          asm volatile("s_nop 1\n\tv_permlane32_swap_b32 %0, %1" : "+v"(a[j]), "+v"(b[j]));
+          u[j] = a[j] + b[j];
+        }
+        float w[2];
+#pragma unroll
+        for (int j = 0; j < 2; ++j) {
+          float x0 = u[j], x1 = u[j + 2];
+          asm volatile("s_nop 1\n\tv_permlane16_swap_b32 %0, %1" : "+v"(x0), "+v"(x1));
+          w[j] = x0 + x1;
+        }
+        const int lane = tid & 63;
+        const bool hi = (lane & 8) != 0;
+        const float keep = hi ? w[1] : w[0], send = hi ? w[0] : w[1];
+        float x = keep + dpp_read<0x140>(send);
+        x += dpp_read<0x141>(x);
+        x += dpp_read<0x4E>(x);
+        x += dpp_read<0xB1>(x);
+        const float x2 = __shfl_xor(x, 8, 64);
+        if ((lane & 15) == 0) {
+          const int r = lane >> 4;
+          const int J = (tid >> 6) * NIT + 2 * r;
+          const int c = (J << 6) / PCF, piece = ((J << 6) % PCF) >> 6;
+          const int k = kb * w2::kNC + 16 * blk + c;
+          const int seg = ((y0 + 8 * piece) >> 4) * (W >> 5) + (x0 >> 5);
+          const float p = r == 0 ? piv[0] : r == 1 ? piv[1] : r == 2 ? piv[2] : piv[3];
+          constexpr float inv_n = 1.0f / 512.0f;
+          gnp[((size_t)img * K + k) * (size_t)((H >> 4) * (W >> 5)) + seg] =
+              make_float2(p + x * inv_n, fmaxf(x2 - x * (x * inv_n), 0.0f));
+        }
       }
       if (blk == 0) __syncthreads();
-      continue;
-    }
-    constexpr int PCF = TXB == 8 ? PH * 8 : NI * 64;
-    constexpr int NIT = 16 * PCF / NT;
-    static_assert(TXB != 8 || NIT == 8, "TXB 8: eight wave instructions per wave");
-    float g1[4] = {0.f, 0.f, 0.f, 0.f}, g2[4] = {0.f, 0.f, 0.f, 0.f}, piv[4] = {0.f, 0.f, 0.f, 0.f};
-#pragma unroll
-    for (int i = 0; i < NIT; ++i) {
-      const int idx = TXB == 8 ? (((tid >> 6) * NIT + i) << 6) + (tid & 63) : i * NT + tid;
-      const int c = idx / PCF, q = idx % PCF;
-      const float4 v0 = *reinterpret_cast<const float4*>(plane_of(c) + 4 * q);
-      const int k = kb * w2::kNC + 16 * blk + c;
-      const float bv = (EPI & 1) ? bias[k] : 0.0f;
-      size_t o;
-      if (TXB == 8) {
-        const int row = q >> 3, c4 = q & 7;
-        o = (((size_t)img * K + k) * H + y0 + row) * W + x0 + 4 * c4;
-      } else {
-        o = ((size_t)(img + (q >> 6)) * K + k) * 256 + 4 * (q & 63);
-      }
-      float4 v = make_float4(v0.x + bv, v0.y + bv, v0.z + bv, v0.w + bv);
-      if (EPI & 2) {
-        const float4 rv = *reinterpret_cast<const float4*>(res + o);
-        v.x += rv.x;
-        v.y += rv.y;
-        v.z += rv.z;
-        v.w += rv.w;
-      }
-      if (dbg & 128) __builtin_nontemporal_store(f32x4{v.x, v.y, v.z, v.w}, reinterpret_cast<f32x4*>(y + o));
-      else if (!(dbg & 64)) *reinterpret_cast<float4*>(y + o) = v;
-      if (TXB == 8 && gnp) {
-        if ((i & 1) == 0) piv[i >> 1] = __builtin_bit_cast(float, __builtin_amdgcn_readfirstlane(__builtin_bit_cast(int, v.x)));
-        const float p = piv[i >> 1];
-        const float dx = v.x - p, dy = v.y - p, dz = v.z - p, dw = v.w - p;
-        g1[i >> 1] += (dx + dy) + (dz + dw);
-        g2[i >> 1] += (dx * dx + dy * dy) + (dz * dz + dw * dw);
-      }
-    }
-    if (TXB == 8 && gnp) {
-      float a[4] = {g1[0], g2[0], g1[1], g2[1]}, b[4] = {g1[2], g2[2], g1[3], g2[3]};
-      float u[4];
-#pragma unroll
-      for (int j = 0; j < 4; ++j) {
-        asm volatile("s_nop 1\n\tv_permlane32_swap_b32 %0, %1" : "+v"(a[j]), "+v"(b[j]));
-        u[j] = a[j] + b[j];
-      }
-      float w[2];
-#pragma unroll
-      for (int j = 0; j < 2; ++j) {
-        float x0 = u[j], x1 = u[j + 2];
-        asm volatile("s_nop 1\n\tv_permlane16_swap_b32 %0, %1" : "+v"(x0), "+v"(x1));
-        w[j] = x0 + x1;
-      }
-      const int lane = tid & 63;
-      const bool hi = (lane & 8) != 0;
-      const float keep = hi ? w[1] : w[0], send = hi ? w[0] : w[1];
-      float x = keep + dpp_read<0x140>(send);
-      x += dpp_read<0x141>(x);
-      x += dpp_read<0x4E>(x);
-      x += dpp_read<0xB1>(x);
-      const float x2 = __shfl_xor(x, 8, 64);
-      if ((lane & 15) == 0) {
-        const int r = lane >> 4;
-        const int J = (tid >> 6) * NIT + 2 * r;
-        const int c = (J << 6) / PCF, piece = ((J << 6) % PCF) >> 6;
-        const int k = kb * w2::kNC + 16 * blk + c;
-        const int seg = ((y0 + 8 * piece) >> 4) * (W >> 5) + (x0 >> 5);
-        const float p = r == 0 ? piv[0] : r == 1 ? piv[1] : r == 2 ? piv[2] : piv[3];
-        constexpr float inv_n = 1.0f / 512.0f;
-        gnp[((size_t)img * K + k) * (size_t)((H >> 4) * (W >> 5)) + seg] =
-            make_float2(p + x * inv_n, fmaxf(x2 - x * (x * inv_n), 0.0f));
-      }
-    }
-    if (blk == 0) __syncthreads();
-  }
-}
-
-template <int EPI, int TXB, int NW = 8>
+    }
+  }
+}
+
+template <int EPI, int TXB, int NW = 8, bool S2 = false>
 __global__ __launch_bounds__(NW * WAVE) __attribute__((amdgpu_waves_per_eu(2, 2))) void wino2_kernel(
     const float* __restrict__ x, const float* __restrict__ U, const float* __restrict__ bias,
     const float* __restrict__ res, float* __restrict__ y, int nimg, int C, int K, int H, int W, int bw, int bpi,
@@ -973,13 +1061,14 @@
   __shared__ __attribute__((aligned(16))) float R0[w2::GeoT<TXB, NW>::RAWF], R1[w2::GeoT<TXB, NW>::RAWF],
       R2[(TXB == 4 && NW == 4) ? 4 : w2::GeoT<TXB, NW>::RAWF],
       R3[(TXB == 8 && NW == 8 && SKP_W2_RS4) ? w2::GeoT<TXB, NW>::RAWF : 4];
-  __shared__ __attribute__((aligned(16))) float U0[w2::kUF], U1[w2::kUF], U2[NW == 4 ? 4 : w2::kUF];
+  constexpr int UF = S2 ? w2::kUF2 : w2::kUF;
+  __shared__ __attribute__((aligned(16))) float U0[UF], U1[UF], U2[NW == 4 ? 4 : UF];
   const int G = gridDim.x;
   const int g = blockIdx.x;
   const int Lg = (G % 8 == 0) ? (g % 8) * (G / 8) + g / 8 : g;
   const int sp = Lg / (nblk * nkb);
   const int L = Lg - sp * (nblk * nkb);
-  y += (size_t)sp * nimg * K * ((EPI & 4) ? (H / 2) * (W / 2) : H * W);
+  y += (size_t)sp * nimg * K * (S2 ? (H / 2) * (W / 2) : H * W);
   int tb, kb;
   if (kb_major) {
     kb = L / nblk;
@@ -1002,8 +1091,8 @@
   const W2Smem sm{R0, R1, R2, R3, U0, U1, U2};
   const int c0 = sp * csplit;
   if (wv < NW / 2)
-    wino2_body<EPI, 0, TXB, NW>(sm, x, U, bias, res, y, C, K, H, W, img, x0, y0, kb, c0, csplit, wv, dbg, gnp);
-  else wino2_body<EPI, 1, TXB, NW>(sm, x, U, bias, res, y, C, K, H, W, img, x0, y0, kb, c0, csplit, wv, dbg, gnp);
+    wino2_body<EPI, 0, TXB, NW, false, S2>(sm, x, U, bias, res, y, C, K, H, W, img, x0, y0, kb, c0, csplit, wv, dbg, gnp);
+  else wino2_body<EPI, 1, TXB, NW, false, S2>(sm, x, U, bias, res, y, C, K, H, W, img, x0, y0, kb, c0, csplit, wv, dbg, gnp);
 }
 
 __global__ void wino2_weights_kernel(const float* __restrict__ w, int K, int C, int flip, float* __restrict__ U) {
@@ -1030,6 +1119,25 @@
     for (int b = 0; b < 6; ++b) {
       const int p = 6 * a + b;
       out[p < 18 ? p : p + 2] = (float)(t[a][0] * Gm[b][0] + t[a][1] * Gm[b][1] + t[a][2] * Gm[b][2]);
+    }
+}
+
+__global__ void wino2s2_weights_kernel(const float* __restrict__ w, int K, int C, float* __restrict__ U) {
+  const long long i = blockIdx.x * (long long)blockDim.x + threadIdx.x;
+  if (i >= (long long)K * C) return;
+  const int k = (int)(i / C), c = (int)(i - (long long)k * C);
+  double g[9];
+  for (int u = 0; u < 9; ++u) g[u] = (double)w[((size_t)k * C + c) * 9 + u];
+  const double Gm[5][3] = {{1.0, 0.0, 0.0}, {1.0, 0.0, 1.0}, {0.0, 0.0, 1.0}, {0.0, 1.0, 0.0}, {0.0, 1.0, 0.0}};
+  double t[5][3];
+  for (int a = 0; a < 5; ++a)
+    for (int v = 0; v < 3; ++v) t[a][v] = Gm[a][0] * g[v] + Gm[a][1] * g[3 + v] + Gm[a][2] * g[6 + v];
+  float* out = U + (((size_t)(k / w2::kNC) * C + c) * w2::kNC + (k % w2::kNC)) * w2::kUP2;
+  for (int p = 0; p < w2::kUP2; ++p) out[p] = 0.0f;
+  for (int a = 0; a < 5; ++a)
+    for (int b = 0; b < 5; ++b) {
+      const int p = 5 * a + b;
+      out[p < 15 ? p : p + 1] = (float)(t[a][0] * Gm[b][0] + t[a][1] * Gm[b][1] + t[a][2] * Gm[b][2]);
     }
 }
 
@@ -1129,6 +1237,17 @@
   return SKP_OK;
 }
 
+extern "C" int skp_wino2s2_weights(const float* w, int K, int C, float* U, void* stream) {
+  SKP_CHECK_ARG(w && U, "null pointer");
+  SKP_CHECK_ARG(K > 0 && C > 0, "non-positive shape");
+  SKP_CHECK_ARG(K % w2::kNC == 0, "output channels must be a multiple of 32");
+  const long long n = (long long)K * C;
+  hipLaunchKernelGGL(wino2s2_weights_kernel, dim3((unsigned)((n + 255) / 256)), dim3(256), 0, as_stream(stream), w, K,
+                     C, U);
+  SKP_LAUNCH_CHECK();
+  return SKP_OK;
+}
+
 namespace {
 int wino_nt_flag(long long out_bytes, int nsplit) {
   if (nsplit > 1) return 0;
@@ -1136,8 +1255,8 @@
 }
 }
 
-extern "C" int skp_conv3x3s2_wino2(const float* x, const float* U, const float* bias, float* y, int B, int C, int K,
-                                   int H, int W, int nsplit, float* ws, void* stream) {
+extern "C" int skp_conv3x3s2_f2(const float* x, const float* U, const float* bias, float* y, int B, int C, int K,
+                                int H, int W, int nsplit, float* ws, void* stream) {
   SKP_CHECK_ARG(x && U && y, "null pointer");
   SKP_CHECK_ARG(B > 0 && C > 0 && K > 0 && H > 0 && W > 0, "non-positive shape");
   SKP_CHECK_ARG(C % w2::kCK == 0, "input channels must be a multiple of 4");
@@ -1156,11 +1275,11 @@
   const dim3 grid((unsigned)(nblk * nkb * nsplit));
   const int fl = SKP_WINO2_DEBUG | wino_nt_flag((long long)B * K * (H / 2) * (W / 2) * 4, nsplit);
   if (nsplit == 1 && bias)
-    hipLaunchKernelGGL((wino2_kernel<5, 8, 4>), grid, dim3(4 * WAVE), 0, st, x, U, bias, nullptr, out, B, C, K, H, W,
-                       bw, bpi, (int)nblk, nkb, 0, C / nsplit, fl, nullptr);
+    hipLaunchKernelGGL((wino2_kernel<1, 8, 4, true>), grid, dim3(4 * WAVE), 0, st, x, U, bias, nullptr, out, B, C, K, H,
+                       W, bw, bpi, (int)nblk, nkb, 0, C / nsplit, fl, nullptr);
   else
-    hipLaunchKernelGGL((wino2_kernel<4, 8, 4>), grid, dim3(4 * WAVE), 0, st, x, U, nullptr, nullptr, out, B, C, K, H,
-                       W, bw, bpi, (int)nblk, nkb, 0, C / nsplit, fl, nullptr);
+    hipLaunchKernelGGL((wino2_kernel<0, 8, 4, true>), grid, dim3(4 * WAVE), 0, st, x, U, nullptr, nullptr, out, B, C, K,
+                       H, W, bw, bpi, (int)nblk, nkb, 0, C / nsplit, fl, nullptr);
   SKP_LAUNCH_CHECK();
   if (nsplit > 1) return splitk_reduce(ws, nsplit, B, K, (H / 2) * (W / 2), bias, nullptr, y, st);
   return SKP_OK;
diff --git a/stablekeypoints_amd/ops.py b/stablekeypoints_amd/ops.py
--- a/stablekeypoints_amd/ops.py
+++ b/stablekeypoints_amd/ops.py
@@ -1361,8 +1361,12 @@
         return hit[1]
     w = _c(weight.detach())
     K, C = (w.shape[0], w.shape[1]) if not flip else (w.shape[1], w.shape[0])
-    U = torch.empty(K * C * (40 if v2 else 36), device=w.device, dtype=F32)
-    call("skp_wino2_weights" if v2 else "skp_wino_weights", ptr(w), K, C, int(flip), ptr(U), stream(w.device))
+    if v2 == "s2":
+        U = torch.empty(K * C * 28, device=w.device, dtype=F32)
+        call("skp_wino2s2_weights", ptr(w), K, C, ptr(U), stream(w.device))
+    else:
+        U = torch.empty(K * C * (40 if v2 else 36), device=w.device, dtype=F32)
+        call("skp_wino2_weights" if v2 else "skp_wino_weights", ptr(w), K, C, int(flip), ptr(U), stream(w.device))
     per[(flip, v2)] = (weight._version, U)
     return U
 
@@ -1562,7 +1566,7 @@
 
 
 WINO_S2 = True
-WINO_S2_MIN_PIXELS = 384 * 384
+WINO_S2_MIN_PIXELS = 128 * 128
 
 
 def conv3x3_s2_eligible(x, weight):
@@ -1581,15 +1585,15 @@
     B, C, H, W = x.shape
     K = weight.shape[0]
     y = torch.empty(B, K, H // 2, W // 2, device=x.device, dtype=F32)
-    U = _wino_u(weight, False, True)
+    U = _wino_u(weight, False, "s2")
     b = None if bias is None else _c(bias.detach())
     bmax = max(1, (2 ** 31 - 1) // (C * H * W * 4))
     for b0 in range(0, B, bmax):
         b1 = min(B, b0 + bmax)
         _, nsplit, _ = _wino_plan(b1 - b0, C, K, H, W)
         ws = torch.empty(nsplit, b1 - b0, K, H // 2, W // 2, device=x.device, dtype=F32) if nsplit > 1 else None
-        with _timed("skp_conv3x3s2_wino2", 0):
-            call("skp_conv3x3s2_wino2", ptr(x[b0:b1]), ptr(U), ptr(b), ptr(y[b0:b1]), b1 - b0, C, K, H, W, nsplit,
+        with _timed("skp_conv3x3s2_f2", 0):
+            call("skp_conv3x3s2_f2", ptr(x[b0:b1]), ptr(U), ptr(b), ptr(y[b0:b1]), b1 - b0, C, K, H, W, nsplit,
                  ptr(ws), stream(x.device))
     return y
 
```

New measurement: 45.50, median of 6. 1.01x the previous value.
